# cage-challenge/cage-challenge-4

Measured on AMD Instinct MI355X. Metric: agent-env steps/sec (5 blue agents x N envs), higher is better.
Workload: dtype int32

## Files before the change

### cage_challenge_4_amd/csrc/cc4_engine.h

```cpp
#pragma once
#include "cc4_state.h"
#include "cc4_tables.h"

namespace cc4 {

struct Ctx { EnvState* s; EnvCold* c; Rng* r; HostDyn* hd; StepWork* w; unsigned long long* prof = nullptr;
             unsigned long long* aprof = nullptr; EvLog* lg = nullptr; const uint64_t* gpre = nullptr;
             const ExtAct* ext = nullptr; };

#if defined(__HIP_DEVICE_COMPILE__)
#define CC4_TICK(x, i) do { if ((x).prof) { unsigned long long _t = clock64(); (x).prof[(i)] += _t - (x).prof[15]; (x).prof[15] = _t; } } while (0)
#define CC4_TICK0(x) do { if ((x).prof) (x).prof[15] = clock64(); } while (0)
#define CC4_AT0(x) unsigned long long _at = (x).aprof ? clock64() : 0
#define CC4_AT(x, k) do { if ((x).aprof) { unsigned long long _n = clock64(); (x).aprof[(k)] += _n - _at; _at = _n; } } while (0)
#if defined(CC4_FINE)
#define CC4_FT0(x, r) unsigned long long _ft = ((x).aprof && (r) == 0) ? clock64() : 0
#define CC4_FT(x, r, k) do { if ((x).aprof && (r) == 0) { unsigned long long _n = clock64(); (x).aprof[88 + (k)] += _n - _ft; _ft = _n; } } while (0)
#else
#define CC4_FT0(x, r) do { } while (0)
#define CC4_FT(x, r, k) do { } while (0)
#endif
#else
#define CC4_FT0(x, r) do { } while (0)
#define CC4_FT(x, r, k) do { } while (0)
// ... 238 lines not shown
    const P8 q = proc_load8(x, h, i0);
    int hit = -1;
    CC4_UNROLL for (int k = 7; k >= 0; --k) if (i0 + k < n && pw_pid(q.v[k]) == pid) hit = i0 + k;
    if (hit >= 0) return hit;
  }
  return -1;
}
CC4_HD int find_proc(Ctx x, int h, int pid) { return find_proc(x, h, pid, proc_head(x, h)); }
CC4_HD int proc_ports(Ctx x, int h, const P8N& hd0) {
  const int n = hd0.n;
  int used = 0;
  CC4_UNROLL for (int k = 0; k < 8; ++k) if (k < n) used |= kind_port(pw_kind(hd0.v[k]));
  for (int i0 = 8; i0 < n; i0 += 8) {
    const P8 q = proc_load8(x, h, i0);
    CC4_UNROLL for (int k = 0; k < 8; ++k) if (i0 + k < n) used |= kind_port(pw_kind(q.v[k]));
  }
  return used;
}
CC4_HD int proc_ports(Ctx x, int h) { return proc_ports(x, h, proc_head(x, h)); }
CC4_HD void remove_proc_at(Ctx x, int h, int idx) {
  hd_touch(x, h);
  HostDyn& d = x.hd[h];
  const int n = d.nproc;
  for (int i0 = idx & ~7; i0 < n; i0 += 8) {
    const P8 q = proc_load8(x, h, i0);
    const uint32_t nxt = (i0 + 8 < n) ? proc_get(x, h, i0 + 8) : 0u;
    uint32_t* p = const_cast<uint32_t*>(proc_round_ptr(x, h, i0));
    CC4_UNROLL for (int k = 0; k < 8; ++k) {
      const int i = i0 + k;
      if (i < idx || i + 1 >= n) continue;
      p[k] = k < 7 ? q.v[(k + 1) & 7] : nxt;
    }
  }
  d.nproc = (uint16_t)(n - 1);
}
CC4_HD void ev_conn(Ctx x, int h) { ev_or(x, h, EV_CUR_CONN); }
CC4_HD void ev_proc(Ctx x, int h, int pid) {
  ev_or(x, h, EV_CUR_PROC);
  if (pid > 0 && blue_of_subnet(h_subnet(h)) >= 0) {
    if (x.s->npend >= MAX_PEND) { set_err(x, E_PEND_OVERFLOW); return; }
    x.s->pend[x.s->npend++] = ((uint32_t)h << 16) | (uint32_t)pid;
  }
}
CC4_HD void ev_proc_red(Ctx x, int r, int h, int pid) {
  ev_or(x, h, EV_CUR_PROC);
  if (blue_of_subnet(h_subnet(h)) >= 0) x.w->pend_r[r] = ((uint32_t)h << 16) | (uint32_t)pid;
}
CC4_HD void step_red_merge(Ctx x) {
  EnvState* s = x.s;
  uint32_t pr[NRED];
  CC4_UNROLL for (int r = 0; r < NRED; ++r) pr[r] = x.w->pend_r[r];
  CC4_UNROLL for (int r = 0; r < NRED; ++r) {
    if (!pr[r]) continue;
    if (s->npend >= MAX_PEND) set_err(x, E_PEND_OVERFLOW); else s->pend[s->npend++] = pr[r];
    x.w->pend_r[r] = 0;
  }
}
CC4_HD void pend_drop_host(Ctx x, int h) {
  EnvState* s = x.s;
  int n = 0;
  for (int i = 0; i < s->npend; ++i) if ((int)(s->pend[i] >> 16) != h) s->pend[n++] = s->pend[i];
  s->npend = (uint8_t)n;
}
CC4_HD bool subnet_blocked(Ctx x, int src_sub, int other_sub) { return (x.s->blocks[other_sub] >> src_sub) & 1u; }

struct S8 { uint64_t v[8]; uint64_t slots; };
CC4_HD uint64_t rs_word(const EnvState* s, int slot) { uint64_t v; __builtin_memcpy(&v, &s->spool[slot], 8); return v; }
CC4_HD void rs_word_put(EnvState* s, int slot, uint64_t v) { __builtin_memcpy(&s->spool[slot], &v, 8); }
CC4_HD S8 rs_load8(const EnvState* s, const RedAgent& a, int i0) {
  S8 q;
  __builtin_memcpy(&q.slots, &a.sord[i0], 8);
  CC4_UNROLL for (int k = 0; k < 8; ++k) q.v[k] = rs_word(s, (int)((q.slots >> (8 * k)) & 0xFF));
  return q;
}
CC4_HD int s8_slot(const S8& q, int k) { return (int)((q.slots >> (8 * k)) & 0xFF); }
CC4_HD int rsw_id(uint64_t v) { return (int)(v & 0xFFFF); }
CC4_HD int rsw_pid(uint64_t v) { return (int)((v >> 16) & 0xFFFF); }
CC4_HD int rsw_host(uint64_t v) { return (int)((v >> 32) & 0xFF); }
CC4_HD int rsw_flags(uint64_t v) { return (int)((v >> 40) & 0xFF); }
CC4_HD uint64_t rsw_make(int id, int pid, int host, int flags) {
  return (uint64_t)(id & 0xFFFF) | ((uint64_t)(pid & 0xFFFF) << 16) | ((uint64_t)(host & 0xFF) << 32) | ((uint64_t)(flags & 0xFF) << 40);
}
CC4_HD uint64_t rs_at(const EnvState* s, const RedAgent& a, int i) { return rs_word(s, a.sord[i]); }
CC4_HD int rs_find_id(const EnvState* s, const RedAgent& a, int id, int n) {
  for (int i0 = 0; i0 < n; i0 += 8) {
    const S8 q = rs_load8(s, a, i0);
    int hit = -1;
    CC4_UNROLL for (int k = 7; k >= 0; --k) if (i0 + k < n && rsw_id(q.v[k]) == id) hit = i0 + k;
    if (hit >= 0) return hit;
  }
  return -1;
}
CC4_HD int rs_find_id(const EnvState* s, const RedAgent& a, int id) { return rs_find_id(s, a, id, a.h.nsess); }
struct HostSess { int n, first, first_root; };
CC4_HD HostSess rs_on_host(const EnvState* s, const RedAgent& a, int h) {
  HostSess r; r.n = 0; r.first = -1; r.first_root = -1;
  const int n = a.h.nsess;
  for (int i0 = 0; i0 < n; i0 += 8) {
    const S8 q = rs_load8(s, a, i0);
    CC4_UNROLL for (int k = 0; k < 8; ++k)
      if (i0 + k < n && rsw_host(q.v[k]) == h) {
        r.n++;
        if (r.first < 0) r.first = i0 + k;
        if (r.first_root < 0 && (rsw_flags(q.v[k]) & RS_ROOT)) r.first_root = i0 + k;
      }
  }
  return r;
}
CC4_HD int rs_kth_on_host(const EnvState* s, const RedAgent& a, int h, int kth) {
  const int n = a.h.nsess;
  for (int i0 = 0; i0 < n; i0 += 8) {
    const S8 q = rs_load8(s, a, i0);
    int hit = -1;
    CC4_UNROLL for (int k = 0; k < 8; ++k)
      if (hit < 0 && i0 + k < n && rsw_host(q.v[k]) == h) { if (kth == 0) hit = i0 + k; kth--; }
    if (hit >= 0) return hit;
  }
  return -1;
}
CC4_HD int rs_find_host_pid(const EnvState* s, const RedAgent& a, int h, int pid) {
  const int n = a.h.nsess;
  for (int i0 = 0; i0 < n; i0 += 8) {
    const S8 q = rs_load8(s, a, i0);
    int hit = -1;
    CC4_UNROLL for (int k = 7; k >= 0; --k) if (i0 + k < n && rsw_host(q.v[k]) == h && rsw_pid(q.v[k]) == pid) hit = i0 + k;
    if (hit >= 0) return hit;
  }
  return -1;
}
struct RedPre { int si = -1; HostSess hs = {0, -1, -1}; bool ok = false; };
#if defined(__HIPCC__)
__device__ __forceinline__ RedPre rs_wave_query(const EnvState* s, int lane, int sid, int host) {
  const int r = lane >> 3, k = lane & 7, ra = r < NRED ? r : 0;
  const RedAgent& A = s->red[ra];
  const int ksid = __builtin_amdgcn_ds_bpermute(ra << 2, sid), khost = __builtin_amdgcn_ds_bpermute(ra << 2, host);
  const int n = (r < NRED && ksid >= 0) ? (int)A.h.nsess : 0;
  const int sh = 8 * k;
  RedPre p; p.ok = true;
  for (int i0 = 0; __ballot(i0 < n); i0 += 8) {
    const bool v = i0 + k < n;
    uint64_t w = 0;
    if (v) w = rs_word(s, A.sord[i0 + k]);
    const bool on = v && rsw_host(w) == khost;
    const uint32_t bid = (uint32_t)(__ballot(v && rsw_id(w) == ksid) >> sh) & 0xFFu;
    const uint32_t bh = (uint32_t)(__ballot(on) >> sh) & 0xFFu, br = (uint32_t)(__ballot(on && (rsw_flags(w) & RS_ROOT)) >> sh) & 0xFFu;
    if (p.si < 0 && bid) p.si = i0 + ctz32(bid);
    p.hs.n += __popc(bh);
    if (p.hs.first < 0 && bh) p.hs.first = i0 + ctz32(bh);
    if (p.hs.first_root < 0 && br) p.hs.first_root = i0 + ctz32(br);
  }
  return p;
}
#endif
CC4_HD void rs_list_remove(RedAgent& a, int idx) {
  uint64_t w[MAX_RS / 8];
  __builtin_memcpy(w, a.sord, MAX_RS);
  const int wi = idx >> 3, sh = 8 * (idx & 7);
  CC4_UNROLL for (int k = 0; k < MAX_RS / 8; ++k) {
    if (k < wi) continue;
    const uint64_t nxt = k + 1 < MAX_RS / 8 ? w[k + 1] : 0ull;
    uint64_t v = (w[k] >> 8) | (nxt << 56);
    if (k == wi && sh) v = (w[k] & ((1ull << sh) - 1ull)) | (v & ~((1ull << sh) - 1ull));
    w[k] = v;
  }
  __builtin_memcpy(a.sord, w, MAX_RS);
}
CC4_HD int rs_alloc_lowest(Ctx x) {
  for (int w = 0; w < RS_POOL / 32; ++w) {
    const uint32_t fr = ~x.s->spool_used[w];
    if (fr) return w * 32 + ctz32(fr);
  }
  return -1;
}
CC4_HD void rs_reserve(Ctx x) {
  uint32_t used[RS_POOL / 32];
  CC4_UNROLL for (int w = 0; w < RS_POOL / 32; ++w) used[w] = x.s->spool_used[w];
  int ty[NRED];
  CC4_UNROLL for (int r = 0; r < NRED; ++r) ty[r] = x.s->rexec[r].type;
  CC4_UNROLL for (int r = 0; r < NRED; ++r) {
    int slot = 0xFF;
    if (ty[r] == RA_EXPLOIT) {
      CC4_UNROLL for (int w = 0; w < RS_POOL / 32; ++w) {
        const uint32_t fr = ~used[w];
        if (slot == 0xFF && fr) { slot = w * 32 + ctz32(fr); used[w] |= 1u << (slot & 31); }
      }
    }
    x.w->rs_slot[r] = (uint8_t)slot;
  }
}
CC4_HD int rs_reserve_lane(const EnvState* s, uint32_t exploit_mask, int r) {
  if (!((exploit_mask >> r) & 1u)) return 0xFF;
  int k = popc32(exploit_mask & ((1u << r) - 1u));
  int slot = 0xFF;
  CC4_UNROLL for (int w = 0; w < RS_POOL / 32; ++w) {
    const uint32_t fr = ~s->spool_used[w];
    const int c = popc32(fr);
    if (slot == 0xFF) { if (k < c) slot = w * 32 + nth_bit(fr, k); else k -= c; }
  }
  return slot;
}
CC4_HD int rs_add(Ctx x, int r, int host, int pid, int flags, int slot = -1) {
  EnvState* s = x.s;
  RedAgent& a = s->red[r];
  if (slot < 0) slot = rs_alloc_lowest(x);
  if (a.h.nsess >= MAX_RS || slot < 0 || slot >= RS_POOL) { set_err(x, E_RSESS_OVERFLOW); return -1; }
  int id = 0;
  for (int i0 = 0; i0 < a.h.nsess; i0 += 8) {
    const S8 q = rs_load8(s, a, i0);
    CC4_UNROLL for (int k = 0; k < 8; ++k) if (i0 + k < a.h.nsess && rsw_id(q.v[k]) + 1 > id) id = rsw_id(q.v[k]) + 1;
  }
  (void)or_shared(&s->spool_used[slot >> 5], 1u << (slot & 31));
  rs_word_put(s, slot, rsw_make(id, pid, host, flags));
  if (flags & RS_ABSTRACT) {
    uint64_t* row = reinterpret_cast<uint64_t*>(x.c->kports[slot]);
    for (int k = 0; k < (MAXH + 7) / 8; ++k) row[k] = 0;
  }
  a.sord[a.h.nsess++] = (uint8_t)slot;
  a.h.rsc_dirty = 1; a.h.fsm_dirty = 1;
  if (!bit_get(a.live_hosts, host)) { bit_set(a.live_hosts, host); a.h.nlive++; }
  bit_set_shared(s->red_hosts, host);
  return a.h.nsess - 1;
}
CC4_HD void rs_host_left(Ctx x, int r, int gone) {
  RedAgent& a = x.s->red[r];
  bit_clr(a.live_hosts, gone); a.h.nlive--;
  uint32_t lw[NRED];
  CC4_UNROLL for (int q = 0; q < NRED; ++q) lw[q] = x.s->red[q].live_hosts[gone >> 5];
  uint32_t any_other = 0;
  CC4_UNROLL for (int q = 0; q < NRED; ++q) any_other |= lw[q];
  if (!((any_other >> (gone & 31)) & 1u)) bit_clr_shared(x.s->red_hosts, gone);
}
CC4_HD void rs_remove_at(Ctx x, int r, int idx, bool keep_record = false) {
  EnvState* s = x.s;
  RedAgent& a = s->red[r];
  const int slot = a.sord[idx];
  const int gone = rsw_host(rs_word(s, slot));
  if (!keep_record) bit_clr_shared(s->spool_used, slot);
  rs_list_remove(a, idx);
  a.h.nsess--;
  a.h.rsc_dirty = 1; a.h.fsm_dirty = 1;
  if (rs_on_host(s, a, gone).n == 0) rs_host_left(x, r, gone);
}
CC4_HD void rs_remove_on_host(Ctx x, int r, int h) {
  EnvState* s = x.s;
  RedAgent& a = s->red[r];
  const int n = a.h.nsess;
  int out = 0, removed = 0;
  bool left = false;
  for (int i0 = 0; i0 < n; i0 += 8) {
    const S8 q = rs_load8(s, a, i0);
    CC4_UNROLL for (int k = 0; k < 8; ++k) {
      if (i0 + k >= n) continue;
      const bool here = rsw_host(q.v[k]) == h;
      if (here && !(rsw_flags(q.v[k]) & RS_ORIG)) { bit_clr_shared(s->spool_used, s8_slot(q, k)); removed++; continue; }
      if (here) left = true;
      if (out != i0 + k) a.sord[out] = (uint8_t)s8_slot(q, k);
      out++;
    }
  }
  if (!removed) return;
  a.h.nsess = (uint8_t)out;
  a.h.rsc_dirty = 1; a.h.fsm_dirty = 1;
  if (!left) rs_host_left(x, r, h);
}
CC4_HD void rs_move_to_end(EnvState* s, RedAgent& a, int idx, int new_id) {
  const int slot = a.sord[idx];
  rs_list_remove(a, idx);
  a.sord[a.h.nsess - 1] = (uint8_t)slot;
  if (new_id >= 0) rs_word_put(s, slot, (rs_word(s, slot) & ~0xFFFFull) | (uint64_t)(new_id & 0xFFFF));
  a.h.rsc_dirty = 1;
}
CC4_HD bool sid_known(const RedAgent& a, const uint16_t* ks, int id, int nknown) {
  if (id < 256) return bit_get(a.known_bm, id);
  for (int i = 0; i < nknown; ++i) if (ks[i] == id) return true;
  return false;
}
CC4_HD void as_know_sid(Ctx x, int r, int id) {
  RedAgent& a = x.s->red[r];
  if (sid_known(a, x.c->known_sid[r], id, a.h.nknown)) return;
  if (a.h.nknown >= MAX_KS) { set_err(x, E_KS_OVERFLOW); return; }
  x.c->known_sid[r][a.h.nknown++] = (uint16_t)id;
  if (id < 256) bit_set(a.known_bm, id);
}
CC4_HD void obs_put(Ctx x, int r, bool key_ip, int host, int flags, bool subnet_known) {
  RedAgent& a = x.s->red[r];
  if (flags & OE_IFACE) bit_set(a.as_ip, host);
  if (flags & OE_SYSHN) bit_set(a.as_hn, host);
  if (subnet_known) a.h.as_subnet |= (uint16_t)(1u << h_subnet(host));
  uint8_t want = (uint8_t)(key_ip ? OE_KEY_IP : 0);
  uint32_t* has = a.obs_has[key_ip ? 1 : 0];
  if (bit_get(has, host)) {
    for (int i = 0; i < a.h.nobs; ++i)
      if (a.obs[i].host == host && (a.obs[i].flags & OE_KEY_IP) == want) { a.obs[i].flags |= (uint8_t)flags; return; }
  }
  bit_set(has, host);
  if (a.h.nobs >= MAX_OBS) { set_err(x, E_OBS_OVERFLOW); return; }
  a.obs[a.h.nobs].host = (uint8_t)host;
  a.obs[a.h.nobs].flags = (uint8_t)(flags | want);
  a.h.nobs++;
}
CC4_HD void obs_first(Ctx x, int r, int success, int atype, int ahost, int aarg) {
  RedAgent& a = x.s->red[r];
  if (a.h.obs_success != 0) return;
  a.h.obs_success = (uint8_t)success; a.h.obs_act_type = (uint8_t)atype; a.h.obs_act_host = (uint8_t)ahost; a.h.obs_act_arg = (uint8_t)aarg;
}

CC4_HD int path_to_root(int h, uint8_t* out) {
  int n = 0;
  out[n++] = (uint8_t)h;
  if (h == H_INTERNET) return n;
  int s = h_subnet(h);
  if (!h_is_router(h)) out[n++] = (uint8_t)h_make(s, 0);
  while (true) {
    int p = router_parent(s);
    if (p == S_INT) { out[n++] = (uint8_t)H_INTERNET; break; }
    out[n++] = (uint8_t)h_make(p, 0);
    s = p;
  }
  return n;
}
CC4_HD int route(int src, int dst, uint8_t* work) {
  uint8_t* a = work; uint8_t* b = work + 6; uint8_t* out = work + 12;
  int na = path_to_root(src, a), nb = path_to_root(dst, b);
  while (na >= 2 && nb >= 2 && a[na - 2] == b[nb - 2]) { na--; nb--; }
  int n = 0;
  for (int i = 0; i < na; ++i) out[n++] = a[i];
  for (int i = nb - 2; i >= 0; --i) out[n++] = b[i];
  return n;
}

CC4_HD int gen_pid(Ctx x, uint32_t* used) {
  while (true) {
    int pid = rng_range(x.r, 1000, 10000);
    if (!bit_get(used, pid - 1000)) { bit_set(used, pid - 1000); return pid; }
  }
}
CC4_HD int start_session_proc(Ctx x, int h, int kind) {
  HostDyn& st = x.hd[h];
  int mx = 0;
  for (int i = 0; i < st.nproc; ++i) if (st.procs[i].pid > mx) mx = st.procs[i].pid;
  int pid = mx + 1 + (int)rng_below(x.r, 9);
  st.procs[st.nproc].pid = (uint16_t)pid; st.procs[st.nproc].kind = (uint8_t)kind; st.procs[st.nproc].flags = 0;
  st.nproc++;
  return pid;
}
CC4_HD void host_backup(Ctx x, int h, int ip_octet) {
  const HostDyn& d = x.hd[h];
  HostStatic st;
  for (int i = 0; i < 8; ++i) st.procs[i] = d.procs[i];
  for (int i = 0; i < 5; ++i) st.svcs[i] = d.svcs[i];
  st.nproc = (uint8_t)d.nproc; st.nsvc = (uint8_t)hd_nsvc(d); st.exists = (uint8_t)(1 | ((d.gtmp & 1) << 1)); st.ip_octet = (uint8_t)ip_octet;
  if (d.nproc > PIN - 1 || hd_nsvc(d) > 5) set_err(x, E_PROC_OVERFLOW);
  __builtin_memcpy(&x.c->hs[h], &st, sizeof(HostStatic));
}
CC4_HD void host_restore(Ctx x, int h) {
  hd_touch(x, h);
  HostDyn& d = x.hd[h];
  HostStatic st;
  __builtin_memcpy(&st, &x.c->hs[h], sizeof(HostStatic));
  for (int i = 0; i < 8; ++i) d.procs[i] = st.procs[i];
  for (int i = 0; i < 5; ++i) d.svcs[i] = st.svcs[i];
  d.nproc = st.nproc; d.gtmp = 0; d.nsf = st.nsvc;
  x.s->hev[h] = 0;
  eph_clear(x, h);
  pend_drop_host(x, h);
}

struct ResetCarry { uint64_t env_key; };
enum : int { RESET_WS_SEEN = 0, RESET_WS_DUP = 288, RESET_WS_HOSTS = 576, RESET_WS_WORDS = 584 };

CC4_HD void reset_zero(EnvState* s, HostDyn* hd, EnvCold* c, int t, int nt) {
  static_assert(offsetof(EnvState, rng) == 0, "the generator leads the row");
  uint32_t* w = (uint32_t*)s;
  for (size_t i = sizeof(Rng) / 4 + (size_t)t; i < offsetof(EnvState, hd) / 4; i += (size_t)nt) w[i] = i == PA_WORD ? w[i] & PA_WORD_MASK : 0;
  uint32_t* hw = (uint32_t*)hd;
  for (size_t i = (size_t)t; i < sizeof(HostDyn) * MAXH / 4; i += (size_t)nt) hw[i] = 0;
  uint32_t* b = (uint32_t*)c->hs;
  for (size_t i = (size_t)t; i < sizeof(c->hs) / 4; i += (size_t)nt) b[i] = 0;
}
static_assert(sizeof(RSess) * RS_POOL >= 4 * 282, "the idle session pool holds the 9000-bit pid set of the generation");
CC4_HD uint32_t* reset_used_set(EnvState* s) { return reinterpret_cast<uint32_t*>(s->spool); }
CC4_HD void reset_used_clear(EnvState* s, int t, int nt) { uint32_t* u = reset_used_set(s); for (int i = t; i < 282; i += nt) u[i] = 0; }
template <int RNG_MODE>
CC4_HD void reset_gen_host(Ctx x, int h) {
  EnvState* s = x.s;
  if (!bit_get(s->exists, h)) return;
  if (RNG_MODE == 1) rng_set_stream(x.r, ST_GEN_HOST + (uint32_t)h);
  HostDyn& st = x.hd[h];
  st.gtmp = (uint8_t)rng_below(x.r, 2);
  if (h_is_router(h)) return;
  int n = 0;
  auto put = [&](int kind, int pid) {
    st.svcs[n].kind = (uint8_t)kind; st.svcs[n].pid = (uint16_t)pid; st.svcs[n].st = (uint8_t)(SV_ACTIVE | 5);
    st.procs[n].kind = (uint8_t)kind; st.procs[n].pid = (uint16_t)pid; st.procs[n].flags = 0;
    n++;
  };
  auto pid = [&]() { return RNG_MODE == 1 ? rng_range(x.r, 1000, 10000) : gen_pid(x, reset_used_set(s)); };
  put(K_SSHD, pid());
  int sub = h_subnet(h);
  if (sub == S_OZA || sub == S_OZB) put(K_OT, pid());
  int p_apache = pid(), p_mysql = pid(), p_smtp = pid();
  int n_add = (int)rng_below(x.r, 4);
  uint32_t left = 7;
  for (int k = 0; k < n_add; ++k) {
    int o = nth_bit(left, (int)rng_below(x.r, (uint32_t)popc32(left)));
    left &= ~(1u << o);
    put(o == 0 ? K_APACHE : (o == 1 ? K_MYSQL : K_SMTP), o == 0 ? p_apache : (o == 1 ? p_mysql : p_smtp));
  }
  for (int i = 0; i < n; ++i) (void)rng_random(x.r);
  hd_set_nsvc(st, n); st.nproc = (uint16_t)n;
  if (RNG_MODE == 1) { st.procs[5].pid = (uint16_t)p_apache; st.procs[6].pid = (uint16_t)p_mysql; st.svcs[6].pid = (uint16_t)p_smtp; }
}
struct ResetHostLater { CC4_HD void operator()(Ctx, int) const {} };
struct ResetHostNow { CC4_HD void operator()(Ctx x, int h) const { reset_gen_host<0>(x, h); } };
CC4_HD void reset_mission_phases(EnvState* s, int steps) {
  int q = steps / 3, rem = steps % 3;
  s->steps = steps;
  s->phase_len[0] = q + (rem >= 1 ? 1 : 0); s->phase_len[1] = q + (rem == 2 ? 1 : 0); s->phase_len[2] = q;
}
template <int RNG_MODE, typename HostHook>
CC4_HD ResetCarry reset_topology(Ctx x, uint64_t seed, int steps, bool continue_stream, int policy, uint32_t topo_seed, uint32_t* ws,
                                 bool rng_is_copy, HostHook host_placed) {
  EnvState* s = x.s;
  if (!continue_stream) rng_seed(&s->rng, seed, (uint32_t)RNG_MODE);
  s->rng_mode = (uint8_t)RNG_MODE;
  s->policy = (uint8_t)policy_at_reset(s, policy);
  rng_begin_episode(x.r);
  ResetCarry k; k.env_key = x.r->s_lo;
  if (RNG_MODE == 1 && topo_seed) x.r->s_lo = (uint64_t)topo_seed;
  reset_mission_phases(s, steps);
  if (RNG_MODE == 1) for (int i = 0; i < RESET_WS_WORDS; ++i) ws[i] = 0;
  {
    uint32_t* avail = x.w->scratch;
    for (int i = 0; i < 8; ++i) avail[i] = 0xFFFFFFFFu;
    int n = 256;
    for (int sn = 0; sn < NSUB; ++sn) {
      int v = nth_set(avail, 8, (int)rng_below(x.r, (uint32_t)n));
      s->cidr_octet[sn] = (uint8_t)v;
      bit_clr(avail, v);
      n--;
    }
  }
  for (int sn = 0; sn < NSUB; ++sn) {
    uint32_t* ips = x.w->scratch;
    for (int i = 0; i < 8; ++i) ips[i] = 0xFFFFFFFFu;
    ips[0] &= ~1u; ips[7] &= 0x7FFFFFFFu;
    int n = 254;
    auto place = [&](int h, int v) {
      bit_clr(ips, v); n--; bit_set(s->exists, h); x.hd[h].procs[PIN - 1].pid = (uint16_t)v;
      host_placed(x, h);
    };
    if (sn == S_INT) { place(H_INTERNET, nth_set(ips, 8, (int)rng_below(x.r, (uint32_t)n))); continue; }
    place(h_make(sn, 0), nth_set(ips, 8, (int)rng_below(x.r, (uint32_t)n)));
    int nu = 3 + (int)rng_below(x.r, 8);
    for (int i = 0; i < nu; ++i) place(h_make(sn, 1 + i), nth_set(ips, 8, (int)rng_below(x.r, (uint32_t)n)));
    int ns = 1 + (int)rng_below(x.r, 6);
    for (int i = 0; i < ns; ++i) place(h_make(sn, 11 + i), last_set(ips, 8));
    s->n_users[sn] = (uint8_t)nu; s->n_servers[sn] = (uint8_t)ns;
  }
  if (RNG_MODE == 1 && rng_is_copy) s->rng = *x.r;
  return k;
}
CC4_HD void reset_pid_serial(Ctx x, uint32_t* used) {
  EnvState* s = x.s;
  for (int h = 0; h < MAXH; ++h) {
    if (!bit_get(s->exists, h) || h_is_router(h)) continue;
    HostDyn& st = x.hd[h];
    const int n = hd_nsvc(st);
    const int sub = h_subnet(h);
    const int nfix = (sub == S_OZA || sub == S_OZB) ? 2 : 1;
    Rng t; bool forked = false;
    auto settle = [&](int v0, bool* moved) {
      int v = v0 - 1000;
      *moved = false;
      while (bit_get(used, v)) {
        if (!forked) { rng_fork(&t, x.r, ST_GEN_REDRAW + (uint32_t)h); forked = true; }
        v = (int)rng_below(&t, 9000);
        *moved = true;
      }
      bit_set(used, v);
      return v + 1000;
    };
    for (int i = 0; i < nfix; ++i) {
      bool moved;
      const int v = settle(st.svcs[i].pid, &moved);
      if (moved) { st.svcs[i].pid = (uint16_t)v; st.procs[i].pid = (uint16_t)v; }
    }
    for (int k = 0; k < 3; ++k) {
      const int kind = k == 0 ? K_APACHE : (k == 1 ? K_MYSQL : K_SMTP);
      const int v0 = k == 0 ? st.procs[5].pid : (k == 1 ? st.procs[6].pid : st.svcs[6].pid);
      bool moved;
      const int v = settle(v0, &moved);
      if (moved) for (int i = nfix; i < n; ++i) if (st.svcs[i].kind == kind) { st.svcs[i].pid = (uint16_t)v; st.procs[i].pid = (uint16_t)v; }
    }
    st.procs[5].pid = 0; st.procs[6].pid = 0; st.svcs[6].pid = 0;
  }
}
CC4_HD void reset_agents(Ctx x) {
  EnvState* s = x.s;
  for (int b = 0; b < NBLUE; ++b) {
    int nsub = blue_nsub(b);
    (void)rng_below(x.r, (uint32_t)nsub);
    int cnt = 0;
    for (int i = 0; i < nsub; ++i) { int sn = blue_subnet_alloc(b, i); cnt += 1 + s->n_users[sn] + s->n_servers[sn]; }
    int c = (int)rng_below(x.r, (uint32_t)cnt);
    int ph = -1;
    for (int i = 0; i < nsub && ph < 0; ++i) {
      int sn = blue_subnet_alloc(b, i), nu = s->n_users[sn], ns = s->n_servers[sn];
      if (c < 1 + nu) ph = h_make(sn, c);
      else if (c < 1 + nu + ns) ph = h_make(sn, 11 + (c - 1 - nu));
      else c -= 1 + nu + ns;
    }
    s->blue[b].parent_host = (uint8_t)ph;
  }
  {
    int g = 0;
    for (int sn = 0; sn < NSUB - 1; ++sn) for (int i = 0; i < s->n_users[sn]; ++i) s->green_host[g++] = (uint8_t)h_make(sn, 1 + i);
    s->n_green = (uint8_t)g;
  }
  for (int r = 0; r < NRED; ++r) {
    int sn = red_subnet_alloc(r, (int)rng_below(x.r, (uint32_t)red_nsub(r)));
    int c = (int)rng_below(x.r, (uint32_t)(s->n_users[sn] + s->n_servers[sn]));
    s->red[r].h.start_host = (uint8_t)(c < s->n_users[sn] ? h_make(sn, 1 + c) : h_make(sn, 11 + (c - s->n_users[sn])));
    s->red[r].h.new_sess_host = 0xFF;
  }
}
CC4_HD void reset_seal_host(Ctx x, int h) {
  host_backup(x, h, x.hd[h].procs[PIN - 1].pid);
  x.hd[h].procs[PIN - 1].pid = 0; x.hd[h].gtmp = 0;
}
CC4_HD void reset_host_sessions(Ctx x, int h) {
  EnvState* s = x.s;
  if (!bit_get(s->exists, h)) return;
  rng_set_stream(x.r, ST_GEN_SESS + (uint32_t)h);
  if (blue_of_subnet(h_subnet(h)) >= 0) (void)start_session_proc(x, h, K_SESS_BLUE);
  if (h != H_INTERNET && h_is_user(h)) (void)start_session_proc(x, h, K_SESS_GREEN);
  if (h == s->red[0].h.start_host) (void)start_session_proc(x, h, K_SESS_RED);
  reset_seal_host(x, h);
}
CC4_HD void reset_sessions_agent_order(Ctx x) {
  EnvState* s = x.s;
  for (int b = 0; b < NBLUE; ++b) {
    int ph = s->blue[b].parent_host;
    (void)start_session_proc(x, ph, K_SESS_BLUE);
    for (int i = 0; i < blue_nsub(b); ++i) {
      int sn = blue_subnet_alloc(b, i);
      for (int sl = 0; sl < SLOTS; ++sl) {
        int h = h_make(sn, sl);
        if (!bit_get(s->exists, h) || h == ph) continue;
        (void)start_session_proc(x, h, K_SESS_BLUE);
      }
    }
  }
  for (int g = 0; g < s->n_green; ++g) (void)start_session_proc(x, s->green_host[g], K_SESS_GREEN);
  (void)start_session_proc(x, s->red[0].h.start_host, K_SESS_RED);
}
CC4_HD void reset_seal_all_hosts(Ctx x) {
  EnvState* s = x.s;
  for (int h = 0; h < MAXH; ++h) {
    if (bit_get(s->exists, h)) reset_seal_host(x, h);
    eph_clear(x, h);
  }
  s->npend = 0;
}
CC4_HD void reset_finish(Ctx x, ResetCarry k, int steps, uint32_t topo_seed, bool rng_is_copy) {
  EnvState* s = x.s;
  {
    const HostDyn& d = x.hd[s->red[0].h.start_host];
    int red0_pid = 0;
    for (int i = 0; i < d.nproc; ++i) if (d.procs[i].kind == K_SESS_RED) red0_pid = d.procs[i].pid;
    (void)rs_add(x, 0, s->red[0].h.start_host, red0_pid, RS_ABSTRACT | RS_ORIG);
    s->red[0].h.active = 1;
  }
  for (int r = 0; r < NRED; ++r) {
    RedAgent& a = s->red[r];
    int h = a.h.start_host;
    bit_set(a.as_ip, h); bit_set(a.as_hn, h); a.h.as_subnet |= (uint16_t)(1u << h_subnet(h));
    if (r == 0) {
      as_know_sid(x, 0, 0);
      obs_put(x, 0, false, h, OE_SESS | OE_IFACE | OE_SYSHN, true);
      obs_first(x, 0, T_UNKNOWN, RA_NONE, 0, 0);
    }
    a.h.exec_type = RA_SLEEP;
  }
  s->done = (uint8_t)(0 >= steps - 1);
  s->n_actions = NBLUE + s->n_green + NRED;
  if (topo_seed) x.r->s_lo = k.env_key;
  if (rng_is_copy) s->rng = *x.r;
  rng_park(&s->rng);
}
CC4_HD void env_reset_counter_mode(Ctx x, uint64_t seed, int steps, bool continue_stream, int policy, uint32_t topo_seed, uint32_t* ws,
                                   bool rng_is_copy) {
  reset_zero(x.s, x.hd, x.c, 0, 1);
  ResetCarry k = reset_topology<1>(x, seed, steps, continue_stream, policy, topo_seed, ws, rng_is_copy, ResetHostLater{});
  {
    Rng t; rng_fork(&t, x.r, ST_GEN_HOST);
    Ctx xh = x; xh.r = &t;
    for (int h = 0; h < MAXH; ++h) reset_gen_host<1>(xh, h);
  }
  reset_pid_serial(x, reset_used_set(x.s));
  reset_used_clear(x.s, 0, 1);
  reset_agents(x);
  {
    Rng t; rng_fork(&t, x.r, ST_GEN_SESS);
    Ctx xh = x; xh.r = &t;
    for (int h = 0; h < MAXH; ++h) reset_host_sessions(xh, h);
  }
// ... 350 lines not shown
  return h_make(sn, 11 + (c - before));
}
CC4_HD constexpr int green_as_dest_loop(uint64_t pre, int c, int* sn_out) {
  int sn = 0, before = 0;
  for (int k = 0; k < NSUB - 2; ++k) { const int tot = (int)((pre >> (8 * k)) & 0xFF); if (tot <= c) { sn = k + 1; before = tot; } }
  *sn_out = sn;
  return h_make(sn, 11 + (c - before));
}
CC4_HD constexpr uint32_t green_lw_active(uint64_t pre) {
  static_assert(SV_ACTIVE == 0x80 && MAXSV == 7, "the active bit is a status byte's top bit; seven of them");
  return dot4_u8((uint32_t)(pre >> 32) & 0x00808080u, 0x00402010u, dot4_u8((uint32_t)pre & 0x80808080u, 0x08040201u, 0u)) >> 7;
}
CC4_HD constexpr uint32_t green_lw_active_loop(uint64_t pre) {
  uint32_t act = 0;
  for (int i = 0; i < MAXSV; ++i) if ((pre >> (8 * i)) & SV_ACTIVE) act |= 1u << i;
  return act;
}
static_assert(green_lw_active(0x0080818283FF7F80ull) == green_lw_active_loop(0x0080818283FF7F80ull) && green_lw_active(0xFF00000000000000ull) == 0 &&
              green_lw_active(0x0080808080808080ull) == 0x7F && green_lw_active(0x0000000080000000ull) == 0x08, "green_lw_active == the loop");
namespace cc4_forms_check {
constexpr uint32_t sv[MAXSV] = {0x81000001u, 0x05FFFFFFu, 0x80123456u, 0x7F000000u, 0xFFFFFFFFu, 0x01020304u, 0x85000000u};
static_assert(green_lw_status(sv, 7) == green_lw_status_loop(sv, 7) && green_lw_status(sv, 7) == 0x008501FF7F800581ull && green_lw_status(sv, 0) == 0 &&
              green_lw_status(sv, 4) == green_lw_status_loop(sv, 4) && green_lw_status(sv, 5) == 0x000000FF7F800581ull, "green_lw_status == the loop");
constexpr int dest_sn(uint64_t pre, int c, bool loop) { int sn = 0; const int d = loop ? green_as_dest_loop(pre, c, &sn) : green_as_dest(pre, c, &sn); return d * 16 + sn; }
constexpr uint64_t tot = 0x302A241E18120C06ull, gap = 0x0909090903030300ull;
static_assert(dest_sn(tot, 0, false) == dest_sn(tot, 0, true) && dest_sn(tot, 5, false) == dest_sn(tot, 5, true) && dest_sn(tot, 6, false) == dest_sn(tot, 6, true) &&
              dest_sn(tot, 47, false) == dest_sn(tot, 47, true) && dest_sn(tot, 41, false) == dest_sn(tot, 41, true) && dest_sn(gap, 0, false) == dest_sn(gap, 0, true) &&
              dest_sn(gap, 2, false) == dest_sn(gap, 2, true) && dest_sn(gap, 3, false) == dest_sn(gap, 3, true) && dest_sn(gap, 8, false) == dest_sn(gap, 8, true),
              "green_as_dest == the loop");
}
CC4_HD bool green_local_work(Ctx x, int gh, uint64_t pre, bool* want_phish, double fp_rate = 0.01, double phish_rate = 0.01) {
  const uint32_t act = green_lw_active(pre);
  if (!act) return false;
  const int c = nth_bit8(act, (int)rng_below(x.r, (uint32_t)popc32(act)));
  const uint32_t st = (uint32_t)(pre >> (8 * c)) & 0xFF;
  int rel = (int)(st & 0x7F) * 20;
  if ((int)rng_below(x.r, 100) >= rel) return false;
  if (rng_random_lt(x.r, fp_rate)) { int port = eph_port(x, gh); ev_proc(x, gh, 0); ev_log(x, gh, gh, 1, gh, port, 0xFF, 0, 0); }
  if (rng_random_lt(x.r, phish_rate)) *want_phish = true;
  return true;
}
CC4_HD bool green_access_service(Ctx x, int gh, uint64_t pre, double fp_rate = 0.01) {
  int own = h_subnet(gh);
  const int n = (int)(pre >> 56);
  const int c = (int)rng_below(x.r, (uint32_t)n);
  int sn;
  const int dest = green_as_dest(pre, c, &sn);
  const int dest_port = eph_port(x, dest);
  int ds = sn;
  if (subnet_blocked(x, ds, own) || subnet_blocked(x, own, ds)) { ev_conn(x, dest); ev_log(x, gh, dest, 0, dest, 0, gh, 8800, 0); return false; }
  if (rng_random_lt(x.r, fp_rate)) { ev_conn(x, dest); ev_log(x, gh, dest, 0, gh, 0, dest, dest_port, 0); }
  return true;
}

CC4_HD void red_result(Ctx x, int r, const Act& a, int success) {
  int arg = a.type == RA_DRS ? a.arg : 0;
  obs_first(x, r, success, a.type, a.host, arg);
}
CC4_HD void red_drs(Ctx x, int r, const Act& a, RedPre pre = RedPre()) {
  EnvState* s = x.s;
  int sn = a.arg; bool any = false;
  if ((pre.ok ? pre.si : rs_find_id(s, s->red[r], a.sid)) < 0) { red_result(x, r, a, T_FALSE); return; }
  bool allowed = (red_allowed_mask(r) >> sn) & 1u;
  RedAgent& A = s->red[r];
  const int lo = sn * SLOTS + 1, w0 = lo >> 5, off = lo & 31, w1 = (w0 + 1 < 5) ? w0 + 1 : w0;
  const uint32_t e0 = s->exists[w0], e1 = s->exists[w1], h0 = A.obs_has[1][w0], h1 = A.obs_has[1][w1];
  auto field = [&](uint32_t a0, uint32_t a1) { uint32_t v = a0 >> off; if (off > 16 && w1 != w0) v |= a1 << (32 - off); return v & 0xFFFFu; };
  const uint32_t ex = field(e0, e1);
  any = ex != 0;
  if (allowed && ex) {
    const uint32_t had = field(h0, h1) & ex;
    uint32_t fresh = ex & ~had;
    const uint32_t m0 = ex << off, m1 = (off > 16 && w1 != w0) ? ex >> (32 - off) : 0u;
    A.as_ip[w0] |= m0; A.obs_has[1][w0] = h0 | m0;
    if (m1) { A.as_ip[w1] |= m1; A.obs_has[1][w1] = h1 | m1; }
    A.h.as_subnet |= (uint16_t)(1u << sn);
    int n = A.h.nobs;
    while (fresh) {
      const int b = ctz32(fresh); fresh &= fresh - 1;
      if (n >= MAX_OBS) { set_err(x, E_OBS_OVERFLOW); break; }
      A.obs[n].host = (uint8_t)(lo + b); A.obs[n].flags = (uint8_t)(OE_IFACE | OE_KEY_IP);
      n++;
    }
    A.h.nobs = (uint8_t)n;
    uint32_t again = had;
    while (again) { const int b = ctz32(again); again &= again - 1; obs_put(x, r, true, lo + b, OE_IFACE, true); }
  }
  red_result(x, r, a, any ? T_TRUE : T_UNKNOWN);
}
CC4_HD int port_of_bit(int pb) { return pb == PB_22 ? 22 : (pb == PB_80 ? 80 : (pb == PB_3390 ? 3390 : (pb == PB_25 ? 25 : (pb == PB_1 ? 1 : 443)))); }
CC4_HD void red_scan(Ctx x, int r, const Act& a, double rate, RedPre pre = RedPre()) {
  EnvState* s = x.s;
  RedAgent& A = s->red[r];
  int si = pre.ok ? pre.si : rs_find_id(s, A, a.sid);
  if (si < 0) { red_result(x, r, a, T_FALSE); return; }
  const int slot = A.sord[si];
  const uint64_t sw = rs_word(s, slot);
  if (!(rsw_flags(sw) & RS_ABSTRACT)) { red_result(x, r, a, T_FALSE); return; }
  int src = rsw_host(sw), tgt = a.host;
  if (subnet_blocked(x, h_subnet(src), h_subnet(tgt))) { red_result(x, r, a, T_FALSE); return; }
  const bool fixed_le_rate = rng_random_le(x.r, rate);
  int ports = 0;
  const P8N hd0 = proc_head(x, tgt);
  const int np = hd0.n;
  for (int i0 = 0; i0 < np; i0 += 8) {
    P8 q = p8_of(hd0);
    if (i0) q = proc_load8(x, tgt, i0);
    CC4_UNROLL for (int k8 = 0; k8 < 8; ++k8) {
      if (i0 + k8 >= np) continue;
      int k = pw_kind(q.v[k8]);
      int pb = kind_port(k);
      if (!pb) continue;
      ports |= pb;
      if (fixed_le_rate || kind_is_decoy(k)) { ev_conn(x, tgt); int ep = eph_port(x, tgt, (i0 + k8) & 63); ev_log(x, 200 + r, tgt, 0, tgt, port_of_bit(pb), src, ep, 0); }
    }
  }
  if (ports) {
    obs_put(x, r, true, tgt, OE_IFACE, false);
    x.c->kports[slot][tgt] = (uint8_t)(PB_HAS | ports);
  }
  red_result(x, r, a, T_TRUE);
}
CC4_HD int exploit_new_session(Ctx x, int r, int parent_sid, int tgt, const P8N& hd0) {
  (void)parent_sid;
  int pid = create_pid(x, tgt, hd0);
  if (!add_proc_n(x, tgt, hd0.n, pid, K_SHELL, 0)) return -1;
  x.hd[tgt].nsf = (uint8_t)((hd0.nsf & 0x0F) | ((((hd0.nsf >> 4) | HF_CMD) & ~HF_ESC_LAST) << 4));
  return rs_add(x, r, tgt, pid, RS_CHILD, x.w->rs_slot[r]);
}
CC4_HD void red_exploit(Ctx x, int r, const Act& a, RedPre pre = RedPre()) {
  EnvState* s = x.s;
  RedAgent& A = s->red[r];
  int si = pre.ok ? pre.si : rs_find_id(s, A, a.sid);
  if (si < 0) { red_result(x, r, a, T_FALSE); return; }
  const int slot = A.sord[si];
  const uint64_t sw = rs_word(s, slot);
  if (!(rsw_flags(sw) & RS_ABSTRACT)) { red_result(x, r, a, T_FALSE); return; }
  int src = rsw_host(sw), tgt = a.host;
  const P8N thd0 = proc_head(x, tgt);
  int known = x.c->kports[slot][tgt];
  if (!(known & PB_HAS)) { red_result(x, r, a, T_FALSE); return; }
  if (subnet_blocked(x, h_subnet(src), h_subnet(tgt))) { red_result(x, r, a, T_FALSE); return; }
  enum { X_HTTPRFI = 0, X_HTTPSRFI = 1, X_SSH = 2, X_SQLI = 3, X_HARAKA = 4 };
  uint32_t opts = 0;
  if (known & PB_80) opts |= 1u << X_HTTPRFI;
  if (known & PB_443) opts |= 1u << X_HTTPSRFI;
  if (known & PB_22) opts |= 1u << X_SSH;
  if ((known & PB_3390) && (known & (PB_80 | PB_443))) opts |= 1u << X_SQLI;
  if (known & PB_25) opts |= 1u << X_HARAKA;
  if (opts == 0) { red_result(x, r, a, T_FALSE); return; }
  int sel = ctz32(opts);
  if (popc32(opts) > 1) {
    int top = (opts >> X_HARAKA) & 1u ? X_HARAKA : ((opts >> X_SQLI) & 1u ? X_SQLI : ((opts >> X_HTTPSRFI) & 1u ? X_HTTPSRFI : X_HTTPRFI));
    opts &= ~(1u << top);
    sel = nth_bit(opts, (int)rng_below(x.r, (uint32_t)popc32(opts)));
    (void)rng_random(x.r);
  }
  const int tnp = thd0.n;
  if (sel == X_SSH) {
    uint8_t* work = reinterpret_cast<uint8_t*>(x.w->scratch + 6 * r);
    int nh = route(src, tgt, work);
    for (int i = 0; i < nh; ++i) if (!rng_random_le(x.r, 0.050000000000000044)) { ev_conn(x, work[12 + i]); ev_log(x, 200 + r, work[12 + i], 0, tgt, 0, src, 22, 0); }
    int vp = -1;
    for (int i0 = 0; i0 < tnp && vp < 0; i0 += 8) {
      P8 q = p8_of(thd0);
      if (i0) q = proc_load8(x, tgt, i0);
      CC4_UNROLL for (int k = 7; k >= 0; --k) if (i0 + k < tnp && pw_kind(q.v[k]) == K_SSHD) vp = i0 + k;
    }
    if (vp < 0) { red_result(x, r, a, T_FALSE); return; }
    obs_put(x, r, true, tgt, OE_IFACE, false);
    const int bf_port = eph_port(x, tgt);
    ev_conn(x, tgt);
    ev_log(x, 200 + r, tgt, 0, tgt, 22, src, bf_port, 0, 10);
    int ni = exploit_new_session(x, r, a.sid, tgt, thd0);
    if (ni < 0) { red_result(x, r, a, T_FALSE); return; }
    const uint64_t nw = rs_at(s, A, ni);
    ev_proc_red(x, r, tgt, rsw_pid(nw));
    ev_log(x, 200 + r, tgt, 1, 0xFF, 0, 0xFF, 0, rsw_pid(nw));
    obs_put(x, r, true, tgt, OE_SESS | OE_IFACE | OE_SYSHN, false);
    obs_put(x, r, true, src, OE_IFACE, false);
    A.h.new_sess_host = (uint8_t)tgt; A.h.new_sess_id = (uint16_t)rsw_id(nw);
    red_result(x, r, a, T_TRUE);
    return;
  }
  int vp = -1, vk = 0;
  {
    const uint32_t want = sel == X_HTTPRFI ? ((1u << K_APACHE) | (1u << K_DEC_APACHE) | (1u << K_DEC_VSFTPD))
                        : sel == X_HTTPSRFI ? (1u << K_DEC_TOMCAT)
                        : sel == X_SQLI ? (1u << K_MYSQL)
                        : ((1u << K_SMTP) | (1u << K_DEC_HARAKA));
    for (int i0 = 0; i0 < tnp && vp < 0; i0 += 8) {
      P8 q = p8_of(thd0);
      if (i0) q = proc_load8(x, tgt, i0);
      CC4_UNROLL for (int k = 7; k >= 0; --k) if (i0 + k < tnp && ((want >> pw_kind(q.v[k])) & 1u)) { vp = i0 + k; vk = pw_kind(q.v[k]); }
    }
  }
  if (vp < 0) { red_result(x, r, a, T_FALSE); return; }
  bool decoy = kind_is_decoy(vk);
  const int xport = sel == X_HTTPRFI ? 80 : (sel == X_HTTPSRFI ? 443 : (sel == X_SQLI ? 3390 : 25));
  if (decoy) { ev_conn(x, tgt); int ep = eph_port(x, tgt, 1); ev_log(x, 200 + r, tgt, 0, tgt, xport, src, ep, 0); }
  obs_put(x, r, true, tgt, OE_IFACE, false);
  bool works = (sel == X_SQLI) || decoy;
  if (!works) { red_result(x, r, a, T_FALSE); return; }
  if (rng_random_le(x.r, 0.0)) { red_result(x, r, a, T_FALSE); return; }
  const int lport = eph_port(x, tgt, 2);
  if (decoy) { ev_conn(x, tgt); int ep = eph_port(x, tgt, 3); ev_log(x, 200 + r, tgt, 0, tgt, lport, src, ep, 0); red_result(x, r, a, T_FALSE); return; }
  int ni = exploit_new_session(x, r, a.sid, tgt, thd0);
  if (ni < 0) { red_result(x, r, a, T_FALSE); return; }
  const uint64_t nw = rs_at(s, A, ni);
  if (!rng_random_le(x.r, 0.050000000000000044)) { ev_proc_red(x, r, tgt, rsw_pid(nw)); ev_log(x, 200 + r, tgt, 1, 0xFF, 0, 0xFF, 0, rsw_pid(nw)); }
  obs_put(x, r, true, tgt, OE_SESS | OE_IFACE | OE_SYSHN, false);
  obs_put(x, r, true, src, OE_IFACE, false);
  A.h.new_sess_host = (uint8_t)tgt; A.h.new_sess_id = (uint16_t)rsw_id(nw);
  red_result(x, r, a, T_TRUE);
}
CC4_HD void red_privesc(Ctx x, int r, const Act& a, RedPre pre = RedPre()) {
  EnvState* s = x.s;
  RedAgent& A = s->red[r];
  int h = a.host;
  const HostSess hs = pre.ok ? pre.hs : rs_on_host(s, A, h);
  const int n = hs.n;
  int target = hs.first_root;
  if (n == 0) { red_result(x, r, a, T_FALSE); return; }
  if (target < 0) {
    target = rs_kth_on_host(s, A, h, (int)rng_below(x.r, (uint32_t)n));
    { int ss = pre.ok ? pre.si : rs_find_id(s, A, a.sid);
      if (ss < 0 || !(rsw_flags(rs_at(s, A, ss)) & RS_ABSTRACT)) { red_result(x, r, a, T_FALSE); return; } }
    const int tslot = A.sord[target];
    s->spool[tslot].flags |= RS_ROOT;
    hd_touch(x, h);
    hd_set_files(x.hd[h], hd_files(x.hd[h]) | HF_ESC | HF_ESC_LAST);
    int pi = find_proc(x, h, s->spool[tslot].pid);
    if (pi >= 0) proc_put(x, h, pi, proc_get(x, h, pi) | ((uint32_t)PF_ROOT << 24));
  }
  obs_put(x, r, false, h, OE_SESS, false);
  { const uint64_t tw = rs_at(s, A, target); if (rsw_flags(tw) & RS_ABSTRACT) as_know_sid(x, r, rsw_id(tw)); }
  if ((pre.ok ? pre.si : rs_find_id(s, A, a.sid)) >= 0 && h_slot(h) == 11) {
    uint32_t m = info_links(h_subnet(h));
    for (int sn = 0; sn < NSUB; ++sn) if ((m >> sn) & 1u) obs_put(x, r, false, h_make(sn, 11), OE_IFACE, false);
  }
  red_result(x, r, a, T_TRUE);
}
CC4_HD void red_impact(Ctx x, int r, const Act& a, RedPre pre = RedPre()) {
  EnvState* s = x.s;
  RedAgent& A = s->red[r];
  int h = a.host;
  if ((pre.ok ? pre.hs : rs_on_host(s, A, h)).first_root < 0) { red_result(x, r, a, T_FALSE); return; }
  HostDyn& d = x.hd[h];
  const SvTab sv = svc_load(d);
  int si = -1;
  uint32_t sw = 0;
  CC4_UNROLL for (int i = MAXSV - 1; i >= 0; --i) if (i < sv.n && svw_kind(sv.w[i]) == K_OT && (svw_st(sv.w[i]) & SV_ACTIVE)) { si = i; sw = sv.w[i]; }
  if (si < 0) { red_result(x, r, a, T_FALSE); return; }
  if ((pre.ok ? pre.si : rs_find_id(s, A, a.sid)) < 0) { red_result(x, r, a, T_FALSE); return; }
  hd_touch(x, h);
  d.svcs[si].st = (uint8_t)(svw_st(sw) & ~SV_ACTIVE);
  int pi = find_proc(x, h, (int)(sw & 0xFFFF));
  if (pi >= 0) remove_proc_at(x, h, pi);
  obs_put(x, r, false, h, 0, false);
  red_result(x, r, a, T_TRUE);
}
CC4_HD void red_degrade(Ctx x, int r, const Act& a, RedPre pre = RedPre()) {
  EnvState* s = x.s;
  RedAgent& A = s->red[r];
  int h = a.host;
  if ((pre.ok ? pre.hs : rs_on_host(s, A, h)).first_root < 0) { red_result(x, r, a, T_FALSE); return; }
  HostDyn& d = x.hd[h];
  int n = 0;
  hd_touch(x, h);
  const SvTab sv = svc_load(d);
  CC4_UNROLL for (int i = 0; i < MAXSV; ++i) if (i < sv.n && (svw_st(sv.w[i]) & SV_ACTIVE)) {
    n++;
    int rel = svw_st(sv.w[i]) & 0x7F;
    if (rel > 0) rel--;
    d.svcs[i].st = (uint8_t)(SV_ACTIVE | rel);
  }
  if (n == 0) { red_result(x, r, a, T_FALSE); return; }
  obs_put(x, r, false, h, 0, false);
  red_result(x, r, a, T_TRUE);
}
CC4_HD void red_deception(Ctx x, int r, const Act& a, RedPre pre = RedPre()) {
  EnvState* s = x.s;
  RedAgent& A = s->red[r];
  if ((pre.ok ? pre.si : rs_find_id(s, A, a.sid)) < 0) { red_result(x, r, a, T_FALSE); return; }
  int tgt = a.host;
  const double det_rate = (x.ext && (a.busy & AQ_RATE0)) ? x.c->xrate[r][0] : 0.5;
  const double fp_rate = (x.ext && (a.busy & AQ_RATE1)) ? x.c->xrate[r][1] : 0.1;
  const P8N hd0 = proc_head(x, tgt);
  const int np = hd0.n;
  for (int i0 = 0; i0 < np; i0 += 8) {
    P8 q = p8_of(hd0);
    if (i0) q = proc_load8(x, tgt, i0);
    CC4_UNROLL for (int k = 0; k < 8; ++k) {
      if (i0 + k >= np) continue;
      bool decoy = kind_is_decoy(pw_kind(q.v[k]));
      bool rep = false;
      if (rng_random_le(x.r, det_rate) && decoy) rep = true;
      else if (rng_random_le(x.r, fp_rate) && !decoy) rep = true;
      if (rep) obs_put(x, r, false, tgt, OE_IFACE, false);
    }
  }
  red_result(x, r, a, T_TRUE);
}
CC4_HD void red_session_check(Ctx x, int r) {
  EnvState* s = x.s;
  RedAgent& A = s->red[r];
  obs_first(x, r, T_TRUE, RA_NONE, 0, 0);
  if (A.h.nsess == 0) return;
  if (rsw_id(rs_at(s, A, 0)) != 0 && rsw_id(rs_at(s, A, A.h.nsess - 1)) != 0 && rs_find_id(s, A, 0) < 0) {
    int c = (int)rng_below(x.r, (uint32_t)A.h.nsess);
    rs_move_to_end(s, A, c, 0);
    for (int i = 0; i < A.h.nsess; ++i) s->spool[A.sord[i]].flags &= (uint8_t)~RS_CHILD;
  }
  A.h.rsc_listed = 1;
  if (!A.h.rsc_dirty) return;
  const B5 live = b5_load(A.live_hosts);
  { const B5 ip = b5_load(A.as_ip), hn = b5_load(A.as_hn); b5_store(A.as_ip, b5_or(ip, live)); b5_store(A.as_hn, b5_or(hn, live)); }
  {
    uint32_t sub = 0;
    CC4_UNROLL for (int sn = 0; sn < NSUB; ++sn) {
      const int lo = sn * SLOTS, w = lo >> 5, off = lo & 31;
      uint32_t bits = live.w[w] >> off;
      if (off > 32 - SLOTS && w + 1 < 5) bits |= live.w[w + 1] << (32 - off);
      if (bits & ((1u << SLOTS) - 1u)) sub |= 1u << sn;
    }
    A.h.as_subnet |= (uint16_t)sub;
  }
  const int n = A.h.nsess;
  int fresh = 0, fresh_id = 0;
  for (int i0 = 0; i0 < n; i0 += 8) {
    const S8 q = rs_load8(s, A, i0);
    uint32_t kw[8];
    CC4_UNROLL for (int k = 0; k < 8; ++k) kw[k] = A.known_bm[(rsw_id(q.v[k]) >> 5) & 7];
    CC4_UNROLL for (int k = 0; k < 8; ++k) {
      if (i0 + k >= n || !(rsw_flags(q.v[k]) & RS_ABSTRACT)) continue;
      const int id = rsw_id(q.v[k]);
      if (id < 256 && ((kw[k] >> (id & 31)) & 1u)) continue;
      fresh++; fresh_id = id;
    }
  }
  if (fresh == 1) as_know_sid(x, r, fresh_id);
  else if (fresh > 1)
    for (int i = 0; i < n; ++i) {
      const int h = rsw_host(rs_at(s, A, i));
      bool first = true;
      for (int j = 0; j < i && first; ++j) first = rsw_host(rs_at(s, A, j)) != h;
      if (!first) continue;
      for (int j = i; j < n; ++j) {
        const uint64_t w = rs_at(s, A, j);
        if (rsw_host(w) == h && (rsw_flags(w) & RS_ABSTRACT)) as_know_sid(x, r, rsw_id(w));
      }
    }
  A.h.rsc_dirty = 0;
}
CC4_HD void red_withdraw(Ctx x, int r, const Act& a, RedPre pre = RedPre()) {
  EnvState* s = x.s;
  RedAgent& A = s->red[r];
  if ((pre.ok ? pre.si : rs_find_id(s, A, a.sid)) < 0) { red_result(x, r, a, T_FALSE); return; }
  const int h = a.arg;
  uint16_t* ids = reinterpret_cast<uint16_t*>(x.w->scratch + 36);
  int n = 0;
  const int cap = (int)((sizeof(x.w->scratch) - 36 * 4) / 2);
  for (int pass = 0; pass < 2; ++pass)
    for (int i = 0; i < A.h.nsess; ++i) {
      const uint64_t w = rs_at(s, A, i);
      if (rsw_host(w) != h) continue;
      bool child = (rsw_flags(w) & RS_CHILD) != 0;
      if ((pass == 0 && child) || (pass == 1 && !child && rsw_id(w) != 0)) { if (n < cap) ids[n++] = (uint16_t)rsw_id(w); else set_err(x, E_RSESS_OVERFLOW); }
    }
  { int self = rs_find_id(s, A, a.sid); if (rsw_host(rs_at(s, A, self)) == h) { if (n < cap) ids[n++] = (uint16_t)a.sid; else set_err(x, E_RSESS_OVERFLOW); } }
  if (n == 0) { red_result(x, r, a, T_FALSE); return; }
  int ok = T_FALSE;
  for (int k = 0; k < n; ++k) {
    int self = rs_find_id(s, A, a.sid), ti = rs_find_id(s, A, ids[k]);
    if (self < 0 || ti < 0) { ok = T_FALSE; break; }
    int pid = rsw_pid(rs_at(s, A, ti));
    int pi = find_proc(x, h, pid);
    if (pi < 0) { ok = T_FALSE; break; }
    kill_process(x, h, pi, proc_get(x, h, pi));
    ok = T_TRUE;
  }
  red_result(x, r, a, ok);
}
CC4_HD void red_execute(Ctx x, int r, const Act& a, RedPre pre = RedPre()) {
  switch (a.type) {
    case RA_DRS: red_drs(x, r, a, pre); break;
    case RA_AGGR: red_scan(x, r, a, (x.ext && (a.busy & AQ_RATE0)) ? x.c->xrate[r][0] : 0.75, pre); break;
    case RA_STEALTH: red_scan(x, r, a, (x.ext && (a.busy & AQ_RATE0)) ? x.c->xrate[r][0] : 0.25, pre); break;
    case RA_DECEPTION: red_deception(x, r, a, pre); break;
    case RA_EXPLOIT: red_exploit(x, r, a, pre); break;
    case RA_PRIVESC: red_privesc(x, r, a, pre); break;
    case RA_IMPACT: red_impact(x, r, a, pre); break;
    case RA_DEGRADE: red_degrade(x, r, a, pre); break;
    case RA_INVALID: obs_first(x, r, T_FALSE, RA_NONE, 0, 0); break;
    case RA_WITHDRAW: red_withdraw(x, r, a, pre); break;
    default: obs_first(x, r, T_UNKNOWN, RA_NONE, 0, 0); break;
  }
}

CC4_HD int fsm_next(int cur, int act, bool success) {
  uint64_t row;
  if (success) switch (cur) {
    case FS_K: row = 0xffffff221ull; break;  case FS_KD: row = 0xffffff331ull; break;
    case FS_S: row = 0xffff42ff3ull; break;  case FS_SD: row = 0xffff53ff3ull; break;
    case FS_U: row = 0x2ff6ffff5ull; break;  case FS_UD: row = 0x3ff7ffff5ull; break;
    case FS_R: row = 0x266fffff7ull; break;  case FS_RD: row = 0x377fffff7ull; break;
    default: row = 0xffffffff8ull; break;
  } else switch (cur) {
    case FS_K: row = 0xffffff000ull; break;  case FS_KD: row = 0xffffff111ull; break;
    case FS_S: row = 0xffff22ff2ull; break;  case FS_SD: row = 0xffff33ff3ull; break;
    case FS_U: row = 0x4ff4ffff4ull; break;  case FS_UD: row = 0x5ff5ffff5ull; break;
    case FS_R: row = 0x666fffff6ull; break;  case FS_RD: row = 0x777fffff7ull; break;
    default: row = 0xffffffff8ull; break;
  }
  int v = (int)((row >> (4 * act)) & 0xF);
  return v == 0xF ? 0xFF : v;
}
CC4_HD int fsm_get(const RedAgent& A, int h) {
  const int v = (A.fsm_st4[h >> 1] >> (4 * (h & 1))) & 0xF;
  return v ? v - 1 : FS_NONE;
}
CC4_HD void fsm_put(RedAgent& A, int h, int st) {
  const int sh = 4 * (h & 1);
  A.fsm_st4[h >> 1] = (uint8_t)((A.fsm_st4[h >> 1] & ~(0xF << sh)) | ((st + 1) << sh));
}
CC4_HD void fsm_set_state(RedAgent& A, int h, int st) {
  if (st >= FS_U && st <= FS_RD) bit_set(A.fsm_ur, h); else bit_clr(A.fsm_ur, h);
  if ((st & 1) || st == FS_F) bit_set(A.fsm_nodrs, h); else bit_clr(A.fsm_nodrs, h);
  fsm_put(A, h, st);
}
CC4_HD void fsm_apply(Ctx x, int r, RedHdr& H, int h, int act, bool success) {
  RedAgent& A = x.s->red[r];
  int cur = fsm_get(A, h);
  if (cur == FS_NONE) return;
  int nx = fsm_next(cur, act, success);
  if (nx == FS_U) nx = ((red_allowed_mask(r) >> h_subnet(h)) & 1u) ? FS_U : FS_F;
  if (nx == 0xFF) nx = cur;
  if (nx != cur) fsm_set_state(A, h, nx);
  if (nx == FS_F && cur != FS_F) {
    int n = 0;
    for (int i = 0; i < H.fsm_n; ++i) if (A.fsm_order[i] != h) A.fsm_order[n++] = A.fsm_order[i];
    H.fsm_n = (uint8_t)n;
  }
}
CC4_HD void fsm_observe(Ctx x, int r, RedHdr& H) {
  RedAgent& A = x.s->red[r];
  CC4_AT0(x);
  if (H.obs_success == T_IN_PROGRESS && H.nobs == 0 && H.rsc_listed && !H.fsm_dirty) return;
  if (H.obs_act_type <= RA_WITHDRAW && H.obs_success != T_IN_PROGRESS && H.obs_success != 0) {
    bool ok = H.obs_success == T_TRUE;
    int t = H.obs_act_type;
    if (t == RA_DRS) {
      const int lo = H.obs_act_arg * SLOTS, hi = lo + SLOTS - 1;
      for (int w = lo >> 5; w <= (hi >> 5) && w < 5; ++w) {
        uint32_t m = A.fsm_known[w];
        if (ok) m &= ~A.fsm_nodrs[w];
        const int l = lo - 32 * w, u = hi - 32 * w;
        if (l > 0) m &= 0xFFFFFFFFu << l;
        if (u < 31) m &= (2u << u) - 1u;
        while (m) { int b = ctz32(m); m &= m - 1; fsm_apply(x, r, H, w * 32 + b, t, ok); }
      }
    } else if (t == RA_PRIVESC || t == RA_IMPACT || t == RA_DEGRADE) {
      int h = H.obs_act_host;
      if (bit_get(A.fsm_known, h) && bit_get(A.fsm_hn, h)) fsm_apply(x, r, H, h, t, ok);
    } else {
      fsm_apply(x, r, H, H.obs_act_host, t, ok);
    }
  }
  CC4_AT(x, 3);
  B5 seen = b5_zero();
  for (int i = 0; i < H.nobs; ++i) {
    int h = A.obs[i].host; int f = A.obs[i].flags;
    if (f & OE_SESS) b5_set(seen, h);
    bool hn = !(f & OE_KEY_IP) || (f & OE_SYSHN);
    bool ip = (f & OE_KEY_IP) || (f & OE_IFACE);
    if (!ip) {
      if (!(bit_get(A.fsm_known, h) && bit_get(A.fsm_hn, h))) { set_err(x, E_UNREACHABLE); }
      continue;
    }
    if (!bit_get(A.fsm_known, h)) {
      fsm_set_state(A, h, H.fsm_step == 0 ? FS_U : FS_K);
      A.fsm_order[H.fsm_n++] = (uint8_t)h;
      bit_set(A.fsm_known, h);
    }
    if (hn) bit_set(A.fsm_hn, h);
  }
  CC4_AT(x, 4);
  if (H.rsc_listed) {
    const B5 live = b5_load(A.live_hosts), known = b5_load(A.fsm_known), hn = b5_load(A.fsm_hn);
    seen = b5_or(seen, live);
    if (b5_any(b5_andn(live, known)))
      for (int i = 0; i < H.nsess; ++i) {
        int h = rsw_host(rs_at(x.s, A, i));
        if (bit_get(A.fsm_known, h)) continue;
        fsm_set_state(A, h, H.fsm_step == 0 ? FS_U : FS_K);
        A.fsm_order[H.fsm_n++] = (uint8_t)h;
        bit_set(A.fsm_known, h);
      }
    b5_store(A.fsm_hn, b5_or(hn, live));
    H.fsm_dirty = 0;
  }
  CC4_AT(x, 5);
  {
    const B5 lost = b5_andn(b5_load(A.fsm_ur), seen);
    if (b5_any(lost))
      CC4_UNROLL for (int w = 0; w < 5; ++w) {
        uint32_t m = lost.w[w];
        while (m) { int b = ctz32(m); m &= m - 1; fsm_set_state(A, w * 32 + b, FS_KD); }
      }
  }
  CC4_AT(x, 6);
}
CC4_HD int fsm_choose_host_discovery(Ctx x, int r, RedHdr& H) {
  RedAgent& A = x.s->red[r];
  uint32_t order = 0; int nst = 0; uint32_t seen = 0;
  for (int i = 0; i < H.fsm_n && nst < 8; ++i) {
    int st = fsm_get(A, A.fsm_order[i]);
    if (!((seen >> st) & 1u)) { seen |= 1u << st; order |= (uint32_t)st << (4 * nst); nst++; }
  }
  int sum = 0;
  for (int k = 0; k < nst; ++k) { int st = (order >> (4 * k)) & 0xF; sum += st <= FS_SD ? 20 : (st <= FS_UD ? 10 : 0); }
  int chosen_state;
  if (sum > 0) {
    double mult = 1.0 / ((double)sum / 100.0);
    double last = 0.0;
    for (int k = 0; k < nst; ++k) { int st = (order >> (4 * k)) & 0xF; int p = st <= FS_SD ? 20 : (st <= FS_UD ? 10 : 0); last = last + ((double)p / 100.0) * mult; }
    double u = rng_random(x.r);
    double run = 0.0; int idx = 0;
    for (int k = 0; k < nst; ++k) {
      int st = (order >> (4 * k)) & 0xF; int p = st <= FS_SD ? 20 : (st <= FS_UD ? 10 : 0);
      run = run + ((double)p / 100.0) * mult;
      if (run / last <= u) idx++;
    }
    if (idx >= nst) idx = nst - 1;
    chosen_state = (order >> (4 * idx)) & 0xF;
  } else {
    chosen_state = (order >> (4 * (int)rng_below(x.r, (uint32_t)nst))) & 0xF;
  }
  int n_all = 0, n_srv = 0;
  for (int i = 0; i < H.fsm_n; ++i) {
    int h = A.fsm_order[i];
    if (fsm_get(A, h) != chosen_state) continue;
    n_all++;
    if (h_is_server(h) && bit_get(A.fsm_hn, h)) n_srv++;
  }
  int want_srv = -1;
  if (n_all > 1 && n_srv > 0) {
    double i01 = rng_random(x.r);
    want_srv = (i01 <= 0.75 || n_srv == n_all) ? 1 : 0;
  }
  int cnt = want_srv < 0 ? n_all : (want_srv ? n_srv : n_all - n_srv);
  int c = (int)rng_below(x.r, (uint32_t)cnt);
  for (int i = 0; i < H.fsm_n; ++i) {
    int h = A.fsm_order[i];
    if (fsm_get(A, h) != chosen_state) continue;
    bool srv = h_is_server(h) && bit_get(A.fsm_hn, h);
    if (want_srv >= 0 && (int)srv != want_srv) continue;
    if (c-- == 0) return h;
  }
  return A.fsm_order[0];
}
CC4_HD constexpr uint32_t fsm_pk_switch(bool discovery, int host_state) {
  if (!discovery) switch (host_state) {
    case FS_K:  return 0xF432u << 16 | (RA_DRS | RA_AGGR << 4 | RA_STEALTH << 8);
    case FS_KD: return 0xFF42u << 16 | (RA_AGGR | RA_STEALTH << 4);
    case FS_S:  return 0xF431u << 16 | (RA_DRS | RA_EXPLOIT << 4 | RA_DECEPTION << 8);
    case FS_SD: return 0xFF43u << 16 | (RA_EXPLOIT | RA_DECEPTION << 4);
    case FS_U:  return 0xF442u << 16 | (RA_DRS | RA_PRIVESC << 4 | RA_WITHDRAW << 8);
    case FS_UD: return 0xFF44u << 16 | (RA_PRIVESC | RA_WITHDRAW << 4);
    case FS_R:  return 0x4432u << 16 | (RA_DRS | RA_DEGRADE << 4 | RA_IMPACT << 8 | RA_WITHDRAW << 12);
    default:    return 0xF442u << 16 | (RA_DEGRADE | RA_IMPACT << 4 | RA_WITHDRAW << 8);
  } else switch (host_state) {
    case FS_K:  return 0xF441u << 16 | (RA_DRS | RA_AGGR << 4 | RA_STEALTH << 8);
    case FS_KD: return 0xFF44u << 16 | (RA_AGGR | RA_STEALTH << 4);
    case FS_S:  return 0xF441u << 16 | (RA_DRS | RA_EXPLOIT << 4 | RA_DECEPTION << 8);
    case FS_SD: return 0xFF44u << 16 | (RA_EXPLOIT | RA_DECEPTION << 4);
    case FS_U:  return 0xF440u << 16 | (RA_DRS | RA_PRIVESC << 4 | RA_WITHDRAW << 8);
    case FS_UD: return 0xFF44u << 16 | (RA_PRIVESC | RA_WITHDRAW << 4);
    case FS_R:  return 0x4444u << 16 | (RA_DRS | RA_DEGRADE << 4 | RA_IMPACT << 8 | RA_WITHDRAW << 12);
    default:    return 0xF442u << 16 | (RA_DEGRADE | RA_IMPACT << 4 | RA_WITHDRAW << 8);
  }
}
struct FsmPkTab { uint32_t v[16]; };
CC4_HD constexpr int fsm_pk_index(bool discovery, int host_state) { return (discovery ? 8 : 0) + (host_state < 7 ? host_state : 7); }
constexpr FsmPkTab make_fsm_pk_tab() {
  FsmPkTab t{};
  for (int d = 0; d < 2; ++d) for (int st = 0; st < 8; ++st) t.v[fsm_pk_index(d != 0, st)] = fsm_pk_switch(d != 0, st);
  return t;
}
constexpr bool fsm_pk_tab_matches() {
  const FsmPkTab t = make_fsm_pk_tab();
  for (int d = 0; d < 2; ++d) {
    for (int st = 0; st <= FS_F; ++st) if (t.v[fsm_pk_index(d != 0, st)] != fsm_pk_switch(d != 0, st)) return false;
    if (t.v[fsm_pk_index(d != 0, FS_NONE)] != fsm_pk_switch(d != 0, FS_NONE)) return false;
  }
  return true;
}
static_assert(fsm_pk_tab_matches(), "fsm_get_action's option table == its switch");
#if defined(__HIP_DEVICE_COMPILE__)
static __device__ const FsmPkTab fsm_pk_tab = make_fsm_pk_tab();
#else
static constexpr FsmPkTab fsm_pk_tab = make_fsm_pk_tab();
#endif
CC4_HD uint32_t fsm_pk(bool discovery, int host_state) { return fsm_pk_tab.v[fsm_pk_index(discovery, host_state)]; }
CC4_HD Act fsm_get_action(Ctx x, int r, RedHdr& H, bool observed = false) {
  EnvState* s = x.s;
  RedAgent& A = s->red[r];
  Act out; out.type = RA_SLEEP; out.host = 0; out.arg = 0; out.ticks = 1; out.sid = 0; out.busy = 0;
  CC4_FT0(x, r);
  if (!observed) fsm_observe(x, r, H);
  CC4_FT(x, r, 5);
  if (H.obs_success == T_IN_PROGRESS) { H.fsm_step++; return out; }
  int n = H.fsm_n;
  if (n == 0) { set_err(x, E_FSM_NO_HOST); H.fsm_step++; return out; }
  const bool discovery = (s->policy & 3) == RP_DISCOVERY;
  int host;
  if (!discovery) host = A.fsm_order[rng_below(x.r, (uint32_t)n)];
  else host = fsm_choose_host_discovery(x, r, H);
  CC4_FT(x, r, 6);
  const uint32_t pk = fsm_pk(discovery, fsm_get(A, host));
  const int fl = rng_random_quarter(x.r);
  int k = 0;
  for (int i = 0; i < 4; ++i) if ((int)((pk >> (16 + 4 * i)) & 0xF) <= fl) k++;
  int t = (int)((pk >> (4 * k)) & 0xF);
  out.type = (uint8_t)t; out.host = (uint8_t)host;
  bool bad = false;
  if (t == RA_DRS) {
    uint32_t known = H.as_subnet;
    if (known == 0) bad = true; else out.arg = (uint8_t)nth_bit(known, (int)rng_below(x.r, (uint32_t)popc32(known)));
  }
  if ((t == RA_PRIVESC || t == RA_IMPACT || t == RA_DEGRADE) && !bit_get(A.fsm_hn, host)) bad = true;
  if (!bad) {
    if (H.nknown == 0) bad = true; else out.sid = x.c->known_sid[r][rng_below(x.r, (uint32_t)H.nknown)];
  }
  if (bad) { set_err(x, E_UNREACHABLE); out.type = RA_SLEEP; }
  out.ticks = (uint8_t)red_duration(out.type);
  H.fsm_step++;
  CC4_FT(x, r, 7);
  return out;
}
CC4_HD Act random_red_get_action(Ctx x, int r, RedHdr& H) {
  RedAgent& A = x.s->red[r];
  Act out; out.type = RA_SLEEP; out.host = 0; out.arg = 0; out.ticks = 1; out.sid = 0; out.busy = 0;
  const int nip = popc32(A.as_ip[0]) + popc32(A.as_ip[1]) + popc32(A.as_ip[2]) + popc32(A.as_ip[3]) + popc32(A.as_ip[4]);
  const int nhn = popc32(A.as_hn[0]) + popc32(A.as_hn[1]) + popc32(A.as_hn[2]) + popc32(A.as_hn[3]) + popc32(A.as_hn[4]);
  const int nsub = popc32(H.as_subnet), nsid = H.nknown;
  const uint8_t types[10] = {RA_DRS, RA_AGGR, RA_STEALTH, RA_EXPLOIT, RA_PRIVESC, RA_DEGRADE, RA_DECEPTION, RA_IMPACT, RA_WITHDRAW, RA_SLEEP};
  uint32_t valid = 0;
  for (int c = 0; c < 10; ++c) {
    int t = types[c];
    bool ok = true;
    if (t != RA_SLEEP && nsid == 0) ok = false;
    if (t == RA_DRS && nsub == 0) ok = false;
    if ((t == RA_AGGR || t == RA_STEALTH || t == RA_EXPLOIT || t == RA_DECEPTION || t == RA_WITHDRAW) && nip == 0) ok = false;
    if ((t == RA_PRIVESC || t == RA_DEGRADE || t == RA_IMPACT || t == RA_WITHDRAW) && nhn == 0) ok = false;
    if (ok) valid |= 1u << c;
  }
  const int t = types[nth_bit(valid, (int)rng_below(x.r, (uint32_t)popc32(valid)))];
  auto pick_sid = [&]() { return (int)x.c->known_sid[r][rng_below(x.r, (uint32_t)nsid)]; };
  auto pick_ip = [&]() { return nth_set(A.as_ip, 5, (int)rng_below(x.r, (uint32_t)nip)); };
  auto pick_hn = [&]() { return nth_set(A.as_hn, 5, (int)rng_below(x.r, (uint32_t)nhn)); };
  out.type = (uint8_t)t;
  switch (t) {
    case RA_DRS: out.arg = (uint8_t)nth_bit(H.as_subnet, (int)rng_below(x.r, (uint32_t)nsub)); out.sid = (uint16_t)pick_sid(); break;
    case RA_AGGR: case RA_STEALTH: case RA_DECEPTION: out.sid = (uint16_t)pick_sid(); out.host = (uint8_t)pick_ip(); break;
    case RA_EXPLOIT: out.host = (uint8_t)pick_ip(); out.sid = (uint16_t)pick_sid(); break;
    case RA_PRIVESC: case RA_DEGRADE: case RA_IMPACT: out.host = (uint8_t)pick_hn(); out.sid = (uint16_t)pick_sid(); break;
    case RA_WITHDRAW: out.sid = (uint16_t)pick_sid(); out.host = (uint8_t)pick_ip(); out.arg = (uint8_t)pick_hn(); break;
    default: break;
  }
  out.ticks = (uint8_t)red_duration(out.type);
  H.fsm_step++;
  return out;
}
CC4_HD void red_validate(Ctx x, int r, const RedHdr& H, Act& a) {
  RedAgent& A = x.s->red[r];
  if (a.type >= RA_SLEEP) return;
  bool ok = true;
  if (!sid_known(A, x.c->known_sid[r], a.sid, H.nknown)) ok = false;
  if (a.type == RA_DRS) { if (!((H.as_subnet >> a.arg) & 1u)) ok = false; }
  else if (a.type == RA_PRIVESC || a.type == RA_IMPACT || a.type == RA_DEGRADE) { if (!bit_get(A.as_hn, a.host)) ok = false; }
  else if (a.type == RA_WITHDRAW) { if (!bit_get(A.as_ip, a.host) || !bit_get(A.as_hn, a.arg)) ok = false; }
  else { if (!bit_get(A.as_ip, a.host)) ok = false; }
  if (!ok) { a.type = RA_INVALID; a.ticks = 1; }
}

CC4_HD constexpr uint32_t red_zone_hosts(int r, int w) {
  uint32_t m = 0;
  for (int i = 0; i < red_nsub(r); ++i) {
    int lo = red_subnet_alloc(r, i) * SLOTS - 32 * w, hi = lo + SLOTS - 1;
    if (hi < 0 || lo > 31) continue;
    uint32_t up = hi >= 31 ? 0xFFFFFFFFu : ((2u << hi) - 1u);
    uint32_t dn = lo <= 0 ? 0xFFFFFFFFu : (0xFFFFFFFFu << lo);
    m |= up & dn;
  }
  return m;
}
CC4_HD void red_reassign(Ctx x, uint32_t foreign) {
  EnvState* s = x.s;
  uint32_t* mv = x.w->scratch; int nm = 0;
  const int cap = (int)(sizeof(x.w->scratch) / 4);
  for (int r = 0; r < NRED; ++r) {
    if (!((foreign >> r) & 1u)) continue;
    const RedAgent& A = s->red[r];
    const int n = A.h.nsess;
    for (int i0 = 0; i0 < n; i0 += 8) {
      const S8 q = rs_load8(s, A, i0);
      CC4_UNROLL for (int k = 0; k < 8; ++k) {
        if (i0 + k >= n) continue;
        const int host = rsw_host(q.v[k]);
        const int sn = h_subnet(host);
        if ((red_allowed_mask(r) >> sn) & 1u) continue;
        const int to = red_of_subnet(sn);
        if (to < 0) { set_err(x, E_UNREACHABLE); continue; }
        if (nm < cap) mv[nm++] = (uint32_t)r | ((uint32_t)to << 3) | ((uint32_t)(i0 + k) << 6) | ((uint32_t)s8_slot(q, k) << 12);
        else set_err(x, E_RSESS_OVERFLOW);
      }
    }
  }
  int gone_from[NRED];
  CC4_UNROLL for (int r = 0; r < NRED; ++r) gone_from[r] = 0;
  for (int m = 0; m < nm; ++m) {
    const uint32_t w = mv[m];
    const int from = (int)(w & 7u), to = (int)((w >> 3) & 7u), slot = (int)((w >> 12) & 0xFFu);
    RedAgent& F = s->red[from];
    int shift = 0;
    CC4_UNROLL for (int r = 0; r < NRED; ++r) if (r == from) shift = gone_from[r];
    int i = (int)((w >> 6) & 0x3Fu) - shift;
    if (i < 0 || i >= F.h.nsess || F.sord[i] != slot) {
      i = -1;
      for (int k = 0; k < F.h.nsess; ++k) if (F.sord[k] == slot) { i = k; break; }
      if (i < 0) continue;
    }
    CC4_UNROLL for (int r = 0; r < NRED; ++r) if (r == from) gone_from[r]++;
    const uint64_t rec = rs_word(s, slot);
    const int old_host = rsw_host(rec), old_pid = rsw_pid(rec), old_flags = rsw_flags(rec), old_id = rsw_id(rec);
    rs_remove_at(x, from, i, true);
    int ni = rs_add(x, to, old_host, old_pid, RS_ABSTRACT | (old_flags & RS_ROOT), slot);
    if (ni < 0) { bit_clr_shared(s->spool_used, slot); continue; }
    if (F.h.new_sess_host == old_host && F.h.new_sess_id == old_id) {
      obs_first(x, to, T_UNKNOWN, RA_NONE, 0, 0);
      obs_put(x, to, true, old_host, OE_SESS | OE_IFACE | OE_SYSHN, false);
      as_know_sid(x, to, rsw_id(rs_at(s, s->red[to], ni)));
    }
  }
  int ns[NRED];
  CC4_UNROLL for (int r = 0; r < NRED; ++r) ns[r] = s->red[r].h.nsess;
  CC4_UNROLL for (int r = 0; r < NRED; ++r) s->red[r].h.active = (uint8_t)(ns[r] > 0);
}


CC4_HD int step_phase_of(int st, int len0, int len1, int len2) {
  if (st < len0) return 0;
  if (st < len0 + len1) return 1;
  if (st < len0 + len1 + len2) return 2;
  return -1;
}
CC4_HD bool step_phase(Ctx x, bool init_accumulators = true) {
  EnvState* s = x.s;
  {
    const int st = s->step_count;
    const int ph = step_phase_of(st, s->phase_len[0], s->phase_len[1], s->phase_len[2]);
    if (ph < 0) { set_err(x, E_STEP_PAST_END); return false; }
    s->obs_dirty = (uint8_t)(ph > s->phase ? OD_PHASE : 0);
    if (ph > s->phase) s->phase = ph;
  }
  rng_begin_step(&s->rng, (uint32_t)s->step_count);
  if (x.lg) { x.lg->n = 0; x.lg->step = (uint32_t)s->step_count; }
  if (x.ext) { x.c->gfail[0] = 0; x.c->gfail[1] = 0; x.c->gfail[2] = 0; }
  s->action_cost = 0.f;
  if (init_accumulators) {
    s->brm = 0; s->n_restore = 0;
    s->n_actions = NBLUE + s->n_green + NRED;
  }
  return true;
}
CC4_HD Act blue_random_policy(Ctx x, int b) {
  EnvState* s = x.s;
  Act a; a.type = BA_SLEEP; a.host = 0; a.arg = 0; a.ticks = 1; a.sid = 0; a.busy = 0;
  rng_set_stream(x.r, ST_BLUE_POL + (uint32_t)b);
  (void)rng_random(x.r);
  const int c = (int)rng_below(x.r, 6);
  const int t = c == 0 ? BA_MONITOR : (c == 1 ? BA_ANALYSE : (c == 2 ? BA_RESTORE : (c == 3 ? BA_REMOVE : (c == 4 ? BA_DECOY : BA_SLEEP))));
  a.type = (uint8_t)t;
  if (t == BA_MONITOR || t == BA_SLEEP) return a;
  int nh = 0;
  for (int i = 0; i < blue_nsub(b); ++i) { const int sn = blue_subnet_alloc(b, i); nh += 1 + s->n_users[sn] + s->n_servers[sn]; }
  int j = (int)rng_below(x.r, (uint32_t)nh);
  for (int i = 0; i < blue_nsub(b); ++i) {
    const int sn = blue_subnet_alloc(b, i), nu = s->n_users[sn], cnt = 1 + nu + s->n_servers[sn];
    if (j >= cnt) { j -= cnt; continue; }
    a.host = (uint8_t)(j == 0 ? h_make(sn, 0) : (j - 1 < nu ? h_make(sn, 1 + (j - 1)) : h_make(sn, 11 + (j - 1 - nu))));
    break;
  }
  return a;
}
CC4_HD void step_blue_submit(Ctx x, int b, int action_index) {
  EnvState* s = x.s;
  const bool builtin = action_index < 0 && (s->policy & BP_RANDOM_BIT);
  const int dur = action_index >= 0 ? (action_index >> BLUE_DUR_SHIFT) & 0xFF : 0;
  if (action_index >= 0) action_index &= BLUE_IDX_MASK;
  Act a = builtin ? blue_random_policy(x, b) : blue_decode(s, b, action_index);
  if (a.type == BA_RESTORE && !builtin) {
#if defined(__HIP_DEVICE_COMPILE__)
    atomicAdd(&s->n_restore, 1);
#else
    s->n_restore++;
#endif
  }
  a.ticks = (uint8_t)(dur ? dur : blue_duration(a.type));
  if (!s->blue[b].queue.busy) { s->blue[b].queue = a; s->blue[b].queue.busy = 1; }
}
CC4_HD void rng_policy_swap(Ctx x, bool back) {
  EnvState* s = x.s;
  (void)back;
  if (!s->rng_split) return;
  Rng* a = x.r; Rng* b = &x.c->rng2;
  { uint64_t t = a->s_hi; a->s_hi = b->s_hi; b->s_hi = t; }
  { uint64_t t = a->s_lo; a->s_lo = b->s_lo; b->s_lo = t; }
  { uint64_t t = a->inc_hi; a->inc_hi = b->inc_hi; b->inc_hi = t; }
  { uint64_t t = a->inc_lo; a->inc_lo = b->inc_lo; b->inc_lo = t; }
  { uint32_t t = a->has32; a->has32 = b->has32; b->has32 = t; }
  { uint32_t t = a->u32; a->u32 = b->u32; b->u32 = t; }
  { uint32_t t = a->ndraw; a->ndraw = b->ndraw; b->ndraw = t; }
}
CC4_HD void step_green_policy(Ctx x, int g, const uint32_t* pre = nullptr) {
  if (x.ext && x.ext[NRED + g].type != XA_NONE) {
    const ExtAct& ea = x.ext[NRED + g];
    int t = ea.type;
    if ((t == XG_ACCESS || t == XG_LOCAL) && !(ea.flags & XF_SKIP_VALID)) {
      const EnvState* s = x.s;
      const int own = h_subnet(s->green_host[g]);
      int ph = step_phase_of(s->step_count, s->phase_len[0], s->phase_len[1], s->phase_len[2]);
      if (ph < s->phase) ph = s->phase;
      if (((s->policy & GP_SLEEP_BIT) && !(s->policy & GP_OPEN_BIT)) || ea.host != s->green_host[g] || (t == XG_ACCESS && (ea.sid & ~green_allowed_mask(ph, own)))) t = XG_INVALID;
    }
    x.w->green_act[g] = (uint8_t)(t == XG_ACCESS ? 0 : (t == XG_LOCAL ? 1 : (t == XG_INVALID ? 3 : 2)));
    return;
  }
  if (x.s->policy & GP_SLEEP_BIT) { x.w->green_act[g] = 2; return; }
  rng_set_stream(x.r, ST_GREEN_POL + (uint32_t)g);
  if (pre) rng_preload(x.r, pre);
  x.w->green_act[g] = (uint8_t)rng_below(x.r, 3);
}
CC4_HD void step_red_observe(Ctx x, int r) {
  EnvState* s = x.s;
  RedAgent& A = s->red[r];
  const int pol = s->policy & 3;
  if (!A.h.active || pol == RP_RANDOM || pol == RP_SLEEP) return;
  if (x.ext && x.ext[r].type != XA_NONE) return;
  RedHdr H = A.h;
  fsm_observe(x, r, H);
  A.h = H;
}
CC4_HD bool rsc_draws(const EnvState* s, int r) {
  const RedAgent& A = s->red[r];
  if (!A.h.active || A.h.nsess == 0) return false;
  return rsw_id(rs_at(s, A, 0)) != 0 && rsw_id(rs_at(s, A, A.h.nsess - 1)) != 0 && rs_find_id(s, A, 0) < 0;
}
CC4_HD int step_red_policy_tick(Ctx x, int r, bool observed = false, const uint32_t* pre = nullptr) {
  EnvState* s = x.s;
  RedAgent& A = s->red[r];
  CC4_FT0(x, r);
  RedHdr H = A.h;
  Act a; a.type = RA_SLEEP; a.host = 0; a.arg = 0; a.ticks = 1; a.sid = 0; a.busy = 0;
  rng_set_stream(x.r, ST_RED_POL + (uint32_t)r);
  if (pre) rng_preload(x.r, pre);
  CC4_FT(x, r, 0);
  const ExtAct* ea = (x.ext && x.ext[r].type != XA_NONE) ? &x.ext[r] : nullptr;
  if (ea) {
    a.type = (uint8_t)ea->type; a.host = ea->host; a.arg = ea->arg; a.sid = ea->sid;
    a.ticks = (uint8_t)(ea->ticks ? ea->ticks : red_duration(a.type));
    if (!(ea->flags & XF_SKIP_VALID)) red_validate(x, r, H, a);
    if (a.type < RA_SLEEP && (ea->flags & (XF_RATE0 | XF_RATE1))) a.busy = (uint16_t)((ea->flags & XF_RATE0 ? AQ_RATE0 : 0) | (ea->flags & XF_RATE1 ? AQ_RATE1 : 0));
  }
  else if (H.active && (s->policy & 3) == RP_RANDOM) { a = random_red_get_action(x, r, H); red_validate(x, r, H, a); }
  else if (H.active && (s->policy & 3) != RP_SLEEP) { a = fsm_get_action(x, r, H, observed); CC4_AT0(x); red_validate(x, r, H, a); CC4_AT(x, 7); }
  CC4_FT(x, r, 1);
  if (!H.queue.busy) {
    H.queue = a; H.queue.busy = (uint16_t)(AQ_BUSY | a.busy);
    if (x.ext && (a.busy & (AQ_RATE0 | AQ_RATE1))) { x.c->xrate[r][0] = ea->rate0; x.c->xrate[r][1] = ea->rate1; }
  }
  H.nobs = 0; H.obs_success = 0; H.obs_act_type = RA_NONE; H.new_sess_host = 0xFF; H.rsc_listed = 0;
  for (int w = 0; w < 5; ++w) { A.obs_has[0][w] = 0; A.obs_has[1][w] = 0; }
  Act q = H.queue, ex;
  q.ticks--;
  if (q.ticks < 1) { ex = q; q.busy = 0; }
  else {
    ex.type = RA_SLEEP; ex.host = 0; ex.arg = 0; ex.ticks = 0; ex.sid = 0; ex.busy = 0;
    H.obs_success = T_IN_PROGRESS; H.obs_act_type = RA_NONE; H.obs_act_host = 0; H.obs_act_arg = 0;
  }
  H.queue = q;
  H.exec_type = ex.type; H.exec_host = ex.host;
  int dropped = 0;
  CC4_FT(x, r, 2);
  if (ex.type <= RA_WITHDRAW && rs_find_id(s, A, ex.sid, H.nsess) < 0) { ex.type = RA_NONE; dropped = 1; }
  CC4_FT(x, r, 3);
  s->rexec[r] = ex;
  A.h = H;
  CC4_FT(x, r, 4);
  return dropped;
}
CC4_HD void step_blue_exec(Ctx x, bool shuffle_done = false) {
  EnvState* s = x.s;
  if (!shuffle_done) {
    CC4_TICK(x, 3);
    if (x.r->mode == 0) rng_shuffle_consume(x.r, s->n_actions);
    CC4_TICK(x, 4);
  }
  for (int b = 0; b < NBLUE; ++b) if (s->bexec[b].type == BA_BLOCK || s->bexec[b].type == BA_ALLOW) blue_execute(x, b, s->bexec[b]);
  for (int b = 0; b < NBLUE; ++b)
    if (!(s->bexec[b].type == BA_BLOCK || s->bexec[b].type == BA_ALLOW)) {
      rng_set_stream(x.r, ST_BLUE_EXE + (uint32_t)b);
      blue_execute(x, b, s->bexec[b]);
    }
  CC4_TICK(x, 5);
}
CC4_HD void step_blue_exec_agent(Ctx x, int b, const uint32_t* pre = nullptr) {
  rng_set_stream(x.r, ST_BLUE_EXE + (uint32_t)b);
  if (pre) rng_preload(x.r, pre);
  blue_execute(x, b, x.s->bexec[b]);
}
CC4_HD bool blue_exec_independent(const EnvState* s) {
  if (s->npend) return false;
  for (int b = 0; b < NBLUE; ++b) if (s->bexec[b].type == BA_MONITOR) return false;
  return true;
}
CC4_HD void step_tick_blue(Ctx x, int b) {
  EnvState* s = x.s;
  Act& q = s->blue[b].queue;
  q.ticks--;
  if (q.ticks < 1) { s->bexec[b] = q; q.busy = 0; }
  else { Act z; z.type = BA_SLEEP; z.host = 0; z.arg = 0; z.ticks = 0; z.sid = 0; z.busy = 0; s->bexec[b] = z; }
}
CC4_HD int step_green_exec(Ctx x, int g, const uint32_t* pre = nullptr) {
  EnvState* s = x.s;
  int gh = s->green_host[g];
  int own = h_subnet(gh);
  rng_set_stream(x.r, ST_GREEN_EXE + (uint32_t)g);
  if (pre) rng_preload(x.r, pre);
  const int act = x.w->green_act[g];
  if (act >= 2) return 0;
  const uint64_t gp = x.gpre ? x.gpre[g] : green_prepare(x, g, act);
  const ExtAct* ea = (x.ext && x.ext[NRED + g].type != XA_NONE) ? &x.ext[NRED + g] : nullptr;
  if (act == 0) {
    const bool ok = green_access_service(x, gh, gp, (ea && (ea->flags & XF_RATE0)) ? ea->rate0 : 0.01);
    if (x.ext && !ok) bit_set_shared(x.c->gfail, g);
    return ok ? 0 : reward_table(s->phase, own, RW_ASF);
  }
  if (act == 1) {
    bool want_phish = false;
    bool ok = green_local_work(x, gh, gp, &want_phish, (ea && (ea->flags & XF_RATE0)) ? ea->rate0 : 0.01, (ea && (ea->flags & XF_RATE1)) ? ea->rate1 : 0.01);
    if (want_phish) bit_set_shared(x.w->phish_mask, g);
    if (x.ext && !ok) bit_set_shared(x.c->gfail, g);
    return ok ? 0 : reward_table(s->phase, own, RW_LWF);
  }
  return 0;
}
CC4_HD void step_phishing(Ctx x) {
  EnvState* s = x.s;
  for (int w = 0; w < 3; ++w) {
    uint32_t m = x.w->phish_mask[w];
    if (!m) continue;
    x.w->phish_mask[w] = 0;
    while (m) {
      int g = w * 32 + ctz32(m); m &= m - 1;
      rng_set_stream(x.r, ST_GREEN_PHISH + (uint32_t)g);
      phishing(x, s->green_host[g]);
    }
  }
}
CC4_HD uint32_t red_foreign_agents(const EnvState* s) {
  uint32_t foreign = 0;
  CC4_UNROLL for (int r = 0; r < NRED; ++r) {
    uint32_t acc = 0;
    CC4_UNROLL for (int w = 0; w < 5; ++w) acc |= s->red[r].live_hosts[w] & ~red_zone_hosts(r, w);
    if (acc) foreign |= 1u << r;
  }
  return foreign;
}
struct RedZoneTable { uint32_t out[40]; };
CC4_HD constexpr RedZoneTable red_zone_table() {
  RedZoneTable t{};
  for (int r = 0; r < NRED; ++r) for (int w = 0; w < 5; ++w) t.out[8 * w + r] = ~red_zone_hosts(r, w);
  return t;
}
CC4_HD constexpr uint32_t red_foreign_fold(uint64_t ballot) {
  uint32_t v = (uint32_t)ballot | (uint32_t)(ballot >> 32);
  v |= v >> 16; v |= v >> 8;
  return v & ((1u << NRED) - 1u);
}
static_assert(red_zone_table().out[8 * 2 + 5] == ~red_zone_hosts(5, 2) && red_zone_table().out[8 * 4 + 0] == ~red_zone_hosts(0, 4) && red_zone_table().out[6] == 0 &&
              red_foreign_fold(1ull << (8 * 4 + 3)) == 8u && red_foreign_fold((1ull << 5) | (1ull << 16)) == 0x21u && red_foreign_fold(0) == 0, "zone table and fold");
CC4_HD uint32_t red_foreign_lane(const EnvState* s, const uint32_t* zone_out, int lane) {
  const int r = lane & 7, w = lane >> 3;
  return (r < NRED && w < 5) ? s->red[r].live_hosts[w] & zone_out[lane] : 0u;
}
#if defined(__HIPCC__)
__device__ __forceinline__ uint32_t red_foreign_wave(const EnvState* s, int lane) {
  static constexpr RedZoneTable T = red_zone_table();
  return red_foreign_fold(__ballot(red_foreign_lane(s, T.out, lane) != 0));
}
#endif
CC4_HD void step_red_exec_agent(Ctx x, int r, const uint32_t* pre = nullptr) {
  EnvState* s = x.s;
  if (s->rexec[r].type == RA_NONE) return;
  rng_set_stream(x.r, ST_RED_EXE + (uint32_t)r);
  if (pre) rng_preload(x.r, pre);
  red_execute(x, r, s->rexec[r]);
}
CC4_HD uint32_t red_conflict_mask(const EnvState* s) {
  int ty[NRED], ho[NRED];
  CC4_UNROLL for (int a = 0; a < NRED; ++a) { uint64_t v; __builtin_memcpy(&v, &s->rexec[a], 8); ty[a] = (int)(v & 0xFF); ho[a] = (int)((v >> 8) & 0xFF); }
  uint32_t m = 0;
  bool withdraw = false;
  CC4_UNROLL for (int a = 0; a < NRED; ++a) {
    if (ty[a] == RA_WITHDRAW) withdraw = true;
    CC4_UNROLL for (int b = a + 1; b < NRED; ++b)
      if (ty[a] >= RA_AGGR && ty[a] <= RA_DEGRADE && ty[b] >= RA_AGGR && ty[b] <= RA_DEGRADE && ho[a] == ho[b]) m |= (1u << a) | (1u << b);
  }
  return withdraw ? (1u << NRED) - 1u : m;
}
CC4_HD uint32_t red_conflict_lane(const EnvState* s, int lane) {
  const int a = lane & 7, b = lane >> 3;
  if (a >= NRED || b >= NRED) return 0u;
  uint32_t va, vb;
  __builtin_memcpy(&va, &s->rexec[a], 4); __builtin_memcpy(&vb, &s->rexec[b], 4);
  const int ta = (int)(va & 0xFF), tb = (int)(vb & 0xFF);
  const bool same = a != b && ta >= RA_AGGR && ta <= RA_DEGRADE && tb >= RA_AGGR && tb <= RA_DEGRADE && ((va ^ vb) & 0xFF00u) == 0;
  return (same ? 1u : 0u) | (ta == RA_WITHDRAW ? 2u : 0u);
}
#if defined(__HIPCC__)
__device__ __forceinline__ uint32_t red_conflict_wave(const EnvState* s, int lane) {
  const uint32_t v = red_conflict_lane(s, lane);
  const uint32_t m = red_foreign_fold(__ballot((v & 1u) != 0));
  return __ballot((v & 2u) != 0) ? (1u << NRED) - 1u : m;
}
#endif
CC4_HD void step_red_exec(Ctx x) {
  rs_reserve(x);
  for (int r = 0; r < NRED; ++r) step_red_exec_agent(x, r);
  step_red_merge(x);
  CC4_TICK(x, 7);
}
CC4_HD void step_reassign(Ctx x, uint32_t foreign) {
  EnvState* s = x.s;
  if (foreign) red_reassign(x, foreign);
  else {
    int ns[NRED];
    CC4_UNROLL for (int r = 0; r < NRED; ++r) ns[r] = s->red[r].h.nsess;
    CC4_UNROLL for (int r = 0; r < NRED; ++r) s->red[r].h.active = (uint8_t)(ns[r] > 0);
  }
  CC4_TICK(x, 8);
}
CC4_HD void red_active_from_sessions(EnvState* s, int r) { s->red[r].h.active = (uint8_t)(s->red[r].h.nsess > 0); }
CC4_HD constexpr uint32_t monitor_watch_mask(int w) {
  uint32_t m = 0;
  for (int i = 0; i < 4; ++i) { const int h = 4 * w + i; if (h < MAXH && ((0xf444f3210ull >> (4 * (h / SLOTS))) & 0xF) != 0xF) m |= 0xFFu << (8 * i); }
  return m;
}
CC4_HD uint32_t monitor_roll4(uint32_t ev4, uint32_t watch) {
  static_assert(EV_OLD_CONN == EV_CUR_CONN << 2 && EV_OLD_PROC == EV_CUR_PROC << 2 && (EV_CUR_CONN | EV_CUR_PROC) == 3, "current bits move up two places");
  return (ev4 & ~watch) | (((ev4 & 0x03030303u) << 2) & watch);
}
CC4_HD uint8_t monitor_roll(int h, uint8_t ev) {
  if (blue_of_subnet(h_subnet(h)) < 0) return ev;
  uint8_t nev = 0;
  if (ev & EV_CUR_CONN) nev |= EV_OLD_CONN;
  if (ev & EV_CUR_PROC) nev |= EV_OLD_PROC;
  return nev;
}
CC4_HD int step_monitor_host(Ctx x, int h) {
  EnvState* s = x.s;
  if (!bit_get(s->exists, h)) return 0;
  const uint8_t ev = s->hev[h];
  const uint8_t nev = monitor_roll(h, ev);
  if (nev != ev) s->hev[h] = nev;
  return nev;
}
CC4_HD void step_monitor_pend(Ctx x) {
  EnvState* s = x.s;
  for (int i = 0; i < s->npend; ++i) {
    int b = blue_of_subnet(h_subnet((int)(s->pend[i] >> 16)));
    if (b < 0) continue;
    BlueAgent& A = s->blue[b];
    if (A.nsus >= cold_sus_cap(s->steps)) set_err(x, E_SUS_OVERFLOW); else { cold_sus(x.c, s->steps, b)[A.nsus++] = s->pend[i]; bit_set(A.sus_hosts, (int)(s->pend[i] >> 16)); }
  }
  s->npend = 0;
}
CC4_HD void step_rsc(Ctx x, int r) {
  if (!x.s->red[r].h.active) return;
  rng_set_stream(x.r, ST_RED_RSC + (uint32_t)r);
  red_session_check(x, r);
}
CC4_HD void step_messages(EnvState* s, const uint8_t* messages, int b) {
  static_assert(MSG_LEN == 8, "a message is one 8-byte word");
  uint64_t w = 0;
  if (messages) for (int i = 0; i < MSG_LEN; ++i) w |= (uint64_t)(messages[b * MSG_LEN + i] ? 1 : 0) << (8 * i);
  __builtin_memcpy(&s->msg[b][0], &w, 8);
}
CC4_HD int step_impact_term(const EnvState* s, int r) {
  const RedHdr& h = s->red[r].h;
  return (h.exec_type == RA_IMPACT && h.nsess > 0) ? reward_table(s->phase, h_subnet(h.exec_host), RW_RIA) : 0;
}
CC4_HD void step_end(Ctx x, const uint8_t* messages, bool copy_msgs = true, bool impact = true) {
  EnvState* s = x.s;
  s->step_count++;
  s->done = (uint8_t)(s->step_count >= s->steps - 1);
  int brm = s->brm;
  if (impact) {
    int et[NRED], ns[NRED];
    CC4_UNROLL for (int r = 0; r < NRED; ++r) { et[r] = s->red[r].h.exec_type; ns[r] = s->red[r].h.nsess; }
    CC4_UNROLL for (int r = 0; r < NRED; ++r)
      if (et[r] == RA_IMPACT && ns[r] > 0)
        brm += reward_table(s->phase, h_subnet(s->red[r].h.exec_host), RW_RIA);
  }
  s->action_cost = -(float)s->n_restore;
  s->reward = (float)brm + s->action_cost;
  if (x.ext) for (int g = 0; g < s->n_green; ++g) if (x.w->green_act[g] == 3) bit_set_shared(x.c->gfail, g);
  if (copy_msgs) for (int b = 0; b < NBLUE; ++b) step_messages(s, messages, b);
  s->brm = 0; s->n_restore = 0; s->n_actions = NBLUE + s->n_green + NRED;
  rng_park(&s->rng);
}

CC4_HD void env_step(Ctx x, const int32_t* actions, const uint8_t* messages ) {
  EnvState* s = x.s;
  CC4_TICK0(x);
  if (!step_phase(x)) return;
  rng_policy_swap(x, false);
  for (int b = 0; b < NBLUE; ++b) step_blue_submit(x, b, actions ? actions[b] : -1);
  CC4_TICK(x, 0);
  for (int g = 0; g < s->n_green; ++g) step_green_policy(x, g);
  CC4_TICK(x, 1);
  for (int r = 0; r < NRED; ++r) s->n_actions -= step_red_policy_tick(x, r);
  rng_policy_swap(x, true);
  CC4_TICK(x, 2);
  for (int b = 0; b < NBLUE; ++b) step_tick_blue(x, b);
  step_blue_exec(x);
  for (int g = 0; g < s->n_green; ++g) {
    s->brm += step_green_exec(x, g);
    if (bit_get(x.w->phish_mask, g)) { bit_clr(x.w->phish_mask, g); rng_set_stream(x.r, ST_GREEN_PHISH + (uint32_t)g); phishing(x, s->green_host[g]); }
  }
  CC4_TICK(x, 6);
  step_red_exec(x);
  {
    step_reassign(x, red_foreign_agents(s));
  }
  for (int h = 0; h < MAXH; ++h) step_monitor_host(x, h);
  step_monitor_pend(x);
  CC4_TICK(x, 9);
  for (int r = 0; r < NRED; ++r) step_rsc(x, r);
  CC4_TICK(x, 10);
  step_end(x, messages);
}

enum : int { SE_SET_PHASE = 0, SE_ADD_SERVICE = 1, SE_SET_RELIABILITY = 2, SE_CLEAR_HOST = 3, SE_DEPLOY_DECOY = 4, SE_ADD_RED_SESSION = 5,
             SE_BLOCK = 6, SE_SET_STEP = 7, SE_ADD_EVENT = 8, SE_SET_RED_ACTIVE = 9 };
inline int state_edit(Ctx x, int op, int a0, int a1, int a2) {
  EnvState* s = x.s;
  auto host_ok = [&](int h) { return h >= 0 && h < MAXH && bit_get(s->exists, h); };
  switch (op) {
    case SE_SET_PHASE:
      if (a0 < 0 || a0 > 2) return -1;
      s->phase = a0; s->obs_dirty = OD_PHASE;
      return 0;
    case SE_ADD_SERVICE: {
      if (!host_ok(a0) || a1 < K_SSHD || a1 > K_DEC_VSFTPD) return -1;
      HostDyn& d = x.hd[a0];
      const int nsv = hd_nsvc(d);
      int si = -1;
      for (int i = nsv - 1; i >= 0; --i) if (d.svcs[i].kind == a1) si = i;
      if (si < 0 && nsv >= MAXSV) return -1;
      const int pid = create_pid(x, a0);
      if (!add_proc(x, a0, pid, K_PLAIN, a2 ? PF_ROOT : 0)) return -1;
      if (si < 0) {
        si = nsv; hd_set_nsvc(d, nsv + 1);
        d.svcs[si].kind = (uint8_t)a1; d.svcs[si].pid = (uint16_t)pid; d.svcs[si].st = (uint8_t)(SV_ACTIVE | 5);
      }
      return pid;
    }
    case SE_SET_RELIABILITY: {
      if (!host_ok(a0) || a1 < 0 || a1 > 100 || a1 % 20) return -1;
      HostDyn& d = x.hd[a0];
      for (int i = 0; i < hd_nsvc(d); ++i) d.svcs[i].st = (uint8_t)((d.svcs[i].st & SV_ACTIVE) | (a1 / 20));
      return 0;
    }
    case SE_CLEAR_HOST: {
      if (!host_ok(a0)) return -1;
      HostDyn& d = x.hd[a0];
      d.nproc = 0; hd_set_nsvc(d, 0);
      for (int i = 0; i < PIN; ++i) { d.procs[i].pid = 0; d.procs[i].kind = 0; d.procs[i].flags = 0; }
      for (int i = 0; i < MAXSV; ++i) { d.svcs[i].pid = 0; d.svcs[i].kind = 0; d.svcs[i].st = 0; }
      return 0;
    }
    case SE_DEPLOY_DECOY: {
      if (!host_ok(a0) || a1 < K_DEC_APACHE || a1 > K_DEC_VSFTPD) return -1;
      HostDyn& d = x.hd[a0];
      const int used = proc_ports(x, a0);
      const int need = a1 == K_DEC_APACHE ? PB_80 : (a1 == K_DEC_TOMCAT ? PB_443 : (a1 == K_DEC_HARAKA ? PB_25 : 0));
      if (used & need) return 0;
      const int pid = create_pid(x, a0);
      if (!add_proc(x, a0, pid, a1, 0)) return -1;
      const int nsv = hd_nsvc(d);
      int si = -1;
      for (int i = nsv - 1; i >= 0; --i) if (d.svcs[i].kind == a1) si = i;
      if (si < 0) { if (nsv >= MAXSV) return -1; si = nsv; hd_set_nsvc(d, nsv + 1); }
      d.svcs[si].kind = (uint8_t)a1; d.svcs[si].pid = (uint16_t)pid; d.svcs[si].st = (uint8_t)(SV_ACTIVE | 5);
      return 1;
    }
    case SE_ADD_RED_SESSION: {
      if (a0 < 0 || a0 >= NRED || !host_ok(a1)) return -1;
      const int pid = create_pid(x, a1);
      if (!add_proc(x, a1, pid, (a2 & 4) ? K_SESS_RED : K_SHELL, (a2 & 1) ? PF_ROOT : 0)) return -1;
      const int idx = rs_add(x, a0, a1, pid, ((a2 & 1) ? RS_ROOT : 0) | ((a2 & 2) ? RS_CHILD : 0) | ((a2 & 4) ? RS_ABSTRACT : 0));
      if (idx < 0) return -1;
      return rsw_id(rs_at(s, s->red[a0], idx));
    }
    case SE_BLOCK:
      if (a0 < 0 || a0 >= NSUB - 1 || a1 < 0 || a1 >= NSUB - 1) return -1;
      if (a2) s->blocks[a0] |= (uint16_t)(1u << a1); else s->blocks[a0] &= (uint16_t)~(1u << a1);
      s->obs_dirty = OD_BLOCKS;
      return 0;
    case SE_SET_STEP:
      if (a0 < 0 || a0 >= s->steps) return -1;
      s->step_count = a0;
      return 0;
    case SE_ADD_EVENT: {
      if (!host_ok(a0) || a1 < 0 || a1 > 1) return -1;
      const int port = eph_port(x, a0);
      ev_or(x, a0, a1 ? EV_CUR_PROC : EV_CUR_CONN);
      return port;
    }
    case SE_SET_RED_ACTIVE:
      if (a0 < 0 || a0 >= NRED) return -1;
      s->red[a0].h.active = (uint8_t)(a1 != 0);
      return 0;
    default: return -1;
  }
}

enum : int { OBS_BLOCKS = 7, OBS_BLOCK_LEN = 59, OBS_MSG_BITS = (NBLUE - 1) * MSG_LEN,
             OBS_K_ONEHOT = 0, OBS_K_BLOCKED = 9, OBS_K_COMMS = 18, OBS_K_PROC = 27, OBS_K_CONN = 43,
             OBS_EV_PROC = EV_CUR_PROC | EV_OLD_PROC, OBS_EV_CONN = EV_CUR_CONN | EV_OLD_CONN };
static_assert(OBS_SHORT == 1 + OBS_BLOCK_LEN + OBS_MSG_BITS && OBS_LONG == 1 + 3 * OBS_BLOCK_LEN + OBS_MSG_BITS && OBS_K_CONN + ZONE_HOSTS == OBS_BLOCK_LEN, "segment and block lengths");
CC4_HD constexpr int obs_agent_base(int b) { return b < 4 ? b * OBS_SHORT : 4 * OBS_SHORT; }
CC4_HD constexpr int obs_agent_len(int b) { return b < 4 ? OBS_SHORT : OBS_LONG; }
CC4_HD constexpr int obs_block_agent(int sb) { return sb < 4 ? sb : 4; }
CC4_HD constexpr int obs_block_subnet(int sb) { return blue_subnet_sorted(obs_block_agent(sb), sb < 4 ? 0 : sb - 4); }
CC4_HD constexpr int obs_block_pos(int sb, int k) { return obs_agent_base(obs_block_agent(sb)) + 1 + OBS_BLOCK_LEN * (sb < 4 ? 0 : sb - 4) + k; }
CC4_HD constexpr int obs_zone_host(int sn, int hs) { return hs < MAX_SERVERS ? h_make(sn, 11 + hs) : h_make(sn, 1 + (hs - MAX_SERVERS)); }
CC4_HD constexpr int obs_msg_pos(int b, int m) { return obs_agent_base(b) + obs_agent_len(b) - OBS_MSG_BITS + m; }
CC4_HD constexpr int obs_msg_src(int b, int m) { return MSG_LEN * (m / MSG_LEN < b ? m / MSG_LEN : m / MSG_LEN + 1) + m % MSG_LEN; }
CC4_HD int obs_msg_value(const EnvState* s, int b, int m) { return (&s->msg[0][0])[obs_msg_src(b, m)]; }
CC4_HD int obs_block_value(const EnvState* s, int sn, int k) {
  if (k < OBS_K_BLOCKED) return sorted_subnet(k) == sn;
  if (k < OBS_K_COMMS) return (s->blocks[sn] >> sorted_subnet(k - OBS_K_BLOCKED)) & 1u;
  if (k < OBS_K_PROC) return !((comms_adjacent(s->phase, sn) >> sorted_subnet(k - OBS_K_COMMS)) & 1u);
  const int ev = s->hev[obs_zone_host(sn, k < OBS_K_CONN ? k - OBS_K_PROC : k - OBS_K_CONN)];
  return (ev & (k < OBS_K_CONN ? OBS_EV_PROC : OBS_EV_CONN)) != 0;
}
enum : int { OBS_PARTS = OBS_BLOCKS + NBLUE };
template <typename T>
CC4_HD void env_flat_obs_part(const EnvState* s, T* out, int part) {
  if (part < OBS_BLOCKS) {
    const int sn = obs_block_subnet(part), o = obs_block_pos(part, 0);
    uint32_t blk = s->blocks[sn];
    uint32_t adj = comms_adjacent(s->phase, sn);
    for (int k = 0; k < NSUB; ++k) {
      int ss = sorted_subnet(k);
      out[o + OBS_K_ONEHOT + k] = (T)(ss == sn);
      out[o + OBS_K_BLOCKED + k] = (T)((blk >> ss) & 1u);
      out[o + OBS_K_COMMS + k] = (T)(!((adj >> ss) & 1u));
    }
    for (int hs = 0; hs < ZONE_HOSTS; ++hs) {
      int h = obs_zone_host(sn, hs);
      int ev = bit_get(s->exists, h) ? s->hev[h] : 0;
      out[o + OBS_K_PROC + hs] = (T)((ev & OBS_EV_PROC) != 0);
      out[o + OBS_K_CONN + hs] = (T)((ev & OBS_EV_CONN) != 0);
    }
  } else {
    const int b = part - OBS_BLOCKS;
    out[obs_agent_base(b)] = (T)s->phase;
    for (int m = 0; m < OBS_MSG_BITS; ++m) out[obs_msg_pos(b, m)] = (T)obs_msg_value(s, b, m);
  }
}
template <typename T>
CC4_HD void env_flat_obs(const EnvState* s, T* out) {
  for (int p = 0; p < OBS_PARTS; ++p) env_flat_obs_part<T>(s, out, p);
}
CC4_HD int env_flat_obs_at(const EnvState* s, int idx) {
  const int b = idx < 4 * OBS_SHORT ? idx / OBS_SHORT : 4;
  const int j = idx - obs_agent_base(b), m0 = obs_agent_len(b) - OBS_MSG_BITS;
  if (j == 0) return s->phase;
  if (j >= m0) return obs_msg_value(s, b, j - m0);
  return obs_block_value(s, blue_subnet_sorted(b, (j - 1) / OBS_BLOCK_LEN), (j - 1) % OBS_BLOCK_LEN);
}
enum : int { OBS_FAST = 384 };
CC4_HD constexpr uint32_t obs_fast_entry(int v) {
  if (v >= 224) {
    const int w = v - 224, b = w >> 5, m = w & 31;
    return (uint32_t)obs_msg_pos(b, m) | ((uint32_t)(MAXH + obs_msg_src(b, m)) << 10) | (1u << 18);
  }
  const int sb = v >> 5, r = v & 31;
  const uint32_t mask = r < ZONE_HOSTS ? (uint32_t)OBS_EV_PROC : (uint32_t)OBS_EV_CONN;
  return (uint32_t)obs_block_pos(sb, OBS_K_PROC + r) | ((uint32_t)obs_zone_host(obs_block_subnet(sb), r & 15) << 10) | (mask << 18);
}
CC4_HD int obs_fast_value(uint32_t entry, const EnvState* s) {
  const int src = (int)((entry >> 10) & 0xFF);
  const uint32_t byte = src < MAXH ? s->hev[src] : (&s->msg[0][0])[src - MAXH];
  return (byte & (entry >> 18)) != 0 ? 1 : 0;
}
CC4_HD int env_flat_obs_sorted(const EnvState* s, int v, int* idx) {
  if (v < OBS_FAST) { const uint32_t e = obs_fast_entry(v); *idx = (int)(e & 0x3FFu); return obs_fast_value(e, s); }
  if (v < 573) {
    const int w = v - OBS_FAST, kind = w / 63, q = w % 63, sb = q / 9;
    const int k = (kind == 0 ? OBS_K_BLOCKED : (kind == 1 ? OBS_K_COMMS : OBS_K_ONEHOT)) + q % 9;
    *idx = obs_block_pos(sb, k);
    return obs_block_value(s, obs_block_subnet(sb), k);
  }
  *idx = obs_agent_base(v - 573);
  return s->phase;
}

}
```

### cage_challenge_4_amd/csrc/cc4_philox1_body.h

```cpp
#pragma once
#include "cc4_kernels.h"

__device__ __forceinline__ void philox1_autoreset(const StepArgs& a, const int e, const int lane, EnvState* s, HostDyn* const hd, EnvCold* const cold_e, StepWork& work) {
    reset_counter_mode_block<WAVE, true>(s, hd, cold_e, &work, lane, a.reset_ws + (size_t)e * RESET_WS_WORDS, 0, true, a.steps, a.policy, a.topo);
    if (lane == 0) { a.reward[e] = s->reward; a.done[e] = s->done; }
    __syncthreads();
}

#ifndef CC4_STOP_IN_FAST
#define CC4_STOP_IN_FAST 0
#endif
#define CC4_STOP_ON (LOG || CC4_STOP_IN_FAST)
#define CC4_STOP(n) do { if (CC4_STOP_ON && a.dbg_stop == (n)) return; } while (0)
template <bool LOG, bool PERSIST, bool HEAD = false>
__device__ __forceinline__ void philox1_body(StepArgs a, const int e, const uint32_t rand_t, const uint32_t item_k, const int lane,
                                             const bool first = true, const bool last = true) {
  static_assert(!HEAD || (PERSIST && !LOG), "the headline build is a fast persistent build");
  if constexpr (HEAD) { a.actions = nullptr; a.msgs = nullptr; a.act_sys = 0; a.obs8 = nullptr; }
  extern __shared__ uint4 lds[];
  __shared__ StepWork work;
  __shared__ unsigned long long prof_lds[LOG ? 16 : 1];
  if constexpr (!LOG) a.prof = nullptr;
  (void)item_k;
  EnvCold* const cold_e = cold_at(a.cold, (size_t)e, cold_row_bytes(a.steps));
  unsigned long long t_begin = a.prof ? clock64() : 0;
  const uint4* src = reinterpret_cast<const uint4*>(a.st + e);
  if (first) stage_in<HOT_VEC>(lds, src, lane);
  for (int i = lane; i < (int)(sizeof(StepWork) / 4); i += WAVE) reinterpret_cast<uint32_t*>(&work)[i] = 0;
  unsigned long long* prof = a.prof ? prof_lds : nullptr;
  if (prof && lane < 16) prof_lds[lane] = 0;
  __syncthreads();
  EnvState* s = reinterpret_cast<EnvState*>(lds);
  HostDyn* const hd = a.st[e].hd;
  if (prof && lane == 0) prof[11] += clock64() - t_begin;
  const bool do_reset = a.autoreset && s->done;
  const bool msgs_clean = PERSIST && item_k > 0 && !a.msgs;
  if (do_reset) {
    philox1_autoreset(a, e, lane, s, hd, cold_e, work);
  } else {
    const int st_now = s->step_count;
    const bool step_ok = step_phase_of(st_now, s->phase_len[0], s->phase_len[1], s->phase_len[2]) >= 0;
    if (lane == 0) {
      Ctx x{s, cold_e, &s->rng, hd, &work, prof};
      x.lg = (LOG && cold_e->evlog.enabled) ? &cold_e->evlog : nullptr;
      x.ext = (LOG && a.ext) ? a.ext + (size_t)e * EXT_PER_ENV : nullptr;
      CC4_TICK0(x);
      (void)step_phase(x, false);
    }
    if (step_ok) {
      CC4_STOP(1);
      const int ng = s->n_green;
      Rng rl;
      rng_fork(&rl, &s->rng, ST_RESET);
      rl.mode = 3;
      rng_begin_step(&rl, (uint32_t)st_now);
      EvLog* const lg = (LOG && cold_e->evlog.enabled) ? &cold_e->evlog : nullptr;
      const ExtAct* const xt = (LOG && a.ext) ? a.ext + (size_t)e * EXT_PER_ENV : nullptr;
      Ctx x0{s, cold_e, &rl, hd, &work, lane == 0 ? prof : nullptr};
      x0.lg = lg; x0.ext = xt;
      if (lane == 0) CC4_TICK(x0, 0);
      enum : int { BK_GPOL = 0, BK_GEXE = 16, BK_RPOL = 32, BK_REXE = 38, BK_BEXE = 44, BK_BRAND = 49, BK_END = 54 };
      uint32_t bank[4];
      {
        uint32_t st = 0;
        if (lane < BK_GEXE) st = ST_GREEN_POL + (uint32_t)(WAVE + lane - BK_GPOL);
        else if (lane < BK_REXE) st = ST_RED_POL + (uint32_t)(lane - BK_RPOL);
        else if (lane < BK_BEXE) st = ST_RED_EXE + (uint32_t)(lane - BK_REXE);
        else if (lane < BK_BRAND) st = ST_BLUE_EXE + (uint32_t)(lane - BK_BEXE);
        bank[0] = 0u; bank[1] = st; bank[2] = (uint32_t)rl.inc_lo; bank[3] = (uint32_t)rl.inc_hi;
        uint32_t k0 = (uint32_t)rl.s_lo, k1 = (uint32_t)(rl.s_lo >> 32);
        if ((HEAD || a.rand_out) && lane >= BK_BRAND && lane < BK_END) {
          const uint64_t key = a.rand_seed0 + (uint64_t)e;
          bank[0] = rand_t; bank[1] = (uint32_t)(lane - BK_BRAND); bank[2] = 0xB10Eu; bank[3] = 0u; k0 = (uint32_t)key; k1 = (uint32_t)(key >> 32);
        }
        philox4x32_10(bank, k0, k1, true);
      }
      auto bank_fetch = [&](int shift, uint32_t out[4]) {
        const int addr = ((lane + shift) & (WAVE - 1)) << 2;
#pragma unroll
        for (int k = 0; k < 4; ++k) out[k] = (uint32_t)__builtin_amdgcn_ds_bpermute(addr, (int)bank[k]);
      };
      CC4_STOP(2);
      const bool is_red = lane < NRED;
      unsigned long long* ap = (a.prof && is_red) ? a.prof + PROF_SLOTS * (size_t)e + 16 + 8 * lane : nullptr;
      Ctx xr{s, cold_e, &rl, hd, &work, nullptr, ap, lg};
      Ctx xg{s, cold_e, &rl, hd, &work, nullptr, nullptr, lg};
      xr.ext = xt; xg.ext = xt;
      uint32_t pre_rp[4];
      bank_fetch(BK_RPOL, pre_rp);
      const uint32_t brand = (uint32_t)__builtin_amdgcn_ds_bpermute(((lane + BK_BRAND - 8) & (WAVE - 1)) << 2, (int)bank[0]);
      if (is_red) {
        unsigned long long t0 = ap ? clock64() : 0;
        const int dropped = step_red_policy_tick(xr, lane, false, pre_rp);
        if (ap) ap[0] += clock64() - t0;
        if (dropped) atomicSub(&s->n_actions, 1);
      } else if (lane >= 8 && lane < 8 + NBLUE && !(CC4_STOP_ON && a.dbg_stop == 3)) {
        const int b = lane - 8;
        int32_t act = !a.actions ? -1 : a.act_sys ? __hip_atomic_load(a.actions + e * NBLUE + b, __ATOMIC_RELAXED, __HIP_MEMORY_SCOPE_SYSTEM) : a.actions[e * NBLUE + b];
        if (HEAD || a.rand_out) { act = (int32_t)(((uint64_t)brand * (uint32_t)(b == 4 ? ACT_LONG : ACT_SHORT)) >> 32); a.rand_out[e * NBLUE + b] = act; }
        step_blue_submit(xg, b, act);
        step_tick_blue(xg, b);
        if (!msgs_clean) step_messages(s, a.msgs ? a.msgs + e * NBLUE * MSG_LEN : nullptr, b);
      }
      if (!(CC4_STOP_ON && (a.dbg_stop == 3 || a.dbg_stop == 4))) {
        if (lane < ng) step_green_policy(xg, lane);
        if (lane + WAVE < ng) step_green_policy(xg, lane + WAVE, bank);
      }
      __syncthreads();
      CC4_TICK(x0, 2);
      CC4_STOP(3); CC4_STOP(4); CC4_STOP(5);
      {
        const bool indep = blue_exec_independent(s);
        if (lane == 0) CC4_TICK(x0, 3);
        uint32_t c[4];
        bank_fetch(BK_BEXE, c);
        Ctx xb = xg;
        if (!indep) xb.prof = x0.prof;
        const int rounds = indep ? 1 : 2 * NBLUE;
#pragma nounroll
        for (int i = 0; i < rounds; ++i) {
          int b = lane;
          bool go = lane < NBLUE;
          if (!indep) {
            b = i < NBLUE ? i : i - NBLUE;
            const int ty = s->bexec[b].type;
            go = lane == 0 && ((ty == BA_BLOCK || ty == BA_ALLOW) == (i < NBLUE));
          }
          if (go) {
            rng_set_stream(&rl, ST_BLUE_EXE + (uint32_t)b);
            if (indep) rng_preload(&rl, c);
            blue_execute(xb, b, s->bexec[b]);
          }
        }
        __syncthreads();
        if (lane == 0) CC4_TICK(x0, 5);
      }
      CC4_STOP(6);
      {
        int pen = 0;
        const uint32_t act0 = lane < ng ? work.green_act[lane] : 2u, act1 = lane + WAVE < ng ? work.green_act[lane + WAVE] : 2u;
        const unsigned long long m0 = __ballot(act0 < 2u), m1 = __ballot(act1 < 2u);
        const unsigned long long lt = (1ull << lane) - 1ull;
        const int n0 = __popcll(m0), nact = n0 + __popcll(m1);
        uint8_t* const glist = reinterpret_cast<uint8_t*>(work.scratch);
        static_assert(sizeof(work.scratch) >= MAXG, "the green list fits the scratch words");
        if (act0 < 2u) glist[__popcll(m0 & lt)] = (uint8_t)lane;
        if (act1 < 2u) glist[n0 + __popcll(m1 & lt)] = (uint8_t)(lane + WAVE);
        __syncthreads();
        for (int i = lane; i < nact; i += WAVE) {
          const int g = glist[i];
          uint32_t c[4]; rng_block(&rl, ST_GREEN_EXE + (uint32_t)g, 0, c);
          pen += step_green_exec(xg, g, c);
        }
        if (pen) atomicAdd(&s->brm, pen);
      }
      __syncthreads();
      CC4_TICK(x0, 6);
      CC4_STOP(7);
      {
        const bool phish = __ballot(lane < 3 && work.phish_mask[lane] != 0) != 0ull;
        const uint32_t exploit = (uint32_t)__ballot(is_red && s->rexec[lane].type == RA_EXPLOIT);
        if (phish) { if (lane == 0) step_phishing(x0); __syncthreads(); }
        if (lane == 0) CC4_TICK(x0, 1);
        if (is_red) work.rs_slot[lane] = (uint8_t)(exploit ? rs_reserve_lane(s, exploit, lane) : 0xFF);
      }
      __syncthreads();
      const uint32_t serial_red = red_conflict_wave(s, lane);
      if (lane == 0 && prof && serial_red) prof[4] += 1000000;
      CC4_STOP(8);
      uint32_t pre_re[4];
      bank_fetch(BK_REXE, pre_re);
      {
        uint32_t todo = serial_red;
        bool side = true;
#pragma nounroll
        for (;;) {
          int r = lane;
          bool go = is_red && !((serial_red >> lane) & 1u);
          Ctx xe = xr;
          if (!side) { r = __ffs((int)todo) - 1; todo &= todo - 1u; go = lane == 0; xe.prof = x0.prof; xe.aprof = nullptr; }
          RedPre pe;
          if (side) {
            const bool look = go && s->rexec[lane].type < RA_SLEEP;
            pe = rs_wave_query(s, lane, look ? (int)s->rexec[lane].sid : -1, look ? (int)s->rexec[lane].host : -1);
          }
          if (go) {
            unsigned long long t0 = xe.aprof ? clock64() : 0;
            if (s->rexec[r].type != RA_NONE) {
              rng_set_stream(&rl, ST_RED_EXE + (uint32_t)r);
              if (side) rng_preload(&rl, pre_re);
              red_execute(xe, r, s->rexec[r], pe);
            }
            if (xe.aprof) xe.aprof[1] += clock64() - t0;
          }
          __syncthreads();
          side = false;
          if (!todo) break;
        }
      }
      CC4_STOP(9);
      if (__ballot(is_red && work.pend_r[lane] != 0)) { if (lane == 0) step_red_merge(x0); }
      if (lane == 0) CC4_TICK(x0, 7);
      __syncthreads();
      {
        const uint32_t foreign = red_foreign_wave(s, lane);
        if (foreign) { if (lane == 0) red_reassign(x0, foreign); __syncthreads(); }
        else if (is_red) red_active_from_sessions(s, lane);
        if (lane == 0) CC4_TICK(x0, 8);
        if (is_red) { const int term = step_impact_term(s, lane); if (term) atomicAdd(&s->brm, term); }
      }
      CC4_STOP(10);
      monitor_roll_all(s, lane);
      __syncthreads();
      CC4_TICK(x0, 9);
      CC4_STOP(11);
      if (is_red) { unsigned long long t0 = ap ? clock64() : 0; step_rsc(xr, lane); if (ap) ap[2] += clock64() - t0; }
      if (lane == WAVE - 1) {
        step_monitor_pend(xg);
        step_end(xg, nullptr, false, false);
        a.reward[e] = s->reward; a.done[e] = s->done;
      }
      CC4_TICK(x0, 10);
    } else if (lane == 0) { a.reward[e] = s->reward; a.done[e] = s->done; }
  }
  __syncthreads();
  CC4_STOP(12);
  unsigned long long t_obs = a.prof ? clock64() : 0;
  {
    int32_t* o = a.obs + (size_t)e * OBS_TOTAL;
    const uint32_t dirty = (do_reset || (a.full_obs && (!PERSIST || item_k == 0))) ? (uint32_t)OD_ALL : (uint32_t)s->obs_dirty;
    encode_obs_fast<WAVE>(s, o, nullptr, false, lane, msgs_clean && !do_reset && dirty != (uint32_t)OD_ALL);
    encode_obs_slow(s, o, dirty, lane);
  }
  __syncthreads();
  CC4_STOP(13);
  if (lane == 0) a.err[e] = s->err;
  unsigned long long t_out = a.prof ? clock64() : 0;
  if (prof && lane == 0) prof[12] += t_out - t_obs;
  if (last) stage_out<HOT_VEC>(reinterpret_cast<uint4*>(a.st + e), lds, lane);
  if (a.obs8) {
    asm volatile("s_waitcnt vmcnt(0)" ::: "memory");
    pack_row_from_obs(a.obs8 + (size_t)e * OBS_PACKED, a.obs + (size_t)e * OBS_TOTAL, lane);
  }
  if (prof && lane == 0) { prof[13] += clock64() - t_out; prof[14] += clock64() - t_begin; }
  if (prof) { __syncthreads(); if (lane < 15) a.prof[PROF_SLOTS * (size_t)e + lane] += prof_lds[lane]; }
}
```

### cage_challenge_4_amd/csrc/cc4_state.h

```cpp
#pragma once
#include <stdint.h>
#include <stddef.h>
#include "cc4_rng.h"

namespace cc4 {

enum : int {
  NSUB = 9, SLOTS = 17, MAXH = 137, H_INTERNET = 136,
  MAX_USERS = 10, MAX_SERVERS = 6, ZONE_HOSTS = 16,
  MAXG = 80,
  NBLUE = 5, NRED = 6,
  PIN = 8,
  MAXSV = 7,
  MAX_RS = 64,
  RS_POOL = 192,
  MAX_KS = 96,
  MAX_OBS = 32,
  MAX_PEND = 8,
  EPH_WORDS = 340,
  OBS_SHORT = 92, OBS_LONG = 210, OBS_TOTAL = 4 * 92 + 210,
  ACT_SHORT = 82, ACT_LONG = 242, MASK_TOTAL = 4 * 82 + 242,
  MSG_LEN = 8,
};

enum : int { S_RZA = 0, S_OZA = 1, S_RZB = 2, S_OZB = 3, S_CON = 4, S_PUB = 5, S_ADM = 6, S_OFF = 7, S_INT = 8 };

enum : int {
  K_SSHD = 0, K_OT = 1, K_APACHE = 2, K_MYSQL = 3, K_SMTP = 4,
  K_DEC_APACHE = 5, K_DEC_TOMCAT = 6, K_DEC_HARAKA = 7, K_DEC_VSFTPD = 8,
  K_SESS_BLUE = 9, K_SESS_GREEN = 10, K_SESS_RED = 11,
  K_SHELL = 12,
  K_PLAIN = 13,
};
enum : int { PB_22 = 1, PB_80 = 2, PB_3390 = 4, PB_25 = 8, PB_1 = 16, PB_443 = 32, PB_HAS = 128 };

enum : uint32_t {
  E_PROC_OVERFLOW = 1u << 0, E_RSESS_OVERFLOW = 1u << 1, E_KS_OVERFLOW = 1u << 2, E_KB_OVERFLOW = 1u << 3 ,
  E_SUS_OVERFLOW = 1u << 4, E_OBS_OVERFLOW = 1u << 5, E_PEND_OVERFLOW = 1u << 6,
  E_STEP_PAST_END = 1u << 7,
  E_UNREACHABLE = 1u << 8,
  E_BLUE_GREEN_SESSION_KILLED = 1u << 10,
  E_FSM_NO_HOST = 1u << 11,
};

struct alignas(4) Proc { uint16_t pid; uint8_t kind; uint8_t flags; };
struct alignas(4) Svc  { uint16_t pid; uint8_t kind; uint8_t st; };
enum : int { PF_ROOT = 1, SV_ACTIVE = 0x80 };

enum : int { EV_CUR_CONN = 1, EV_CUR_PROC = 2, EV_OLD_CONN = 4, EV_OLD_PROC = 8 };
enum : int { OD_BLOCKS = 1, OD_PHASE = 2, OD_ALL = 7 };

enum : int { HF_CMD = 1, HF_ESC = 2, HF_ESC_LAST = 4 };
struct alignas(16) HostDyn {
  Proc procs[PIN];
  Svc svcs[MAXSV];
  uint16_t nproc;
  uint8_t gtmp;
  uint8_t nsf;
};
static_assert(sizeof(HostDyn) == 64, "HostDyn is four 16-byte vectors");
struct alignas(8) HostStatic {
  Proc procs[8];
  Svc svcs[5];
  uint8_t nproc, nsvc, exists, ip_octet;
};

enum : int { RS_ABSTRACT = 1, RS_ROOT = 2, RS_ORIG = 4, RS_CHILD = 8 };
struct alignas(8) RSess { uint16_t id; uint16_t pid; uint8_t host; uint8_t flags; uint8_t pad[2]; };

enum : int { FS_K = 0, FS_KD = 1, FS_S = 2, FS_SD = 3, FS_U = 4, FS_UD = 5, FS_R = 6, FS_RD = 7, FS_F = 8, FS_NONE = 0xFF };
enum : int { RA_DRS = 0, RA_AGGR = 1, RA_STEALTH = 2, RA_DECEPTION = 3, RA_EXPLOIT = 4, RA_PRIVESC = 5, RA_IMPACT = 6,
             RA_DEGRADE = 7, RA_WITHDRAW = 8, RA_SLEEP = 9, RA_INVALID = 10, RA_NONE = 11 };
enum : int { BA_SLEEP = 0, BA_MONITOR = 1, BA_ANALYSE = 2, BA_REMOVE = 3, BA_RESTORE = 4, BA_DECOY = 5, BA_BLOCK = 6, BA_ALLOW = 7 };
enum : int { RP_FSM = 0, RP_SLEEP = 1, RP_DISCOVERY = 2, RP_RANDOM = 3, GP_SLEEP_BIT = 0x10,
             GP_OPEN_BIT = 0x40 ,
             BP_RANDOM_BIT = 0x20  };
enum : int { T_TRUE = 1, T_UNKNOWN = 2, T_FALSE = 3, T_IN_PROGRESS = 4 };

struct alignas(8) Act { uint8_t type; uint8_t host; uint8_t arg; uint8_t ticks; uint16_t sid; uint16_t busy; };
enum : int { AQ_BUSY = 1, AQ_RATE0 = 2, AQ_RATE1 = 4 };

enum : int { XA_NONE = -1, XG_ACCESS = 0, XG_LOCAL = 1, XG_SLEEP = 2, XG_INVALID = 3 };
enum : int { XF_RATE0 = 1, XF_RATE1 = 2, XF_SKIP_VALID = 4 };
struct alignas(8) ExtAct { int8_t type; uint8_t host; uint8_t arg; uint8_t ticks; uint16_t sid; uint8_t flags; uint8_t pad; double rate0, rate1; };
static_assert(sizeof(ExtAct) == 24, "ExtAct mirrors cc4_agent_action (include/cc4.h)");
enum : int { EXT_PER_ENV = NRED + MAXG };
enum : int { BLUE_DUR_SHIFT = 20, BLUE_IDX_MASK = (1 << BLUE_DUR_SHIFT) - 1 };

enum : int { OE_KEY_IP = 1, OE_SESS = 2, OE_IFACE = 4, OE_SYSHN = 8 };
struct alignas(2) ObsEnt { uint8_t host; uint8_t flags; };

struct alignas(16) RedHdr {
  Act queue;
  uint16_t as_subnet;
  uint16_t fsm_step;
  uint16_t new_sess_id;
  uint8_t nsess, nknown, fsm_n, nobs;
  uint8_t nlive;
  uint8_t active;
  uint8_t obs_success;
  uint8_t obs_act_type, obs_act_host, obs_act_arg;
  uint8_t exec_type, exec_host;
  uint8_t new_sess_host;
  uint8_t start_host;
  uint8_t rsc_dirty;
  uint8_t rsc_listed;
  uint8_t fsm_dirty;
  uint8_t pad[1];
};
static_assert(sizeof(RedHdr) == 32, "RedHdr is two 16-byte vectors");
struct alignas(16) RedAgent {
  alignas(8) uint8_t sord[MAX_RS];
  uint32_t known_bm[8];
  uint8_t fsm_order[MAXH];
  uint8_t fsm_st4[(MAXH + 1) / 2];
  uint32_t fsm_hn[5];
  uint32_t as_ip[5];
  uint32_t as_hn[5];
  ObsEnt obs[MAX_OBS];
  uint32_t obs_has[2][5];
  uint32_t fsm_known[5];
  uint32_t fsm_ur[5];
  uint32_t fsm_nodrs[5];
  uint32_t live_hosts[5];
  RedHdr h;
};

struct alignas(8) BlueAgent {
  uint32_t sus_hosts[5];
  uint32_t pad2;
  Act queue;
  uint16_t nsus;
  uint8_t parent_host;
  uint8_t last_ok;
};

struct alignas(64) EnvState {
  Rng rng;
  int32_t step_count, steps, phase;
  int32_t phase_len[3];
  uint32_t err;
  float reward;
  uint8_t done, rng_mode, n_green;
  uint8_t policy;
  uint8_t rng_split;
  uint8_t obs_dirty;
  uint8_t assign;
  uint8_t pad0;
  uint16_t blocks[NSUB];
  uint8_t cidr_octet[NSUB];
  uint8_t n_users[NSUB];
  alignas(8) uint8_t n_servers[NSUB];
  uint8_t green_host[MAXG];
  uint32_t pend[MAX_PEND];
  uint8_t npend, pad1[3];
  uint32_t exists[5];
  uint32_t red_hosts[5];
  uint32_t spool_used[RS_POOL / 32];
  uint8_t msg[NBLUE][MSG_LEN];
  Act bexec[NBLUE];
  Act rexec[NRED];
  int32_t brm;
  float action_cost;
  int32_t n_actions;
  int32_t n_restore;
  BlueAgent blue[NBLUE];
  RSess spool[RS_POOL];
  RedAgent red[NRED];
  alignas(4) uint8_t hev[MAXH + 39];
  alignas(64) HostDyn hd[MAXH];
};
static_assert(offsetof(EnvState, hd) % 64 == 0 && sizeof(EnvState) % 64 == 0 && sizeof(EnvState) == offsetof(EnvState, hd) + sizeof(HostDyn) * MAXH, "the host table closes the row; row and table are whole cache lines");

enum : int { PA_SET = 0x80, PA_BITS = 3 | GP_SLEEP_BIT | BP_RANDOM_BIT, PA_KEEP = -1 , PA_DEFAULT = -2  };
static_assert(offsetof(EnvState, assign) % 4 == 2, "EnvState.assign is byte 2 of its word");
enum : uint32_t { PA_WORD = (uint32_t)(offsetof(EnvState, assign) / 4), PA_WORD_MASK = 0x00FF0000u };
CC4_HD int policy_at_reset(const EnvState* s, int handle_policy) { return (s->assign & PA_SET) ? (s->assign & PA_BITS) : handle_policy; }
CC4_HD bool row_assign(EnvState* s, int red, int green, int blue) {
  if (red < PA_DEFAULT || red > 3 || green < PA_DEFAULT || green > 1 || blue < PA_DEFAULT || blue > 1) return false;
  const bool any_default = red == PA_DEFAULT || green == PA_DEFAULT || blue == PA_DEFAULT, any_class = red >= 0 || green >= 0 || blue >= 0;
  if (any_default && any_class) return false;
  if (any_default) { s->assign = 0; return true; }
  if (!any_class) return true;
  int b = ((s->assign & PA_SET) ? s->assign : s->policy) & PA_BITS;
  if (red >= 0) b = (b & ~3) | red;
  if (green >= 0) b = (b & ~GP_SLEEP_BIT) | (green ? GP_SLEEP_BIT : 0);
  if (blue >= 0) b = (b & ~BP_RANDOM_BIT) | (blue ? BP_RANDOM_BIT : 0);
  s->assign = (uint8_t)(PA_SET | b);
  return true;
}
CC4_HD void row_policies(const EnvState* s, int8_t* live, int8_t* assigned) {
  if (live) { live[0] = (int8_t)(s->policy & 3); live[1] = (int8_t)((s->policy & GP_SLEEP_BIT) ? ((s->policy & GP_OPEN_BIT) ? 2 : 1) : 0); live[2] = (int8_t)((s->policy & BP_RANDOM_BIT) ? 1 : 0); }
  if (assigned) {
    const int a = s->assign;
    const bool set = (a & PA_SET) != 0;
    assigned[0] = (int8_t)(set ? (a & 3) : PA_DEFAULT); assigned[1] = (int8_t)(set ? ((a & GP_SLEEP_BIT) ? 1 : 0) : PA_DEFAULT); assigned[2] = (int8_t)(set ? ((a & BP_RANDOM_BIT) ? 1 : 0) : PA_DEFAULT);
  }
}

struct alignas(4) StepWork {
  uint32_t scratch[64];
  uint32_t phish_mask[4];
  uint32_t pend_r[NRED];
  uint8_t rs_slot[NRED + 2];
  uint8_t green_act[MAXG];
  uint32_t hdirty[5];
};

enum : int { MAX_EV = 160 };
struct alignas(4) EvRec {
  uint8_t host;
  uint8_t kind;
  uint8_t laddr;
  uint8_t raddr;
  uint16_t lport;
  uint16_t rport;
  uint16_t pid;
  uint8_t rep;
  uint8_t order;
};
struct alignas(16) EvLog { uint32_t n, step, enabled, pad; EvRec rec[MAX_EV]; };

struct alignas(16) EnvCold {
  HostStatic hs[MAXH];
  uint8_t hs_pad[8];
  uint32_t eph[MAXH][EPH_WORDS];
  EvLog evlog;
  uint8_t kports[RS_POOL][MAXH + 7];
  double xrate[NRED][2];
  uint32_t gfail[4];
  uint16_t known_sid[NRED][MAX_KS];
  Rng rng2;
};
static_assert(sizeof(EnvCold) % 16 == 0, "the containers behind the fixed part start 16-byte aligned");
CC4_HD int cold_sus_cap(int steps) { const int c = (3 * steps) / 2 + 18; return (c + 15) & ~15; }
CC4_HD int cold_povf_cap(int steps) { const int c = steps / 2 + 126; return (c + 7) & ~7; }
CC4_HD size_t cold_row_bytes(int steps) {
  return sizeof(EnvCold) + 4u * ((size_t)NBLUE * (size_t)cold_sus_cap(steps) + (size_t)MAXH * (size_t)cold_povf_cap(steps));
}
CC4_HD EnvCold* cold_at(EnvCold* base, size_t e, size_t row_bytes) { return reinterpret_cast<EnvCold*>(reinterpret_cast<char*>(base) + e * row_bytes); }
CC4_HD const EnvCold* cold_at(const EnvCold* base, size_t e, size_t row_bytes) { return reinterpret_cast<const EnvCold*>(reinterpret_cast<const char*>(base) + e * row_bytes); }
CC4_HD uint32_t* cold_sus(EnvCold* c, int steps, int b) { return reinterpret_cast<uint32_t*>(c + 1) + (size_t)b * (size_t)cold_sus_cap(steps); }
CC4_HD const uint32_t* cold_sus(const EnvCold* c, int steps, int b) { return reinterpret_cast<const uint32_t*>(c + 1) + (size_t)b * (size_t)cold_sus_cap(steps); }
CC4_HD uint32_t* cold_povf(EnvCold* c, int steps, int h) {
  return reinterpret_cast<uint32_t*>(c + 1) + (size_t)NBLUE * (size_t)cold_sus_cap(steps) + (size_t)h * (size_t)cold_povf_cap(steps);
}
CC4_HD const uint32_t* cold_povf(const EnvCold* c, int steps, int h) {
  return reinterpret_cast<const uint32_t*>(c + 1) + (size_t)NBLUE * (size_t)cold_sus_cap(steps) + (size_t)h * (size_t)cold_povf_cap(steps);
}

enum : int { CS_HS = 0, CS_EVHDR = 1, CS_EVREC = 2, CS_TAIL = 3, CS_EPH = 4, CS_FIXED = 5, COLD_SPANS = CS_FIXED + RS_POOL + NBLUE + MAXH };
struct ColdSpan { uint32_t off, bytes; };
CC4_HD ColdSpan cold_live_span(const EnvState* s, int steps, int rng_mode, int evlog_on, uint32_t ev_n, int k) {
  constexpr uint32_t o_ev = (uint32_t)offsetof(EnvCold, evlog), o_tail = (uint32_t)offsetof(EnvCold, xrate);
  static_assert(offsetof(EnvCold, eph) % 16 == 0 && offsetof(EnvCold, evlog) % 16 == 0 && offsetof(EnvCold, kports) % 16 == 0 &&
                offsetof(EnvCold, xrate) % 16 == 0 && (MAXH + 7) % 16 == 0 && offsetof(EvLog, rec) == 16, "live spans start 16-byte aligned");
  static_assert(offsetof(EnvCold, gfail) > offsetof(EnvCold, xrate) && offsetof(EnvCold, known_sid) > offsetof(EnvCold, gfail) &&
                offsetof(EnvCold, rng2) > offsetof(EnvCold, known_sid), "xrate .. rng2 close the fixed part");
  if (k == CS_HS) return {0u, (uint32_t)offsetof(EnvCold, eph)};
  if (k == CS_EVHDR) return {o_ev, 16u};
  if (k == CS_EVREC) return {o_ev + 16u, evlog_on ? (uint32_t)sizeof(EvRec) * (ev_n < (uint32_t)MAX_EV ? ev_n : (uint32_t)MAX_EV) : 0u};
  if (k == CS_TAIL) return {o_tail, (uint32_t)sizeof(EnvCold) - o_tail};
  if (k == CS_EPH) return {(uint32_t)offsetof(EnvCold, eph), rng_mode == 0 ? (uint32_t)sizeof(EnvCold::eph) : 0u};
  k -= CS_FIXED;
  if (k < RS_POOL) {
    const bool used = (s->spool_used[k >> 5] >> (k & 31)) & 1u;
    return {(uint32_t)offsetof(EnvCold, kports) + (uint32_t)k * (uint32_t)(MAXH + 7), used ? (uint32_t)(MAXH + 7) : 0u};
  }
  k -= RS_POOL;
  const uint32_t scap = (uint32_t)cold_sus_cap(steps), pcap = (uint32_t)cold_povf_cap(steps);
  if (k < NBLUE) {
    const uint32_t ns = s->blue[k].nsus;
    return {(uint32_t)sizeof(EnvCold) + 4u * scap * (uint32_t)k, 4u * (ns < scap ? ns : scap)};
  }
  k -= NBLUE;
  const uint32_t np = s->hd[k].nproc, nx = np > (uint32_t)PIN ? np - (uint32_t)PIN : 0u;
  return {(uint32_t)sizeof(EnvCold) + 4u * (scap * (uint32_t)NBLUE + pcap * (uint32_t)k), 4u * (nx < pcap ? nx : pcap)};
}

}
```

Baseline: 1.610 billion.

## Hold red agent header and actions as packed 32/64-bit words in registers

Replaces byte-wise accesses to the red agent header (RedHdr) and action structs with a register-resident array of eight 32-bit words plus a 64-bit action word. Fields are read and written through compile-time shift/mask accessors, and the header is loaded and stored as 16-byte vectors. The aim is to cut scattered byte loads and stores and register shuffling in the red policy, observe and execute paths. Static asserts pin the field layout, at the cost of heavier code and a risk that the compiler produces worse bit-manipulation sequences.

```diff
diff --git a/cage_challenge_4_amd/csrc/cc4_engine.h b/cage_challenge_4_amd/csrc/cc4_engine.h
--- a/cage_challenge_4_amd/csrc/cc4_engine.h
+++ b/cage_challenge_4_amd/csrc/cc4_engine.h
@@ -564,7 +564,8 @@
 CC4_HD void obs_first(Ctx x, int r, int success, int atype, int ahost, int aarg) {
   RedAgent& a = x.s->red[r];
   if (a.h.obs_success != 0) return;
-  a.h.obs_success = (uint8_t)success; a.h.obs_act_type = (uint8_t)atype; a.h.obs_act_host = (uint8_t)ahost; a.h.obs_act_arg = (uint8_t)aarg;
+  const uint32_t v = hdr_obs_word((uint32_t)success, (uint32_t)atype, (uint32_t)ahost, (uint32_t)aarg);
+  __builtin_memcpy(__builtin_assume_aligned(reinterpret_cast<char*>(&a.h) + offsetof(RedHdr, obs_success), 4), &v, 4);
 }
 
 CC4_HD int path_to_root(int h, uint8_t* out) {
@@ -1521,18 +1522,19 @@
   }
   red_result(x, r, a, T_TRUE);
 }
-CC4_HD void red_session_check(Ctx x, int r) {
+CC4_HD void red_session_check(Ctx x, int r, RedHdrW& H) {
   EnvState* s = x.s;
   RedAgent& A = s->red[r];
-  obs_first(x, r, T_TRUE, RA_NONE, 0, 0);
+  if (hget<RH_OBS_SUCCESS>(H) == 0) H.w[hdr_field(RH_OBS_SUCCESS).word] = hdr_obs_word(T_TRUE, RA_NONE, 0, 0);
   if (A.h.nsess == 0) return;
   if (rsw_id(rs_at(s, A, 0)) != 0 && rsw_id(rs_at(s, A, A.h.nsess - 1)) != 0 && rs_find_id(s, A, 0) < 0) {
     int c = (int)rng_below(x.r, (uint32_t)A.h.nsess);
     rs_move_to_end(s, A, c, 0);
+    hset<RH_RSC_DIRTY>(H, 1);
     for (int i = 0; i < A.h.nsess; ++i) s->spool[A.sord[i]].flags &= (uint8_t)~RS_CHILD;
   }
-  A.h.rsc_listed = 1;
-  if (!A.h.rsc_dirty) return;
+  hset<RH_RSC_LISTED>(H, 1);
+  if (!hget<RH_RSC_DIRTY>(H)) return;
   const B5 live = b5_load(A.live_hosts);
   { const B5 ip = b5_load(A.as_ip), hn = b5_load(A.as_hn); b5_store(A.as_ip, b5_or(ip, live)); b5_store(A.as_hn, b5_or(hn, live)); }
   {
@@ -1570,7 +1572,7 @@
         if (rsw_host(w) == h && (rsw_flags(w) & RS_ABSTRACT)) as_know_sid(x, r, rsw_id(w));
       }
     }
-  A.h.rsc_dirty = 0;
+  hset<RH_RSC_DIRTY>(H, 0);
 }
 CC4_HD void red_withdraw(Ctx x, int r, const Act& a, RedPre pre = RedPre()) {
   EnvState* s = x.s;
@@ -1601,7 +1603,8 @@
   }
   red_result(x, r, a, ok);
 }
-CC4_HD void red_execute(Ctx x, int r, const Act& a, RedPre pre = RedPre()) {
+CC4_HD void red_execute(Ctx x, int r, ActW w, RedPre pre = RedPre()) {
+  const Act a = act_unpack(w);
   switch (a.type) {
     case RA_DRS: red_drs(x, r, a, pre); break;
     case RA_AGGR: red_scan(x, r, a, (x.ext && (a.busy & AQ_RATE0)) ? x.c->xrate[r][0] : 0.75, pre); break;
@@ -1648,7 +1651,7 @@
   if ((st & 1) || st == FS_F) bit_set(A.fsm_nodrs, h); else bit_clr(A.fsm_nodrs, h);
   fsm_put(A, h, st);
 }
-CC4_HD void fsm_apply(Ctx x, int r, RedHdr& H, int h, int act, bool success) {
+CC4_HD void fsm_apply(Ctx x, int r, RedHdrW& H, int h, int act, bool success) {
   RedAgent& A = x.s->red[r];
   int cur = fsm_get(A, h);
   if (cur == FS_NONE) return;
@@ -1658,19 +1661,21 @@
   if (nx != cur) fsm_set_state(A, h, nx);
   if (nx == FS_F && cur != FS_F) {
     int n = 0;
-    for (int i = 0; i < H.fsm_n; ++i) if (A.fsm_order[i] != h) A.fsm_order[n++] = A.fsm_order[i];
-    H.fsm_n = (uint8_t)n;
-  }
-}
-CC4_HD void fsm_observe(Ctx x, int r, RedHdr& H) {
+    const int fn = (int)hget<RH_FSM_N>(H);
+    for (int i = 0; i < fn; ++i) if (A.fsm_order[i] != h) A.fsm_order[n++] = A.fsm_order[i];
+    hset<RH_FSM_N>(H, (uint32_t)n);
+  }
+}
+CC4_HD void fsm_observe(Ctx x, int r, RedHdrW& H) {
   RedAgent& A = x.s->red[r];
   CC4_AT0(x);
-  if (H.obs_success == T_IN_PROGRESS && H.nobs == 0 && H.rsc_listed && !H.fsm_dirty) return;
-  if (H.obs_act_type <= RA_WITHDRAW && H.obs_success != T_IN_PROGRESS && H.obs_success != 0) {
-    bool ok = H.obs_success == T_TRUE;
-    int t = H.obs_act_type;
+  const uint32_t obs_success = hget<RH_OBS_SUCCESS>(H), nobs = hget<RH_NOBS>(H);
+  if (obs_success == T_IN_PROGRESS && nobs == 0 && hget<RH_RSC_LISTED>(H) && !hget<RH_FSM_DIRTY>(H)) return;
+  if (hget<RH_OBS_ACT_TYPE>(H) <= RA_WITHDRAW && obs_success != T_IN_PROGRESS && obs_success != 0) {
+    bool ok = obs_success == T_TRUE;
+    int t = (int)hget<RH_OBS_ACT_TYPE>(H);
     if (t == RA_DRS) {
-      const int lo = H.obs_act_arg * SLOTS, hi = lo + SLOTS - 1;
+      const int lo = (int)hget<RH_OBS_ACT_ARG>(H) * SLOTS, hi = lo + SLOTS - 1;
       for (int w = lo >> 5; w <= (hi >> 5) && w < 5; ++w) {
         uint32_t m = A.fsm_known[w];
         if (ok) m &= ~A.fsm_nodrs[w];
@@ -1680,15 +1685,15 @@
         while (m) { int b = ctz32(m); m &= m - 1; fsm_apply(x, r, H, w * 32 + b, t, ok); }
       }
     } else if (t == RA_PRIVESC || t == RA_IMPACT || t == RA_DEGRADE) {
-      int h = H.obs_act_host;
+      int h = (int)hget<RH_OBS_ACT_HOST>(H);
       if (bit_get(A.fsm_known, h) && bit_get(A.fsm_hn, h)) fsm_apply(x, r, H, h, t, ok);
     } else {
-      fsm_apply(x, r, H, H.obs_act_host, t, ok);
+      fsm_apply(x, r, H, (int)hget<RH_OBS_ACT_HOST>(H), t, ok);
     }
   }
   CC4_AT(x, 3);
   B5 seen = b5_zero();
-  for (int i = 0; i < H.nobs; ++i) {
+  for (int i = 0; i < (int)nobs; ++i) {
     int h = A.obs[i].host; int f = A.obs[i].flags;
     if (f & OE_SESS) b5_set(seen, h);
     bool hn = !(f & OE_KEY_IP) || (f & OE_SYSHN);
@@ -1698,26 +1703,26 @@
       continue;
     }
     if (!bit_get(A.fsm_known, h)) {
-      fsm_set_state(A, h, H.fsm_step == 0 ? FS_U : FS_K);
-      A.fsm_order[H.fsm_n++] = (uint8_t)h;
+      fsm_set_state(A, h, hget<RH_FSM_STEP>(H) == 0 ? FS_U : FS_K);
+      A.fsm_order[hget<RH_FSM_N>(H)] = (uint8_t)h; hinc<RH_FSM_N>(H);
       bit_set(A.fsm_known, h);
     }
     if (hn) bit_set(A.fsm_hn, h);
   }
   CC4_AT(x, 4);
-  if (H.rsc_listed) {
+  if (hget<RH_RSC_LISTED>(H)) {
     const B5 live = b5_load(A.live_hosts), known = b5_load(A.fsm_known), hn = b5_load(A.fsm_hn);
     seen = b5_or(seen, live);
     if (b5_any(b5_andn(live, known)))
-      for (int i = 0; i < H.nsess; ++i) {
+      for (int i = 0, ns = (int)hget<RH_NSESS>(H); i < ns; ++i) {
         int h = rsw_host(rs_at(x.s, A, i));
         if (bit_get(A.fsm_known, h)) continue;
-        fsm_set_state(A, h, H.fsm_step == 0 ? FS_U : FS_K);
-        A.fsm_order[H.fsm_n++] = (uint8_t)h;
+        fsm_set_state(A, h, hget<RH_FSM_STEP>(H) == 0 ? FS_U : FS_K);
+        A.fsm_order[hget<RH_FSM_N>(H)] = (uint8_t)h; hinc<RH_FSM_N>(H);
         bit_set(A.fsm_known, h);
       }
     b5_store(A.fsm_hn, b5_or(hn, live));
-    H.fsm_dirty = 0;
+    hset<RH_FSM_DIRTY>(H, 0);
   }
   CC4_AT(x, 5);
   {
@@ -1730,10 +1735,11 @@
   }
   CC4_AT(x, 6);
 }
-CC4_HD int fsm_choose_host_discovery(Ctx x, int r, RedHdr& H) {
+CC4_HD int fsm_choose_host_discovery(Ctx x, int r, const RedHdrW& H) {
   RedAgent& A = x.s->red[r];
+  const int fsm_n = (int)hget<RH_FSM_N>(H);
   uint32_t order = 0; int nst = 0; uint32_t seen = 0;
-  for (int i = 0; i < H.fsm_n && nst < 8; ++i) {
+  for (int i = 0; i < fsm_n && nst < 8; ++i) {
     int st = fsm_get(A, A.fsm_order[i]);
     if (!((seen >> st) & 1u)) { seen |= 1u << st; order |= (uint32_t)st << (4 * nst); nst++; }
   }
@@ -1757,7 +1763,7 @@
     chosen_state = (order >> (4 * (int)rng_below(x.r, (uint32_t)nst))) & 0xF;
   }
   int n_all = 0, n_srv = 0;
-  for (int i = 0; i < H.fsm_n; ++i) {
+  for (int i = 0; i < fsm_n; ++i) {
     int h = A.fsm_order[i];
     if (fsm_get(A, h) != chosen_state) continue;
     n_all++;
@@ -1770,7 +1776,7 @@
   }
   int cnt = want_srv < 0 ? n_all : (want_srv ? n_srv : n_all - n_srv);
   int c = (int)rng_below(x.r, (uint32_t)cnt);
-  for (int i = 0; i < H.fsm_n; ++i) {
+  for (int i = 0; i < fsm_n; ++i) {
     int h = A.fsm_order[i];
     if (fsm_get(A, h) != chosen_state) continue;
     bool srv = h_is_server(h) && bit_get(A.fsm_hn, h);
@@ -1822,16 +1828,16 @@
 static constexpr FsmPkTab fsm_pk_tab = make_fsm_pk_tab();
 #endif
 CC4_HD uint32_t fsm_pk(bool discovery, int host_state) { return fsm_pk_tab.v[fsm_pk_index(discovery, host_state)]; }
-CC4_HD Act fsm_get_action(Ctx x, int r, RedHdr& H, bool observed = false) {
+CC4_HD ActW fsm_get_action(Ctx x, int r, RedHdrW& H, bool observed = false) {
   EnvState* s = x.s;
   RedAgent& A = s->red[r];
-  Act out; out.type = RA_SLEEP; out.host = 0; out.arg = 0; out.ticks = 1; out.sid = 0; out.busy = 0;
+  constexpr ActW sleep = act_word(RA_SLEEP, 0, 0, 1, 0, 0);
   CC4_FT0(x, r);
   if (!observed) fsm_observe(x, r, H);
   CC4_FT(x, r, 5);
-  if (H.obs_success == T_IN_PROGRESS) { H.fsm_step++; return out; }
-  int n = H.fsm_n;
-  if (n == 0) { set_err(x, E_FSM_NO_HOST); H.fsm_step++; return out; }
+  if (hget<RH_OBS_SUCCESS>(H) == T_IN_PROGRESS) { hinc<RH_FSM_STEP>(H); return sleep; }
+  int n = (int)hget<RH_FSM_N>(H);
+  if (n == 0) { set_err(x, E_FSM_NO_HOST); hinc<RH_FSM_STEP>(H); return sleep; }
   const bool discovery = (s->policy & 3) == RP_DISCOVERY;
   int host;
   if (!discovery) host = A.fsm_order[rng_below(x.r, (uint32_t)n)];
@@ -1842,28 +1848,29 @@
   int k = 0;
   for (int i = 0; i < 4; ++i) if ((int)((pk >> (16 + 4 * i)) & 0xF) <= fl) k++;
   int t = (int)((pk >> (4 * k)) & 0xF);
-  out.type = (uint8_t)t; out.host = (uint8_t)host;
+  uint32_t arg = 0, sid = 0;
   bool bad = false;
   if (t == RA_DRS) {
-    uint32_t known = H.as_subnet;
-    if (known == 0) bad = true; else out.arg = (uint8_t)nth_bit(known, (int)rng_below(x.r, (uint32_t)popc32(known)));
+    uint32_t known = hget<RH_AS_SUBNET>(H);
+    if (known == 0) bad = true; else arg = (uint32_t)nth_bit(known, (int)rng_below(x.r, (uint32_t)popc32(known)));
   }
   if ((t == RA_PRIVESC || t == RA_IMPACT || t == RA_DEGRADE) && !bit_get(A.fsm_hn, host)) bad = true;
   if (!bad) {
-    if (H.nknown == 0) bad = true; else out.sid = x.c->known_sid[r][rng_below(x.r, (uint32_t)H.nknown)];
-  }
-  if (bad) { set_err(x, E_UNREACHABLE); out.type = RA_SLEEP; }
-  out.ticks = (uint8_t)red_duration(out.type);
-  H.fsm_step++;
+    const uint32_t nknown = hget<RH_NKNOWN>(H);
+    if (nknown == 0) bad = true; else sid = x.c->known_sid[r][rng_below(x.r, nknown)];
+  }
+  if (bad) { set_err(x, E_UNREACHABLE); t = RA_SLEEP; }
+  hinc<RH_FSM_STEP>(H);
   CC4_FT(x, r, 7);
-  return out;
-}
-CC4_HD Act random_red_get_action(Ctx x, int r, RedHdr& H) {
+  return act_word((uint32_t)t, (uint32_t)host, arg, (uint32_t)red_duration(t), sid, 0);
+}
+CC4_HD ActW random_red_get_action(Ctx x, int r, RedHdrW& H) {
   RedAgent& A = x.s->red[r];
   Act out; out.type = RA_SLEEP; out.host = 0; out.arg = 0; out.ticks = 1; out.sid = 0; out.busy = 0;
   const int nip = popc32(A.as_ip[0]) + popc32(A.as_ip[1]) + popc32(A.as_ip[2]) + popc32(A.as_ip[3]) + popc32(A.as_ip[4]);
   const int nhn = popc32(A.as_hn[0]) + popc32(A.as_hn[1]) + popc32(A.as_hn[2]) + popc32(A.as_hn[3]) + popc32(A.as_hn[4]);
-  const int nsub = popc32(H.as_subnet), nsid = H.nknown;
+  const uint32_t as_subnet = hget<RH_AS_SUBNET>(H);
+  const int nsub = popc32(as_subnet), nsid = (int)hget<RH_NKNOWN>(H);
   const uint8_t types[10] = {RA_DRS, RA_AGGR, RA_STEALTH, RA_EXPLOIT, RA_PRIVESC, RA_DEGRADE, RA_DECEPTION, RA_IMPACT, RA_WITHDRAW, RA_SLEEP};
   uint32_t valid = 0;
   for (int c = 0; c < 10; ++c) {
@@ -1881,7 +1888,7 @@
   auto pick_hn = [&]() { return nth_set(A.as_hn, 5, (int)rng_below(x.r, (uint32_t)nhn)); };
   out.type = (uint8_t)t;
   switch (t) {
-    case RA_DRS: out.arg = (uint8_t)nth_bit(H.as_subnet, (int)rng_below(x.r, (uint32_t)nsub)); out.sid = (uint16_t)pick_sid(); break;
+    case RA_DRS: out.arg = (uint8_t)nth_bit(as_subnet, (int)rng_below(x.r, (uint32_t)nsub)); out.sid = (uint16_t)pick_sid(); break;
     case RA_AGGR: case RA_STEALTH: case RA_DECEPTION: out.sid = (uint16_t)pick_sid(); out.host = (uint8_t)pick_ip(); break;
     case RA_EXPLOIT: out.host = (uint8_t)pick_ip(); out.sid = (uint16_t)pick_sid(); break;
     case RA_PRIVESC: case RA_DEGRADE: case RA_IMPACT: out.host = (uint8_t)pick_hn(); out.sid = (uint16_t)pick_sid(); break;
@@ -1889,19 +1896,21 @@
     default: break;
   }
   out.ticks = (uint8_t)red_duration(out.type);
-  H.fsm_step++;
-  return out;
-}
-CC4_HD void red_validate(Ctx x, int r, const RedHdr& H, Act& a) {
+  hinc<RH_FSM_STEP>(H);
+  return act_pack(out);
+}
+CC4_HD ActW red_validate(Ctx x, int r, const RedHdrW& H, ActW a) {
   RedAgent& A = x.s->red[r];
-  if (a.type >= RA_SLEEP) return;
+  const int type = (int)aget<AW_TYPE>(a), host = (int)aget<AW_HOST>(a), arg = (int)aget<AW_ARG>(a);
+  if (type >= RA_SLEEP) return a;
   bool ok = true;
-  if (!sid_known(A, x.c->known_sid[r], a.sid, H.nknown)) ok = false;
-  if (a.type == RA_DRS) { if (!((H.as_subnet >> a.arg) & 1u)) ok = false; }
-  else if (a.type == RA_PRIVESC || a.type == RA_IMPACT || a.type == RA_DEGRADE) { if (!bit_get(A.as_hn, a.host)) ok = false; }
-  else if (a.type == RA_WITHDRAW) { if (!bit_get(A.as_ip, a.host) || !bit_get(A.as_hn, a.arg)) ok = false; }
-  else { if (!bit_get(A.as_ip, a.host)) ok = false; }
-  if (!ok) { a.type = RA_INVALID; a.ticks = 1; }
+  if (!sid_known(A, x.c->known_sid[r], (int)aget<AW_SID>(a), (int)hget<RH_NKNOWN>(H))) ok = false;
+  if (type == RA_DRS) { if (!((hget<RH_AS_SUBNET>(H) >> arg) & 1u)) ok = false; }
+  else if (type == RA_PRIVESC || type == RA_IMPACT || type == RA_DEGRADE) { if (!bit_get(A.as_hn, host)) ok = false; }
+  else if (type == RA_WITHDRAW) { if (!bit_get(A.as_ip, host) || !bit_get(A.as_hn, arg)) ok = false; }
+  else { if (!bit_get(A.as_ip, host)) ok = false; }
+  if (!ok) a = aset<AW_TICKS>(aset<AW_TYPE>(a, RA_INVALID), 1);
+  return a;
 }
 
 CC4_HD constexpr uint32_t red_zone_hosts(int r, int w) {
@@ -2028,7 +2037,7 @@
 #endif
   }
   a.ticks = (uint8_t)(dur ? dur : blue_duration(a.type));
-  if (!s->blue[b].queue.busy) { s->blue[b].queue = a; s->blue[b].queue.busy = 1; }
+  if (!aget<AW_BUSY>(act_load(&s->blue[b].queue))) act_store(&s->blue[b].queue, aset<AW_BUSY>(act_pack(a), 1));
 }
 CC4_HD void rng_policy_swap(Ctx x, bool back) {
   EnvState* s = x.s;
@@ -2068,9 +2077,9 @@
   const int pol = s->policy & 3;
   if (!A.h.active || pol == RP_RANDOM || pol == RP_SLEEP) return;
   if (x.ext && x.ext[r].type != XA_NONE) return;
-  RedHdr H = A.h;
+  RedHdrW H = hdr_load(&A.h);
   fsm_observe(x, r, H);
-  A.h = H;
+  hdr_store(&A.h, H, HDR_HI);
 }
 CC4_HD bool rsc_draws(const EnvState* s, int r) {
   const RedAgent& A = s->red[r];
@@ -2081,42 +2090,41 @@
   EnvState* s = x.s;
   RedAgent& A = s->red[r];
   CC4_FT0(x, r);
-  RedHdr H = A.h;
-  Act a; a.type = RA_SLEEP; a.host = 0; a.arg = 0; a.ticks = 1; a.sid = 0; a.busy = 0;
+  RedHdrW H = hdr_load(&A.h);
+  ActW a = act_word(RA_SLEEP, 0, 0, 1, 0, 0);
   rng_set_stream(x.r, ST_RED_POL + (uint32_t)r);
   if (pre) rng_preload(x.r, pre);
   CC4_FT(x, r, 0);
   const ExtAct* ea = (x.ext && x.ext[r].type != XA_NONE) ? &x.ext[r] : nullptr;
   if (ea) {
-    a.type = (uint8_t)ea->type; a.host = ea->host; a.arg = ea->arg; a.sid = ea->sid;
-    a.ticks = (uint8_t)(ea->ticks ? ea->ticks : red_duration(a.type));
-    if (!(ea->flags & XF_SKIP_VALID)) red_validate(x, r, H, a);
-    if (a.type < RA_SLEEP && (ea->flags & (XF_RATE0 | XF_RATE1))) a.busy = (uint16_t)((ea->flags & XF_RATE0 ? AQ_RATE0 : 0) | (ea->flags & XF_RATE1 ? AQ_RATE1 : 0));
-  }
-  else if (H.active && (s->policy & 3) == RP_RANDOM) { a = random_red_get_action(x, r, H); red_validate(x, r, H, a); }
-  else if (H.active && (s->policy & 3) != RP_SLEEP) { a = fsm_get_action(x, r, H, observed); CC4_AT0(x); red_validate(x, r, H, a); CC4_AT(x, 7); }
+    const uint32_t type = (uint8_t)ea->type;
+    a = act_word(type, ea->host, ea->arg, (uint32_t)(ea->ticks ? ea->ticks : red_duration((int)type)), ea->sid, 0);
+    if (!(ea->flags & XF_SKIP_VALID)) a = red_validate(x, r, H, a);
+    if (aget<AW_TYPE>(a) < RA_SLEEP && (ea->flags & (XF_RATE0 | XF_RATE1))) a = aset<AW_BUSY>(a, (uint32_t)((ea->flags & XF_RATE0 ? AQ_RATE0 : 0) | (ea->flags & XF_RATE1 ? AQ_RATE1 : 0)));
+  }
+  else if (hget<RH_ACTIVE>(H) && (s->policy & 3) == RP_RANDOM) { a = random_red_get_action(x, r, H); a = red_validate(x, r, H, a); }
+  else if (hget<RH_ACTIVE>(H) && (s->policy & 3) != RP_SLEEP) { a = fsm_get_action(x, r, H, observed); CC4_AT0(x); a = red_validate(x, r, H, a); CC4_AT(x, 7); }
   CC4_FT(x, r, 1);
-  if (!H.queue.busy) {
-    H.queue = a; H.queue.busy = (uint16_t)(AQ_BUSY | a.busy);
-    if (x.ext && (a.busy & (AQ_RATE0 | AQ_RATE1))) { x.c->xrate[r][0] = ea->rate0; x.c->xrate[r][1] = ea->rate1; }
-  }
-  H.nobs = 0; H.obs_success = 0; H.obs_act_type = RA_NONE; H.new_sess_host = 0xFF; H.rsc_listed = 0;
+  if (!hget<RH_Q_BUSY>(H)) {
+    hdr_set_queue(H, a | (ActW)AQ_BUSY << (32 + act_field(AW_BUSY).shift));
+    if (x.ext && (aget<AW_BUSY>(a) & (AQ_RATE0 | AQ_RATE1))) { x.c->xrate[r][0] = ea->rate0; x.c->xrate[r][1] = ea->rate1; }
+  }
+  hdr_tick_reset(H);
   for (int w = 0; w < 5; ++w) { A.obs_has[0][w] = 0; A.obs_has[1][w] = 0; }
-  Act q = H.queue, ex;
-  q.ticks--;
-  if (q.ticks < 1) { ex = q; q.busy = 0; }
+  ActW q = act_tick(hdr_queue(H)), ex;
+  if (aget<AW_TICKS>(q) < 1) { ex = q; q = aset<AW_BUSY>(q, 0); }
   else {
-    ex.type = RA_SLEEP; ex.host = 0; ex.arg = 0; ex.ticks = 0; ex.sid = 0; ex.busy = 0;
-    H.obs_success = T_IN_PROGRESS; H.obs_act_type = RA_NONE; H.obs_act_host = 0; H.obs_act_arg = 0;
-  }
-  H.queue = q;
-  H.exec_type = ex.type; H.exec_host = ex.host;
+    ex = act_word(RA_SLEEP, 0, 0, 0, 0, 0);
+    H.w[hdr_field(RH_OBS_SUCCESS).word] = hdr_obs_word(T_IN_PROGRESS, RA_NONE, 0, 0);
+  }
+  hdr_set_queue(H, q);
+  hset<RH_EXEC_TYPE>(H, aget<AW_TYPE>(ex)); hset<RH_EXEC_HOST>(H, aget<AW_HOST>(ex));
   int dropped = 0;
   CC4_FT(x, r, 2);
-  if (ex.type <= RA_WITHDRAW && rs_find_id(s, A, ex.sid, H.nsess) < 0) { ex.type = RA_NONE; dropped = 1; }
+  if (aget<AW_TYPE>(ex) <= RA_WITHDRAW && rs_find_id(s, A, (int)aget<AW_SID>(ex), (int)hget<RH_NSESS>(H)) < 0) { ex = aset<AW_TYPE>(ex, RA_NONE); dropped = 1; }
   CC4_FT(x, r, 3);
-  s->rexec[r] = ex;
-  A.h = H;
+  act_store(&s->rexec[r], ex);
+  hdr_store(&A.h, H);
   CC4_FT(x, r, 4);
   return dropped;
 }
@@ -2147,10 +2155,10 @@
 }
 CC4_HD void step_tick_blue(Ctx x, int b) {
   EnvState* s = x.s;
-  Act& q = s->blue[b].queue;
-  q.ticks--;
-  if (q.ticks < 1) { s->bexec[b] = q; q.busy = 0; }
-  else { Act z; z.type = BA_SLEEP; z.host = 0; z.arg = 0; z.ticks = 0; z.sid = 0; z.busy = 0; s->bexec[b] = z; }
+  ActW q = act_tick(act_load(&s->blue[b].queue));
+  if (aget<AW_TICKS>(q) < 1) { act_store(&s->bexec[b], q); q = aset<AW_BUSY>(q, 0); }
+  else act_store(&s->bexec[b], act_word(BA_SLEEP, 0, 0, 0, 0, 0));
+  act_store(&s->blue[b].queue, q);
 }
 CC4_HD int step_green_exec(Ctx x, int g, const uint32_t* pre = nullptr) {
   EnvState* s = x.s;
@@ -2223,10 +2231,11 @@
 #endif
 CC4_HD void step_red_exec_agent(Ctx x, int r, const uint32_t* pre = nullptr) {
   EnvState* s = x.s;
-  if (s->rexec[r].type == RA_NONE) return;
+  const ActW w = act_load(&s->rexec[r]);
+  if (aget<AW_TYPE>(w) == RA_NONE) return;
   rng_set_stream(x.r, ST_RED_EXE + (uint32_t)r);
   if (pre) rng_preload(x.r, pre);
-  red_execute(x, r, s->rexec[r]);
+  red_execute(x, r, w);
 }
 CC4_HD uint32_t red_conflict_mask(const EnvState* s) {
   int ty[NRED], ho[NRED];
@@ -2308,9 +2317,12 @@
   s->npend = 0;
 }
 CC4_HD void step_rsc(Ctx x, int r) {
-  if (!x.s->red[r].h.active) return;
+  RedHdr* const h = &x.s->red[r].h;
+  RedHdrW H = hdr_load(h, HDR_HI);
+  if (!hget<RH_ACTIVE>(H)) return;
   rng_set_stream(x.r, ST_RED_RSC + (uint32_t)r);
-  red_session_check(x, r);
+  red_session_check(x, r, H);
+  hdr_store(h, H, HDR_HI);
 }
 CC4_HD void step_messages(EnvState* s, const uint8_t* messages, int b) {
   static_assert(MSG_LEN == 8, "a message is one 8-byte word");
@@ -2320,7 +2332,9 @@
 }
 CC4_HD int step_impact_term(const EnvState* s, int r) {
   const RedHdr& h = s->red[r].h;
-  return (h.exec_type == RA_IMPACT && h.nsess > 0) ? reward_table(s->phase, h_subnet(h.exec_host), RW_RIA) : 0;
+  static_assert(hdr_field(RH_EXEC_TYPE).word == hdr_field(RH_EXEC_HOST).word, "exec_type and exec_host are one word");
+  const uint32_t w = hdr_word(&h, hdr_field(RH_EXEC_TYPE).word);
+  return (wget<RH_EXEC_TYPE>(w) == RA_IMPACT && h.nsess > 0) ? reward_table(s->phase, h_subnet((int)wget<RH_EXEC_HOST>(w)), RW_RIA) : 0;
 }
 CC4_HD void step_end(Ctx x, const uint8_t* messages, bool copy_msgs = true, bool impact = true) {
   EnvState* s = x.s;
diff --git a/cage_challenge_4_amd/csrc/cc4_philox1_body.h b/cage_challenge_4_amd/csrc/cc4_philox1_body.h
--- a/cage_challenge_4_amd/csrc/cc4_philox1_body.h
+++ b/cage_challenge_4_amd/csrc/cc4_philox1_body.h
@@ -180,16 +180,17 @@
           Ctx xe = xr;
           if (!side) { r = __ffs((int)todo) - 1; todo &= todo - 1u; go = lane == 0; xe.prof = x0.prof; xe.aprof = nullptr; }
           RedPre pe;
+          const ActW rex = go ? act_load(&s->rexec[r]) : act_word(RA_NONE, 0, 0, 0, 0, 0);
           if (side) {
-            const bool look = go && s->rexec[lane].type < RA_SLEEP;
-            pe = rs_wave_query(s, lane, look ? (int)s->rexec[lane].sid : -1, look ? (int)s->rexec[lane].host : -1);
+            const bool look = aget<AW_TYPE>(rex) < RA_SLEEP;
+            pe = rs_wave_query(s, lane, look ? (int)aget<AW_SID>(rex) : -1, look ? (int)aget<AW_HOST>(rex) : -1);
           }
           if (go) {
             unsigned long long t0 = xe.aprof ? clock64() : 0;
-            if (s->rexec[r].type != RA_NONE) {
+            if (aget<AW_TYPE>(rex) != RA_NONE) {
               rng_set_stream(&rl, ST_RED_EXE + (uint32_t)r);
               if (side) rng_preload(&rl, pre_re);
-              red_execute(xe, r, s->rexec[r], pe);
+              red_execute(xe, r, rex, pe);
             }
             if (xe.aprof) xe.aprof[1] += clock64() - t0;
           }
diff --git a/cage_challenge_4_amd/csrc/cc4_state.h b/cage_challenge_4_amd/csrc/cc4_state.h
--- a/cage_challenge_4_amd/csrc/cc4_state.h
+++ b/cage_challenge_4_amd/csrc/cc4_state.h
@@ -109,6 +109,146 @@
   uint8_t pad[1];
 };
 static_assert(sizeof(RedHdr) == 32, "RedHdr is two 16-byte vectors");
+
+struct WField { int word, shift, width; };
+constexpr WField wfield_at(size_t off, size_t size) { return WField{(int)(off / 4), (int)(off % 4) * 8, (int)size * 8}; }
+constexpr uint32_t wfield_max(WField f) { return f.width >= 32 ? 0xFFFFFFFFu : ((1u << f.width) - 1u); }
+constexpr uint32_t wfield_mask(WField f) { return wfield_max(f) << f.shift; }
+enum : int {
+  RH_Q_TYPE, RH_Q_HOST, RH_Q_ARG, RH_Q_TICKS, RH_Q_SID, RH_Q_BUSY, RH_AS_SUBNET, RH_FSM_STEP, RH_NEW_SESS_ID, RH_NSESS, RH_NKNOWN, RH_FSM_N,
+  RH_NOBS, RH_NLIVE, RH_ACTIVE, RH_OBS_SUCCESS, RH_OBS_ACT_TYPE, RH_OBS_ACT_HOST, RH_OBS_ACT_ARG, RH_EXEC_TYPE, RH_EXEC_HOST, RH_NEW_SESS_HOST,
+  RH_START_HOST, RH_RSC_DIRTY, RH_RSC_LISTED, RH_FSM_DIRTY, RH_NFIELDS
+};
+enum : int { AW_TYPE, AW_HOST, AW_ARG, AW_TICKS, AW_SID, AW_BUSY, AW_NFIELDS };
+#define CC4_WF(T, m) wfield_at(offsetof(T, m), sizeof(T::m))
+#define CC4_WFQ(m) wfield_at(offsetof(RedHdr, queue) + offsetof(Act, m), sizeof(Act::m))
+constexpr WField act_field(int f) {
+  switch (f) {
+    case AW_TYPE: return CC4_WF(Act, type);   case AW_HOST: return CC4_WF(Act, host);   case AW_ARG: return CC4_WF(Act, arg);
+    case AW_TICKS: return CC4_WF(Act, ticks); case AW_SID: return CC4_WF(Act, sid);     default: return CC4_WF(Act, busy);
+  }
+}
+constexpr WField hdr_field(int f) {
+  switch (f) {
+    case RH_Q_TYPE: return CC4_WFQ(type);   case RH_Q_HOST: return CC4_WFQ(host);   case RH_Q_ARG: return CC4_WFQ(arg);
+    case RH_Q_TICKS: return CC4_WFQ(ticks); case RH_Q_SID: return CC4_WFQ(sid);     case RH_Q_BUSY: return CC4_WFQ(busy);
+    case RH_AS_SUBNET: return CC4_WF(RedHdr, as_subnet);         case RH_FSM_STEP: return CC4_WF(RedHdr, fsm_step);
+    case RH_NEW_SESS_ID: return CC4_WF(RedHdr, new_sess_id);     case RH_NSESS: return CC4_WF(RedHdr, nsess);
+    case RH_NKNOWN: return CC4_WF(RedHdr, nknown);               case RH_FSM_N: return CC4_WF(RedHdr, fsm_n);
+    case RH_NOBS: return CC4_WF(RedHdr, nobs);                   case RH_NLIVE: return CC4_WF(RedHdr, nlive);
+    case RH_ACTIVE: return CC4_WF(RedHdr, active);               case RH_OBS_SUCCESS: return CC4_WF(RedHdr, obs_success);
+    case RH_OBS_ACT_TYPE: return CC4_WF(RedHdr, obs_act_type);   case RH_OBS_ACT_HOST: return CC4_WF(RedHdr, obs_act_host);
+    case RH_OBS_ACT_ARG: return CC4_WF(RedHdr, obs_act_arg);     case RH_EXEC_TYPE: return CC4_WF(RedHdr, exec_type);
+    case RH_EXEC_HOST: return CC4_WF(RedHdr, exec_host);         case RH_NEW_SESS_HOST: return CC4_WF(RedHdr, new_sess_host);
+    case RH_START_HOST: return CC4_WF(RedHdr, start_host);       case RH_RSC_DIRTY: return CC4_WF(RedHdr, rsc_dirty);
+    case RH_RSC_LISTED: return CC4_WF(RedHdr, rsc_listed);       default: return CC4_WF(RedHdr, fsm_dirty);
+  }
+}
+#undef CC4_WF
+#undef CC4_WFQ
+constexpr bool wfields_tile(WField (*field)(int), int nfields, int nwords, int pad_bits) {
+  uint32_t used[8] = {0, 0, 0, 0, 0, 0, 0, 0};
+  int bits = 0;
+  for (int f = 0; f < nfields; ++f) {
+    const WField d = field(f);
+    if (d.word < 0 || d.word >= nwords || d.width < 8 || d.shift + d.width > 32 || (used[d.word] & wfield_mask(d))) return false;
+    used[d.word] |= wfield_mask(d); bits += d.width;
+  }
+  return bits + pad_bits == 32 * nwords;
+}
+static_assert(wfields_tile(hdr_field, RH_NFIELDS, 8, 8 * (int)sizeof(RedHdr::pad)), "the header's word fields are RedHdr's members");
+static_assert(wfields_tile(act_field, AW_NFIELDS, 2, 0) && sizeof(Act) == 8, "the action word's fields are Act's members");
+static_assert(hdr_field(RH_Q_TYPE).word == act_field(AW_TYPE).word && hdr_field(RH_Q_BUSY).word == act_field(AW_BUSY).word && offsetof(RedHdr, queue) == 0,
+              "RedHdr.queue is words 0 and 1 of the header: the header's queue as an action word is w[0] | w[1] << 32");
+static_assert(hdr_field(RH_OBS_SUCCESS).word == 5 && hdr_field(RH_OBS_SUCCESS).shift == 0 && hdr_field(RH_OBS_ACT_TYPE).word == 5 &&
+              hdr_field(RH_OBS_ACT_HOST).word == 5 && hdr_field(RH_OBS_ACT_ARG).word == 5, "obs_first's four bytes are word 5, obs_success lowest");
+static_assert(act_field(AW_TICKS).word == 0 && act_field(AW_TICKS).shift == 24 && hdr_field(RH_FSM_STEP).shift == 16 && hdr_field(RH_FSM_STEP).width == 16,
+              "ticks and fsm_step are the top fields of their words: a count on the word wraps as the member does");
+
+struct RedHdrW { uint32_t w[8]; };
+typedef uint64_t ActW;
+template <int F> CC4_HD uint32_t hget(const RedHdrW& H) { constexpr WField d = hdr_field(F); return (H.w[d.word] >> d.shift) & wfield_max(d); }
+template <int F> CC4_HD void hset(RedHdrW& H, uint32_t v) {
+  constexpr WField d = hdr_field(F);
+  H.w[d.word] = (H.w[d.word] & ~wfield_mask(d)) | ((v & wfield_max(d)) << d.shift);
+}
+template <int F> CC4_HD void hinc(RedHdrW& H) {
+  constexpr WField d = hdr_field(F);
+  if (d.shift + d.width == 32) H.w[d.word] += 1u << d.shift; else hset<F>(H, hget<F>(H) + 1u);
+}
+template <int F> CC4_HD uint32_t aget(ActW a) { constexpr WField d = act_field(F); return ((uint32_t)(a >> (32 * d.word)) >> d.shift) & wfield_max(d); }
+template <int F> CC4_HD ActW aset(ActW a, uint32_t v) {
+  constexpr WField d = act_field(F);
+  return (a & ~((uint64_t)wfield_mask(d) << (32 * d.word))) | ((uint64_t)(v & wfield_max(d)) << (32 * d.word + d.shift));
+}
+CC4_HD constexpr ActW act_word(uint32_t type, uint32_t host, uint32_t arg, uint32_t ticks, uint32_t sid, uint32_t busy) {
+  return (uint64_t)((type & 0xFFu) << act_field(AW_TYPE).shift | (host & 0xFFu) << act_field(AW_HOST).shift | (arg & 0xFFu) << act_field(AW_ARG).shift |
+                    (ticks & 0xFFu) << act_field(AW_TICKS).shift) |
+         (uint64_t)((sid & 0xFFFFu) << act_field(AW_SID).shift | (busy & 0xFFFFu) << act_field(AW_BUSY).shift) << 32;
+}
+CC4_HD ActW act_tick(ActW a) { return (a & 0xFFFFFFFF00000000ull) | (uint32_t)((uint32_t)a - (1u << 24)); }
+CC4_HD ActW act_pack(const Act& a) { return act_word(a.type, a.host, a.arg, a.ticks, a.sid, a.busy); }
+CC4_HD Act act_unpack(ActW w) {
+  Act a; a.type = (uint8_t)aget<AW_TYPE>(w); a.host = (uint8_t)aget<AW_HOST>(w); a.arg = (uint8_t)aget<AW_ARG>(w); a.ticks = (uint8_t)aget<AW_TICKS>(w);
+  a.sid = (uint16_t)aget<AW_SID>(w); a.busy = (uint16_t)aget<AW_BUSY>(w);
+  return a;
+}
+CC4_HD ActW hdr_queue(const RedHdrW& H) { return (uint64_t)H.w[0] | (uint64_t)H.w[1] << 32; }
+CC4_HD void hdr_set_queue(RedHdrW& H, ActW q) { H.w[0] = (uint32_t)q; H.w[1] = (uint32_t)(q >> 32); }
+CC4_HD void hdr_tick_reset(RedHdrW& H) {
+  H.w[hdr_field(RH_NOBS).word] &= ~wfield_mask(hdr_field(RH_NOBS));
+  uint32_t& ow = H.w[hdr_field(RH_OBS_SUCCESS).word];
+  ow = (ow & ~(wfield_mask(hdr_field(RH_OBS_SUCCESS)) | wfield_mask(hdr_field(RH_OBS_ACT_TYPE)))) | (uint32_t)RA_NONE << hdr_field(RH_OBS_ACT_TYPE).shift;
+  H.w[hdr_field(RH_NEW_SESS_HOST).word] |= wfield_mask(hdr_field(RH_NEW_SESS_HOST));
+  H.w[hdr_field(RH_RSC_LISTED).word] &= ~wfield_mask(hdr_field(RH_RSC_LISTED));
+}
+CC4_HD constexpr uint32_t hdr_obs_word(uint32_t success, uint32_t type, uint32_t host, uint32_t arg) {
+  return (success & 0xFFu) | (type & 0xFFu) << hdr_field(RH_OBS_ACT_TYPE).shift | (host & 0xFFu) << hdr_field(RH_OBS_ACT_HOST).shift | (arg & 0xFFu) << hdr_field(RH_OBS_ACT_ARG).shift;
+}
+#if defined(__HIP_DEVICE_COMPILE__)
+typedef uint32_t cc4_u32x4 __attribute__((ext_vector_type(4)));
+#endif
+enum : int { HDR_LO = 1, HDR_HI = 2, HDR_BOTH = 3 };
+CC4_HD RedHdrW hdr_load(const RedHdr* h, int which = HDR_BOTH) {
+  RedHdrW H;
+#if defined(__HIP_DEVICE_COMPILE__)
+  cc4_u32x4 a = {0u, 0u, 0u, 0u}, b = {0u, 0u, 0u, 0u};
+  if (which & HDR_LO) { __builtin_memcpy(&a, h, 16); asm volatile("" : "+v"(a)); }
+  if (which & HDR_HI) { __builtin_memcpy(&b, reinterpret_cast<const char*>(h) + 16, 16); asm volatile("" : "+v"(b)); }
+  H.w[0] = a.x; H.w[1] = a.y; H.w[2] = a.z; H.w[3] = a.w; H.w[4] = b.x; H.w[5] = b.y; H.w[6] = b.z; H.w[7] = b.w;
+#else
+  for (int i = 0; i < 8; ++i) H.w[i] = 0;
+  if (which & HDR_LO) __builtin_memcpy(H.w, h, 16);
+  if (which & HDR_HI) __builtin_memcpy(H.w + 4, reinterpret_cast<const char*>(h) + 16, 16);
+#endif
+  return H;
+}
+CC4_HD uint32_t hdr_word(const RedHdr* h, int word) {
+  uint32_t w; __builtin_memcpy(&w, reinterpret_cast<const char*>(__builtin_assume_aligned(h, 16)) + 4 * word, 4);
+#if defined(__HIP_DEVICE_COMPILE__)
+  asm volatile("" : "+v"(w));
+#endif
+  return w;
+}
+template <int F> CC4_HD uint32_t wget(uint32_t w) { constexpr WField d = hdr_field(F); return (w >> d.shift) & wfield_max(d); }
+CC4_HD void hdr_store(RedHdr* h, const RedHdrW& H, int which = HDR_BOTH) {
+#if defined(__HIP_DEVICE_COMPILE__)
+  if (which & HDR_LO) { cc4_u32x4 a = {H.w[0], H.w[1], H.w[2], H.w[3]}; asm volatile("" : "+v"(a)); __builtin_memcpy(h, &a, 16); }
+  if (which & HDR_HI) { cc4_u32x4 b = {H.w[4], H.w[5], H.w[6], H.w[7]}; asm volatile("" : "+v"(b)); __builtin_memcpy(reinterpret_cast<char*>(h) + 16, &b, 16); }
+#else
+  if (which & HDR_LO) __builtin_memcpy(h, H.w, 16);
+  if (which & HDR_HI) __builtin_memcpy(reinterpret_cast<char*>(h) + 16, H.w + 4, 16);
+#endif
+}
+CC4_HD ActW act_load(const Act* a) {
+  ActW w; __builtin_memcpy(&w, a, 8);
+#if defined(__HIP_DEVICE_COMPILE__)
+  asm volatile("" : "+v"(w));
+#endif
+  return w;
+}
+CC4_HD void act_store(Act* a, ActW w) { __builtin_memcpy(a, &w, 8); }
+
 struct alignas(16) RedAgent {
   alignas(8) uint8_t sord[MAX_RS];
   uint32_t known_bm[8];
```

Result: faster. 1.637 billion, median of 6 (+1.7%).
